# NDLOHGRP/pyReCoDe

Measured on AMD Instinct MI355X. Metric: frames/sec + GB/s in, 4096x4096 uint16 @1% sparsity, 1/2/4/8 GPU, higher is better.
Workload: dtype u16; 1 GPU; 4096x4096 uint16, 1.00% sparsity, L1 + LZ4 frame, source_bit_depth 16, batch 64 frames/GPU/step, 256-frame stack/GPU in HBM; parallelism=dp1 (contiguous frame blocks per rank; single process: no collective), gather_every=0, gathers_issued_in_all=0, launch=single process, collective_ranks=1

## Files before the change

### pyrecode_amd/csrc/rc_api.hip

```cpp
#include "rc_host.h"
#include "rc_deflate_model.h"

thread_local std::string g_last_error;
WorkerPool *g_pool = new WorkerPool;
Util g_utils[RC_MAX_DEV];
thread_local Util *t_util = nullptr;


struct rc_ctx {
    int device = 0;
    hipStream_t own_stream = nullptr, stream = nullptr;
    uint32_t nx = 0, ny = 0, depth = 0, level = 0, op_mode = 0, scheme = 0, clevel = 0, max_batch = 0;
    uint32_t emit = rc::EMIT_RAW;
    rc::Scratch sets[2];
    int cur = 0;
    int last = 0;
    const rc::Scratch &geo() const { return sets[0]; }
    const rc::Scratch &recent() const { return sets[last]; }
    DevMem dmem, model_mem[2];
    PinMem hmem;
    hipStream_t pstream = nullptr;
    hipStream_t pstream_b = nullptr;
    hipStream_t last_ps = nullptr;
    bool two_chains = false;
    hipEvent_t ev_red[2] = {}, ev_post[2] = {}, ev_in[2] = {};
    bool post_pending[2] = {false, false};
    bool pipelined = false;
    bool thr_set = false;
    bool keep_bitmap = true;
    uint32_t src_bytes = 2;
    uint32_t *thr32 = nullptr;
    uint32_t last_n = 0;
    DevBuf d_frames, d_out, d_dark;
    uint64_t *d_rec_off = nullptr;
    uint32_t *d_md = nullptr;
    void *d_ztab = nullptr;
    rc::ValueStage values = rc::VALUES_NONE;
    bool values_on = false;
    bool modelled = false, model_ready = false;
    rc::ZstdModel *d_model = nullptr, *h_model = nullptr;
    rc::ZstdSample *d_sample = nullptr, *h_sample = nullptr;
    rc::DeflateModel *d_dzm = nullptr, *h_dzm = nullptr;
    uint32_t *d_dzhist = nullptr, *h_dzhist = nullptr;
    uint32_t l2_sum = 0;
    rc::u32x2 *d_l2_node[2] = {};
    uint16_t *d_l2_base[2] = {};
    rc::BatchStatus *h_status = nullptr;
    rc::BatchStatus *d_first_err = nullptr;
    uint32_t batch_seq = 0;
    const uint8_t *prev_out = nullptr, *prev_rec = nullptr, *prev_md = nullptr;
    uint64_t prev_out_cap = 0;
    uint32_t prev_n = 0;
    hipEvent_t ev[5] = {};
    float stage_ms[5] = {};
    bool profiling = false;
    uint32_t prof_every = 1, prof_phase = 0;
    bool profile_all = getenv("RC_PROFILE_ALL_STAGES") != nullptr;
    struct PipeSlot {
        uint8_t *d_in = nullptr;
        uint8_t *d_out = nullptr;
        uint64_t *d_rec = nullptr, *h_rec = nullptr;
        uint32_t *d_md = nullptr, *h_md = nullptr;
        rc::BatchStatus *h_stat = nullptr;
        hipEvent_t ev_h2d = nullptr, ev_done = nullptr, ev_fetch = nullptr, ev_val = nullptr;
        uint32_t *d_val = nullptr, *h_val = nullptr;
        bool has_val = false;
        uint32_t n = 0;
        bool zero_copy = false;
        enum State { FREE, SUBMITTED, RESULT_TAKEN, FETCHING } state = FREE;
    } pipe[RC_PIPE_SLOTS];
    hipStream_t copy_stream = nullptr, d2h_stream = nullptr;
    uint32_t val_gap = 0, val_x0 = 0, val_y0 = 0, val_w = 0, val_h = 0;
    std::vector<hipEvent_t> prof_ev;
    size_t prof_used = 0;
    double prof_sum_ms[5] = {};
    uint64_t prof_batches = 0;
};

RC_EXPORT int rc_abi_version(void) { return RC_ABI_VERSION; }

RC_EXPORT const char *rc_strerror(int status)
{
    switch (status) {
    case RC_OK: return "ok";
    case RC_ERR_BAD_ARG: return "bad argument";
    case RC_ERR_OUT_TOO_SMALL: return "output buffer too small";
    case RC_ERR_DEVICE: return "GPU / HIP error";
    case RC_ERR_UNSUPPORTED: return "not implemented on device";
    case RC_ERR_RECORD_TOO_LARGE: return "Buffer size smaller than compressed data size";
    case RC_ERR_CORRUPT: return "corrupt input stream";
    case RC_ERR_WORKSPACE: return "out of device memory for the ctx's workspace";
    default: return "unknown status";
    }
}
RC_EXPORT const char *rc_last_error(void) { return g_last_error.c_str(); }

RC_EXPORT int rc_device_count(int *count)
{
    if (!count) return fail(RC_ERR_BAD_ARG, "count is NULL");
    int n = 0;
    if (hipGetDeviceCount(&n) != hipSuccess) {
        (void)hipGetLastError();
        n = 0;
    }
    *count = n;
    return RC_OK;
}
RC_EXPORT int rc_scheme_on_device(uint32_t scheme)
{
    return (scheme == RC_SCHEME_LZ4 || scheme == RC_SCHEME_ZSTD || scheme == RC_SCHEME_BLOSC_LZ4 || scheme == RC_SCHEME_ZLIB_DEVICE) ? 1 : 0;
}

static int alloc_set(rc_ctx *c, rc::Scratch &sc, DevMem &model_mem)
{
    using namespace rc;
    DevMem &m = c->dmem;
    const uint64_t B = c->max_batch, T = sc.ntiles;
    RC_ALLOC(m, sc.bitmap, B * sc.nb_stride + 64);
    RC_ALLOC(m, sc.tile_cnt, B * T * 4);
    RC_ALLOC(m, sc.tile_off, B * T * 4);
    RC_ALLOC(m, sc.tile_next, B * T * 4);
    RC_ALLOC(m, sc.frame_nnz, B * 4);
    RC_ALLOC(m, sc.frame_cbytes, B * 4);
    RC_ALLOC(m, sc.scan_part, B * ((T + 255) / 256) * 32);
    RC_ALLOC(m, sc.status, sizeof(BatchStatus));
    if (c->level != 3) RC_ALLOC(m, sc.pix_slots, B * T * TILE_PX * 2 + 64);
    if (c->emit != EMIT_RAW) {
        if (c->level == 1) {
            sc.comb = c->emit == EMIT_ZSTD ? COMB_AT_BLK_SLOT : COMB_BEHIND_BLOCK;
            sc.blk_stride = 1536;
        }
        RC_ALLOC(m, sc.blk_slots, B * T * (uint64_t)sc.blk_stride + 256);
        RC_ALLOC(m, sc.blk_size, B * T * 4);
        RC_ALLOC(m, sc.blk_off, B * T * 4);
        if (c->emit == EMIT_DEFLATE) {
            RC_ALLOC(m, sc.blk_aux, B * T * 4);
            RC_ALLOC(m, sc.zl_acc, B * 32);
            HIP_TRY(hipMemset(sc.zl_acc, 0, B * 32));
        }
    }
    if (c->values != VALUES_NONE) {
        const ValueGeom g = value_geom(c->values);
        sc.pixraw_stride = ((sc.N * 2 + 15) & ~15ull) + 32;
        sc.nchunk_max = (uint32_t)((sc.N * 2 + g.chunk - 1) / g.chunk) + 1;
        RC_ALLOC(model_mem, sc.pixraw, B * sc.pixraw_stride + 64);
        RC_ALLOC(model_mem, sc.pix_chunks, B * (uint64_t)sc.nchunk_max * g.slot + 64);
        if (c->values == VALUES_DEFLATE_HUFF) RC_ALLOC(model_mem, sc.chunk_aux, B * (uint64_t)(sc.nchunk_max + 1) * 8);
        RC_ALLOC(model_mem, sc.chunk_size, B * (uint64_t)sc.nchunk_max * 4);
        RC_ALLOC(model_mem, sc.chunk_off, B * (uint64_t)sc.nchunk_max * 4);
        RC_ALLOC(model_mem, sc.frame_pbytes, B * 4);
        HIP_TRY(hipMemset(sc.frame_pbytes, 0, B * 4));
    }
    HIP_TRY(hipMemset(sc.frame_nnz, 0, B * 4));
    HIP_TRY(hipMemset(sc.frame_cbytes, 0, B * 4));
    HIP_TRY(hipMemset(sc.status, 0, sizeof(BatchStatus)));
    return RC_OK;
}

static void free_value_stage(rc_ctx *c)
{
    c->values = rc::VALUES_NONE;
    c->values_on = false;
    for (int k = 0; k < 2; ++k) {
        rc::Scratch &set = c->sets[k];
        c->model_mem[k].release_all();
        set.pixraw = nullptr; set.pix_chunks = nullptr; set.chunk_aux = nullptr; set.chunk_size = nullptr; set.chunk_off = nullptr;
        set.frame_pbytes = nullptr; set.pixraw_stride = 0; set.nchunk_max = 0;
    }
}

static int ctx_alloc(rc_ctx *c)
{
    using namespace rc;
    const uint64_t B = c->max_batch;
    RC_ON_DEVICE(c->device);
    HIP_TRY(hipStreamCreateWithFlags(&c->own_stream, hipStreamNonBlocking));
    HIP_TRY(hipStreamCreateWithFlags(&c->pstream, hipStreamNonBlocking));
    {
        int lo = 0, hi = 0;
        HIP_TRY(hipDeviceGetStreamPriorityRange(&lo, &hi));
        HIP_TRY(hipStreamCreateWithPriority(&c->pstream_b, hipStreamNonBlocking, hi));
    }
    c->last_ps = c->pstream;
    c->stream = c->own_stream;
    DevMem &m = c->dmem;
    int r;
    RC_ALLOC(m, c->sets[0].thr, c->geo().N * 2);
    RC_ALLOC(m, c->d_first_err, sizeof(BatchStatus));
    HIP_TRY(hipMemset(c->d_first_err, 0, sizeof(BatchStatus)));
    c->sets[0].first_err = c->d_first_err;
    c->sets[1] = c->sets[0];
    for (int k = 0; k < 2; ++k)
        if ((r = alloc_set(c, c->sets[k], c->model_mem[k])) != RC_OK) return r;
    c->two_chains = false;
    if (c->level == 2) {
        const uint64_t ids = (uint64_t)c->geo().ntiles * rc::TILE_PX;
        RC_ALLOC(m, c->d_l2_node[0], B * ids * 8);
        HIP_TRY(hipMemset(c->d_l2_node[0], 0, B * ids * 8));
        RC_ALLOC(m, c->d_l2_base[0], B * (uint64_t)c->geo().ntiles * 64 * 2);
        for (int i = 0; i < 2; ++i) {
            Scratch &set = c->sets[i];
            set.l2_node = c->d_l2_node[0]; set.l2_ids_per_frame = ids; set.l2_base = c->d_l2_base[0];
        }
    }
    if (c->emit == EMIT_ZSTD) {
        if ((r = zstd_encoder_tables(m, c->d_ztab)) != RC_OK) return r;
        c->modelled = c->clevel != 0;
        if (c->modelled) {
            RC_ALLOC(m, c->d_model, sizeof(ZstdModel));
            RC_ALLOC(m, c->d_sample, sizeof(ZstdSample));
            RC_ALLOC(c->hmem, c->h_model, sizeof(ZstdModel));
            RC_ALLOC(c->hmem, c->h_sample, sizeof(ZstdSample));
        }
    }
    if (c->values == VALUES_DEFLATE_HUFF) {
        RC_ALLOC(m, c->d_dzm, sizeof(DeflateModel));
        RC_ALLOC(m, c->d_dzhist, 256 * 4);
        RC_ALLOC(c->hmem, c->h_dzm, sizeof(DeflateModel));
        RC_ALLOC(c->hmem, c->h_dzhist, 256 * 4);
    }
    RC_ALLOC(m, c->d_rec_off, (B + 1) * 8);
    RC_ALLOC(m, c->d_md, B * 3 * 4);
    RC_ALLOC(c->hmem, c->h_status, 2 * sizeof(BatchStatus));
    for (auto &e : c->ev) HIP_TRY(hipEventCreate(&e));
    for (auto &e : c->ev_red) HIP_TRY(hipEventCreateWithFlags(&e, hipEventDisableTiming));
    for (auto &e : c->ev_post) HIP_TRY(hipEventCreateWithFlags(&e, hipEventDisableTiming));
    for (auto &e : c->ev_in) HIP_TRY(hipEventCreateWithFlags(&e, hipEventDisableTiming));
    return RC_OK;
}

RC_EXPORT rc_ctx *rc_ctx_create(uint32_t nx, uint32_t ny, uint32_t src_bit_depth, uint32_t reduction_level,
                                uint32_t op_mode, uint32_t scheme, uint32_t clevel, int device_id, uint32_t max_batch,
                                int *status)
{
    int dummy;
    if (!status) status = &dummy;
    *status = RC_OK;
    if (nx == 0 || ny == 0 || max_batch == 0 || max_batch > 65535u || op_mode > 1) {
        *status = fail(RC_ERR_BAD_ARG, "nx, ny, max_batch must be > 0, max_batch <= 65535 and op_mode 0 or 1");
        return nullptr;
    }
    if ((uint64_t)nx * ny >= (1ull << 32)) {
        *status = fail(RC_ERR_BAD_ARG, "nx*ny must be < 2^32");
        return nullptr;
    }
    if ((uint64_t)nx * ny * 2 >= (1ull << 32)) {
        *status = fail(RC_ERR_UNSUPPORTED, "a raw frame of 4 GiB or more (nx*ny*bytes_per_pixel >= 2^32) does not fit the format's u32 size fields");
        return nullptr;
    }
    if (reduction_level < 1 || reduction_level > 3) {
        *status = fail(RC_ERR_UNSUPPORTED, "reduction_level 4 (centroiding) is not implemented on device");
        return nullptr;
    }
    if (reduction_level == 2 && nx > 65535u) {
        *status = fail(RC_ERR_UNSUPPORTED, "reduction_level 2 needs nx <= 65535");
        return nullptr;
    }
    if (src_bit_depth < 1 || src_bit_depth > 32) {
        *status = fail(RC_ERR_UNSUPPORTED, "source_bit_depth must be 1..32 (uint8 / uint16 / uint32 source frames)");
        return nullptr;
    }
    int ndev = 0;
    if (hipGetDeviceCount(&ndev) != hipSuccess || device_id < 0 || device_id >= ndev) {
        (void)hipGetLastError();
        *status = fail(RC_ERR_DEVICE, "no such HIP device (this library has no CPU path)");
        return nullptr;
    }
    rc_ctx *c = new (std::nothrow) rc_ctx();
    if (!c) {
        *status = fail(RC_ERR_DEVICE, "out of host memory");
        return nullptr;
    }
    c->device = device_id;
    c->nx = nx; c->ny = ny; c->depth = src_bit_depth; c->level = reduction_level; c->op_mode = op_mode;
    c->scheme = scheme; c->clevel = clevel; c->max_batch = max_batch;
    c->emit = (op_mode == 1 && rc_scheme_on_device(scheme)) ? scheme : rc::EMIT_RAW;
    c->values = rc::value_stage_of(c->emit, clevel, reduction_level);
    rc::Scratch &sc = c->sets[0];
    sc.N = (uint64_t)nx * ny;
    sc.ntiles = (uint32_t)((sc.N + rc::TILE_PX - 1) / rc::TILE_PX);
    sc.nb = (sc.N + 7) / 8;
    sc.nb_stride = (uint64_t)sc.ntiles * rc::TILE_BM;
    sc.max_batch = max_batch;
    sc.guarded_loads = getenv("RC_REDUCE_GUARDED_LOADS") != nullptr;
    int rcode = ctx_alloc(c);
    if (rcode != RC_OK) {
        *status = rcode;
        std::string keep = g_last_error;
        rc_ctx_destroy(c);
        g_last_error = keep;
        return nullptr;
    }
    return c;
}

RC_EXPORT int rc_ctx_destroy(rc_ctx *c)
{
    if (!c) return RC_OK;
    DeviceGuard dev_guard_;
    (void)dev_guard_.enter(c->device);
    for (hipStream_t st : {c->stream, c->pstream, c->pstream_b, c->own_stream, c->copy_stream, c->d2h_stream})
        if (st) (void)hipStreamSynchronize(st);
    c->dmem.release_all();
    for (DevMem &m : c->model_mem) m.release_all();
    c->hmem.release_all();
    for (auto &p : c->pipe)
        for (hipEvent_t e : {p.ev_h2d, p.ev_done, p.ev_fetch, p.ev_val})
            if (e) (void)hipEventDestroy(e);
    for (hipEvent_t e : {c->ev_red[0], c->ev_red[1], c->ev_post[0], c->ev_post[1], c->ev_in[0], c->ev_in[1]})
        if (e) (void)hipEventDestroy(e);
    for (auto &e : c->ev)
        if (e) (void)hipEventDestroy(e);
    for (auto &e : c->prof_ev) (void)hipEventDestroy(e);
    for (hipStream_t st : {c->copy_stream, c->d2h_stream, c->pstream, c->pstream_b, c->own_stream})
        if (st) (void)hipStreamDestroy(st);
    delete c;
    return RC_OK;
}

RC_EXPORT int rc_ctx_set_stream(rc_ctx *c, void *hip_stream)
{
    if (!c) return fail(RC_ERR_BAD_ARG, "ctx is NULL");
    c->stream = hip_stream ? reinterpret_cast<hipStream_t>(hip_stream) : c->own_stream;
    return RC_OK;
}

RC_EXPORT int rc_set_threshold(rc_ctx *c, const void *thr)
{
    if (!c || !thr) return fail(RC_ERR_BAD_ARG, "ctx / thr is NULL");
    if (c->depth > 16 && c->src_bytes != 4) return fail(RC_ERR_BAD_ARG, "src_bit_depth > 16 means uint32 sources: rc_ctx_set_source_bytes(ctx, 4) first");
    RC_ON_DEVICE(c->device);
    HIP_TRY(hipMemcpyAsync(c->src_bytes == 4 ? (void *)c->thr32 : (void *)c->geo().thr, thr, c->geo().N * (c->src_bytes == 4 ? 4 : 2),
                           is_device_ptr(thr) ? hipMemcpyDeviceToDevice : hipMemcpyHostToDevice,
                           c->stream));
    HIP_TRY(hipStreamSynchronize(c->stream));
    c->thr_set = true;
    return RC_OK;
}

RC_EXPORT int rc_set_dark(rc_ctx *c, const void *dark, int64_t epsilon)
{
    if (!c || !dark) return fail(RC_ERR_BAD_ARG, "ctx / dark is NULL");
    RC_ON_DEVICE(c->device);
    const void *src = dark;
    const uint64_t bytes = c->geo().N * c->src_bytes;
    if (!is_device_ptr(dark)) {
        int r = c->d_dark.ensure(c->dmem, bytes);
        if (r != RC_OK) return r;
        HIP_TRY(hipMemcpyAsync(c->d_dark.p, dark, bytes, hipMemcpyHostToDevice, c->stream));
        src = c->d_dark.p;
    }
    if (c->depth > 16 && c->src_bytes != 4) return fail(RC_ERR_BAD_ARG, "src_bit_depth > 16 means uint32 sources: rc_ctx_set_source_bytes(ctx, 4) first");
    if (c->src_bytes == 4) rc::launch_threshold32(static_cast<const uint32_t *>(src), epsilon, c->geo().N, c->thr32, c->stream);
    else rc::launch_threshold(src, epsilon, c->geo().N, c->geo().thr, c->stream, c->src_bytes);
    HIP_TRY(hipGetLastError());
    HIP_TRY(hipStreamSynchronize(c->stream));
    c->thr_set = true;
    return RC_OK;
}

RC_EXPORT int rc_ctx_set_source_bytes(rc_ctx *c, uint32_t bytes_per_pixel)
{
    if (!c) return fail(RC_ERR_BAD_ARG, "ctx is NULL");
    if (bytes_per_pixel != 1 && bytes_per_pixel != 2 && bytes_per_pixel != 4) return fail(RC_ERR_BAD_ARG, "rc_ctx_set_source_bytes: 1 (uint8), 2 (uint16) or 4 (uint32)");
    if (bytes_per_pixel == 1 && c->depth > 8) return fail(RC_ERR_BAD_ARG, "rc_ctx_set_source_bytes: uint8 sources need src_bit_depth <= 8");
    if (bytes_per_pixel == 2 && c->depth > 16) return fail(RC_ERR_BAD_ARG, "rc_ctx_set_source_bytes: uint16 sources need src_bit_depth <= 16");
    if (c->batch_seq || c->thr_set) return fail(RC_ERR_BAD_ARG, "rc_ctx_set_source_bytes: call before rc_set_dark / rc_set_threshold and the first batch");
    if (c->geo().N * bytes_per_pixel >= (1ull << 32))
        return fail(RC_ERR_UNSUPPORTED, "rc_ctx_set_source_bytes: a raw frame of 4 GiB or more (nx*ny*bytes_per_pixel >= 2^32) does not fit the format's u32 size fields");
    if (bytes_per_pixel == 4) {
        if (c->depth <= 16) return fail(RC_ERR_BAD_ARG, "rc_ctx_set_source_bytes: uint32 sources are what source_bit_depth > 16 means (misc.py:41-49)");
        if (c->level == 2) return fail(RC_ERR_UNSUPPORTED, "rc_ctx_set_source_bytes: reduction level 2 is not implemented for uint32 sources");
        if (c->emit == rc::EMIT_DEFLATE) return fail(RC_ERR_UNSUPPORTED, "rc_ctx_set_source_bytes: the device DEFLATE encoder is not implemented for uint32 sources (use RC_SCHEME_ZLIB: the host's zlib)");
        RC_ON_DEVICE(c->device);
        uint32_t *thr32 = nullptr;
        uint16_t *slots[2] = {nullptr, nullptr};
        bool ok = c->dmem.try_alloc(thr32, c->geo().N * 4) == hipSuccess;
        for (int k = 0; ok && k < 2 && c->level != 3; ++k)
            ok = c->dmem.try_alloc(slots[k], (uint64_t)c->max_batch * c->geo().ntiles * rc::TILE_PX * 4 + 64) == hipSuccess;
        if (!ok) {
            (void)hipGetLastError();
            c->dmem.free_one(thr32);
            for (uint16_t *&p : slots) c->dmem.free_one(p);
            return fail(RC_ERR_DEVICE, "rc_ctx_set_source_bytes: out of device memory for the uint32 threshold / residual slots");
        }
        if (c->depth % 8 == 0) c->depth = 32;
        c->modelled = false;
        free_value_stage(c);
        c->thr32 = thr32;
        for (int k = 0; k < 2; ++k) {
            rc::Scratch *set = &c->sets[k];
            set->pix_slot_bytes = rc::TILE_PX * 4;
            set->comb = rc::COMB_OFF;
            if (c->level != 3) {
                c->dmem.free_one(set->pix_slots);
                set->pix_slots = slots[k];
            }
        }
    }
    c->src_bytes = bytes_per_pixel;
    return RC_OK;
}
RC_EXPORT uint32_t rc_ctx_source_bytes(const rc_ctx *c) { return c ? c->src_bytes : 0; }

RC_EXPORT uint64_t rc_out_capacity(const rc_ctx *c, uint32_t n) { return c ? (uint64_t)n * c->geo().N * c->src_bytes : 0; }

RC_EXPORT uint32_t rc_md_fields(const rc_ctx *c)
{
    if (!c) return 0;
    const bool comp = c->emit != rc::EMIT_RAW;
    if (c->level != 3) return comp ? 3 : 1;
    return comp ? 1 : 0;
}

static int fit_value_model(rc_ctx *c, const void *frames_dev, uint32_t n)
{
    using namespace rc;
    const bool dz = c->values == VALUES_DEFLATE_HUFF;
    hipStream_t s = c->stream;
    const Scratch &sc = c->sets[c->cur];
    const uint32_t ns = n < 2 ? n : 2;
    void *d_sample = dz ? (void *)c->d_dzhist : c->d_sample, *h_sample = dz ? (void *)c->h_dzhist : c->h_sample;
    void *d_model = dz ? (void *)c->d_dzm : c->d_model, *h_model = dz ? (void *)c->h_dzm : c->h_model;
    const size_t sample_bytes = dz ? 256 * 4 : sizeof(ZstdSample), model_bytes = dz ? sizeof(DeflateModel) : sizeof(ZstdModel);
    for (int k = 0; k < 2; ++k)
        if (c->post_pending[k]) HIP_TRY(hipStreamWaitEvent(s, c->ev_post[k], 0));
    HIP_TRY(hipMemsetAsync(d_sample, 0, sample_bytes, s));
    if (dz) {
        launch_reduce(sc, frames_dev, ns, 1u, CODEC_DEFLATE, true, c->depth, s, nullptr, c->src_bytes);
        launch_scans(sc, ns, true, true, s);
        RecordParams rp;
        rp.level = 1u; rp.emit = c->emit; rp.depth = c->depth; rp.first_frame_id = 0; rp.packed_slots = 1u;
        rp.frame_bytes = c->geo().N * c->src_bytes;
        rp.pix_mode = PIX_MODE_FLAT;
        launch_assemble(sc, rp, ns, nullptr, nullptr, c->batch_seq, s);
        launch_pd_hist(sc, ns, c->depth, c->d_dzhist, s);
    } else {
        launch_reduce(sc, frames_dev, ns, c->level == 3 ? 3u : 1u, CODEC_ZSTD_FAST, true, c->depth, s, nullptr, c->src_bytes);
        launch_zstd_sample(sc, ns, c->level == 1, c->depth, c->d_sample, s);
    }
    HIP_TRY(hipGetLastError());
    HIP_TRY(hipMemcpyAsync(h_sample, d_sample, sample_bytes, hipMemcpyDeviceToHost, s));
    HIP_TRY(hipStreamSynchronize(s));
    if (dz) {
        dm_build_model(c->h_dzhist, c->h_dzm);
        c->values_on = c->h_dzm->usable != 0;
    } else {
        zstd_model_from_sample(c->h_sample, c->h_model, c->clevel == 1 ? 50u : (c->clevel == 2 ? 20u : 0u));
        if (c->values == VALUES_NONE || !zm_code_pays(c->h_sample->pix, c->h_model->pix_code)) c->h_model->valid &= ~ZM_PIX_CODE;
        c->values_on = (c->h_model->valid & ZM_PIX_CODE) != 0;
    }
    HIP_TRY(hipMemcpyAsync(d_model, h_model, model_bytes, hipMemcpyHostToDevice, s));
    HIP_TRY(hipStreamSynchronize(s));
    for (Scratch &set : c->sets) {
        if (dz) { set.dz_model = c->d_dzm; continue; }
        const ZstdModel &M = *c->h_model;
        set.zm_model = c->d_model;
        set.zm_lit_code = c->d_model->lit_code;
        set.zm_valid = M.valid;
        set.zm_budget = zm_block_budget(M, BLK_SLOT);
        set.zm_seq_bits = (M.valid & ZM_SEQ_TABLES) ? M.seq.ll_log + M.seq.ml_log : 12u;
    }
    c->model_ready = true;
    return RC_OK;
}

static uint32_t fused_codec(uint32_t emit, uint32_t clevel, bool modelled, uint32_t src_bytes)
{
    using namespace rc;
    switch (emit) {
    case EMIT_ZSTD: return modelled && src_bytes != 4 ? CODEC_ZSTD_MODELLED : CODEC_ZSTD_FAST;
    case EMIT_LZ4: return clevel != 0 ? CODEC_LZ4_EVENTS : CODEC_LZ4_RUNS;
    case EMIT_BLOSC: return CODEC_BLOSC;
    case EMIT_DEFLATE: return CODEC_DEFLATE;
    default: return CODEC_NONE;
    }
}

static int enqueue_batch(rc_ctx *c, const void *frames_dev, uint32_t n, uint32_t first_frame_id, uint8_t *out_dev,
                         uint64_t out_cap, uint64_t *rec_off_dev, uint32_t *md_dev, bool timed)
{
    using namespace rc;
    hipStream_t s = c->stream;
    if ((c->modelled || c->values == VALUES_DEFLATE_HUFF) && !c->model_ready) {
        int r = fit_value_model(c, frames_dev, n);
        if (r != RC_OK) return r;
    }
    RecordParams rp;
    rp.level = c->level == 3 ? 3u : 1u;
    rp.emit = c->emit; rp.depth = c->depth; rp.first_frame_id = first_frame_id;
    rp.packed_slots = 1u;
    rp.frame_bytes = c->geo().N * c->src_bytes;
    hipEvent_t *ev = nullptr;
    if (timed) ev = c->ev;
    else if (c->profiling && (c->prof_phase++ % c->prof_every) == 0) {
        if (c->prof_used + 5 > c->prof_ev.size()) {
            for (int i = 0; i < 5; ++i) {
                hipEvent_t e;
                HIP_TRY(hipEventCreate(&e));
                c->prof_ev.push_back(e);
            }
        }
        ev = c->prof_ev.data() + c->prof_used;
        c->prof_used += 5;
    }
    const int k = c->cur;
    c->cur ^= 1;
    c->last = k;
    const rc::Scratch &sc = c->sets[k];
    const bool two = c->pipelined && c->two_chains;
    hipStream_t ps = two && k == 1 ? c->pstream_b : c->pstream;
    c->last_ps = ps;
    if (c->post_pending[k]) HIP_TRY(hipStreamWaitEvent(s, c->ev_post[k], 0));
    if (ev) HIP_TRY(hipEventRecord(ev[0], s));
    const bool fitted_seq = c->modelled && (c->h_model->valid & ZM_SEQ_TABLES);
    hipStream_t tail = nullptr;
    if (sc.N % TILE_PX) {
        HIP_TRY(hipEventRecord(c->ev_in[k], s));
        HIP_TRY(hipStreamWaitEvent(ps, c->ev_in[k], 0));
        tail = ps;
    }
    const uint32_t codec = fused_codec(c->emit, c->clevel, c->modelled, c->src_bytes);
    const bool keep_maps = c->keep_bitmap || c->emit == EMIT_RAW;
    if (c->src_bytes == 4)
        launch_reduce32(sc, static_cast<const uint32_t *>(frames_dev), c->thr32, n, c->level, c->depth, s, codec, keep_maps);
    else
        launch_reduce(sc, frames_dev, n, c->level, codec, keep_maps, c->depth, s, tail, c->src_bytes);
    const bool all_ev = ev && (timed || c->profile_all);
    hipEvent_t red = ev ? ev[1] : c->ev_red[k];
    HIP_TRY(hipEventRecord(red, s));
    HIP_TRY(hipStreamWaitEvent(ps, red, 0));
    if (c->level == 2) launch_l2(sc, n, c->nx, c->l2_sum, c->depth, ps);
    const bool lits_only = c->modelled && (c->h_model->valid & ZM_LITS_ONLY);
    if (c->emit == EMIT_ZSTD && !lits_only) launch_zstd_fse(sc, n, fitted_seq ? (const void *)&c->d_model->seq : c->d_ztab, fitted_seq, ps);
    if (all_ev) HIP_TRY(hipEventRecord(ev[2], ps));
    launch_scans(sc, n, c->level != 3, c->emit != EMIT_RAW, ps);
    if (all_ev) HIP_TRY(hipEventRecord(ev[3], ps));
    if (c->values_on) {
        rp.pix_mode = PIX_MODE_FLAT;
        launch_assemble(sc, rp, n, out_dev, rec_off_dev, c->batch_seq, ps);
        launch_values_encode(c->values, sc, n, c->depth, ps);
        launch_values_scan(c->values, sc, n, c->depth, ps);
        rp.pix_mode = PIX_MODE_SKIP;
    }
    if (two && c->post_pending[k ^ 1]) {
        auto overlap = [](const uint8_t *a, uint64_t an, const uint8_t *b, uint64_t bn) { return a && b && a < b + bn && b < a + an; };
        const uint8_t *rec8 = reinterpret_cast<const uint8_t *>(rec_off_dev), *md8 = reinterpret_cast<const uint8_t *>(md_dev);
        if (overlap(out_dev, out_cap, c->prev_out, c->prev_out_cap) || overlap(rec8, (uint64_t)(n + 1) * 8, c->prev_rec, (uint64_t)(c->prev_n + 1) * 8) ||
            overlap(md8, (uint64_t)n * 12, c->prev_md, (uint64_t)c->prev_n * 12))
            HIP_TRY(hipStreamWaitEvent(ps, c->ev_post[k ^ 1], 0));
    }
    c->prev_out = out_dev; c->prev_out_cap = out_cap; c->prev_n = n;
    c->prev_rec = reinterpret_cast<const uint8_t *>(rec_off_dev); c->prev_md = reinterpret_cast<const uint8_t *>(md_dev);
    launch_layout(sc, rp, n, out_cap, rec_off_dev, md_dev, ps);
    launch_assemble(sc, rp, n, out_dev, rec_off_dev, c->batch_seq, ps);
    ++c->batch_seq;
    if (c->values_on) launch_values_gather(c->values, sc, n, c->depth, 16, out_dev, rec_off_dev, ps);
    if (ev) HIP_TRY(hipEventRecord(ev[4], ps));
    if (two && c->post_pending[k ^ 1]) HIP_TRY(hipStreamWaitEvent(ps, c->ev_post[k ^ 1], 0));
    HIP_TRY(hipEventRecord(c->ev_post[k], ps));
    c->post_pending[k] = true;
    if (!c->pipelined) HIP_TRY(hipStreamWaitEvent(s, c->ev_post[k], 0));
    HIP_TRY(hipGetLastError());
    c->last_n = n;
    return RC_OK;
}

static int check_batch_args(rc_ctx *c, const void *frames, uint32_t n, const void *out, const void *rec, const void *md)
{
    if (!c || !frames || !out || !rec || !md) return fail(RC_ERR_BAD_ARG, "NULL argument");
    if (n == 0 || n > c->max_batch) return fail(RC_ERR_BAD_ARG, "n must be in 1..max_batch");
    if (!c->thr_set) return fail(RC_ERR_BAD_ARG, "threshold not set (rc_set_threshold / rc_set_dark)");
    return RC_OK;
}

RC_EXPORT int rc_reduce_compress_batch_async(rc_ctx *c, const void *frames_dev, uint32_t n, uint32_t first_frame_id,
                                             uint8_t *out_dev, uint64_t out_cap, uint64_t *rec_offsets_dev, uint32_t *md_dev)
{
    int r = check_batch_args(c, frames_dev, n, out_dev, rec_offsets_dev, md_dev);
    if (r != RC_OK) return r;
    RC_ON_DEVICE(c->device);
    return enqueue_batch(c, frames_dev, n, first_frame_id, out_dev, out_cap, rec_offsets_dev, md_dev, false);
}

static void l2_second_chain(rc_ctx *c)
{
    if (c->level != 2 || c->two_chains) return;
    const uint64_t B = c->max_batch, ids = (uint64_t)c->geo().ntiles * rc::TILE_PX;
    if (!c->d_l2_node[1]) {
        bool ok = c->dmem.try_alloc(c->d_l2_node[1], B * ids * 8) == hipSuccess && hipMemset(c->d_l2_node[1], 0, B * ids * 8) == hipSuccess &&
                  c->dmem.try_alloc(c->d_l2_base[1], B * (uint64_t)c->geo().ntiles * 64 * 2) == hipSuccess && hipDeviceSynchronize() == hipSuccess;
        if (!ok) {
            (void)hipGetLastError();
            c->dmem.free_one(c->d_l2_node[1]);
            c->dmem.free_one(c->d_l2_base[1]);
            return;
        }
    }
    c->sets[1].l2_node = c->d_l2_node[1];
    c->sets[1].l2_base = c->d_l2_base[1];
    c->two_chains = true;
}

RC_EXPORT int rc_ctx_set_pipelined(rc_ctx *c, int on)
{
    if (!c) return fail(RC_ERR_BAD_ARG, "ctx is NULL");
    RC_ON_DEVICE(c->device);
    HIP_TRY(hipStreamSynchronize(c->pstream));
    HIP_TRY(hipStreamSynchronize(c->pstream_b));
    if (on) l2_second_chain(c);
    c->pipelined = on != 0;
    return RC_OK;
}
RC_EXPORT int rc_ctx_wait_results(rc_ctx *c, void *hip_stream)
{
    if (!c) return fail(RC_ERR_BAD_ARG, "ctx is NULL");
    RC_ON_DEVICE(c->device);
    if (c->post_pending[c->last])
        HIP_TRY(hipStreamWaitEvent(hip_stream ? reinterpret_cast<hipStream_t>(hip_stream) : c->stream, c->ev_post[c->last], 0));
    return RC_OK;
}

RC_EXPORT int rc_ctx_sync(rc_ctx *c)
{
    if (!c) return fail(RC_ERR_BAD_ARG, "ctx is NULL");
    RC_ON_DEVICE(c->device);
    HIP_TRY(hipStreamSynchronize(c->pstream_b));
    HIP_TRY(hipMemcpyAsync(&c->h_status[0], c->recent().status, sizeof(rc::BatchStatus), hipMemcpyDeviceToHost, c->pstream));
    HIP_TRY(hipMemcpyAsync(&c->h_status[1], c->d_first_err, sizeof(rc::BatchStatus), hipMemcpyDeviceToHost, c->pstream));
    HIP_TRY(hipMemsetAsync(c->d_first_err, 0, sizeof(rc::BatchStatus), c->pstream));
    HIP_TRY(hipStreamSynchronize(c->pstream));
    HIP_TRY(hipStreamSynchronize(c->stream));
    const uint32_t n_batches = c->batch_seq;
    c->batch_seq = 0;
    for (size_t b = 0; b + 5 <= c->prof_used; b += 5) {
        float ms;
        if (!c->profile_all) {
            if (hipEventElapsedTime(&ms, c->prof_ev[b], c->prof_ev[b + 1]) == hipSuccess) c->prof_sum_ms[0] += ms;
        } else
        for (int i = 0; i < 4; ++i)
            if (hipEventElapsedTime(&ms, c->prof_ev[b + i], c->prof_ev[b + i + 1]) == hipSuccess) c->prof_sum_ms[i] += ms;
        if (hipEventElapsedTime(&ms, c->prof_ev[b], c->prof_ev[b + 4]) == hipSuccess) c->prof_sum_ms[4] += ms;
        ++c->prof_batches;
    }
    c->prof_used = 0;
    if (c->h_status[1].total != 0) c->h_status[1] = rc::first_err_decode(c->h_status[1].total);
    if (c->h_status[1].code != 0) {
        char msg[160];
        if (n_batches > 1)
            snprintf(msg, sizeof msg, "%s (frame %u of batch %llu of the %u enqueued since the last sync)", rc_strerror(c->h_status[1].code),
                     c->h_status[1].frame, (unsigned long long)c->h_status[1].total, n_batches);
        else
            snprintf(msg, sizeof msg, "%s (frame %u of the batch)", rc_strerror(c->h_status[1].code), c->h_status[1].frame);
        return fail(c->h_status[1].code, msg);
    }
    return RC_OK;
}

RC_EXPORT int rc_reduce_compress_batch(rc_ctx *c, const void *frames, uint32_t n, uint32_t first_frame_id, uint8_t *out,
                                       uint64_t out_cap, uint64_t *rec_offsets, uint32_t *md)
{
    int r = check_batch_args(c, frames, n, out, rec_offsets, md);
    if (r != RC_OK) return r;
    RC_ON_DEVICE(c->device);
    const uint64_t frame_bytes = c->geo().N * c->src_bytes;
    const void *fdev = frames;
    if (!is_device_ptr(frames)) {
        r = c->d_frames.ensure(c->dmem, (uint64_t)n * frame_bytes);
        if (r != RC_OK) return r;
        HIP_TRY(hipMemcpyAsync(c->d_frames.p, frames, (uint64_t)n * frame_bytes, hipMemcpyHostToDevice, c->stream));
        fdev = c->d_frames.p;
    }
    uint8_t *odev = out;
    uint64_t cap = out_cap;
    const bool out_host = !is_device_ptr(out);
    if (out_host) {
        const uint64_t worst = (uint64_t)n * frame_bytes;
        cap = out_cap < worst ? out_cap : worst;
        r = c->d_out.ensure(c->dmem, cap);
        if (r != RC_OK) return r;
        odev = c->d_out.p;
    }
    r = enqueue_batch(c, fdev, n, first_frame_id, odev, cap, c->d_rec_off, c->d_md, true);
    if (r != RC_OK) return r;
    r = rc_ctx_sync(c);
    for (int i = 0; i < 4; ++i) (void)hipEventElapsedTime(&c->stage_ms[i], c->ev[i], c->ev[i + 1]);
    (void)hipEventElapsedTime(&c->stage_ms[4], c->ev[0], c->ev[4]);
    if (r != RC_OK) return r;
    int r2 = copy_out(rec_offsets, c->d_rec_off, (uint64_t)(n + 1) * 8, c->stream);
    if (r2 == RC_OK) r2 = copy_out(md, c->d_md, (uint64_t)n * 12, c->stream);
    if (r2 == RC_OK && out_host) r2 = copy_out(out, c->d_out.p, c->h_status->total, c->stream);
    if (r2 != RC_OK) return r2;
    HIP_TRY(hipStreamSynchronize(c->stream));
    return RC_OK;
}

RC_EXPORT void *rc_host_alloc(uint64_t bytes)
{
    void *p = nullptr;
    if (hipHostMalloc(&p, bytes ? bytes : 16, hipHostMallocDefault) != hipSuccess) {
        (void)hipGetLastError();
        fail(RC_ERR_DEVICE, "hipHostMalloc failed");
        return nullptr;
    }
    return p;
}
RC_EXPORT int rc_host_free(void *p)
{
    if (p) HIP_TRY(hipHostFree(p));
    return RC_OK;
}
RC_EXPORT int rc_host_register(void *p, uint64_t bytes)
{
    if (!p || !bytes) return fail(RC_ERR_BAD_ARG, "NULL / zero argument");
    HIP_TRY(hipHostRegister(p, bytes, hipHostRegisterDefault));
    return RC_OK;
}
RC_EXPORT int rc_host_unregister(void *p)
{
    if (p) HIP_TRY(hipHostUnregister(p));
    return RC_OK;
}

static int pipe_slot_init(rc_ctx *c, rc_ctx::PipeSlot &p)
{
    const uint64_t B = c->max_batch;
    if (!c->copy_stream) HIP_TRY(hipStreamCreateWithFlags(&c->copy_stream, hipStreamNonBlocking));
    if (!c->d2h_stream) HIP_TRY(hipStreamCreateWithFlags(&c->d2h_stream, hipStreamNonBlocking));
    RC_ALLOC(c->dmem, p.d_in, B * c->geo().N * c->src_bytes + 64);
    RC_ALLOC(c->dmem, p.d_out, rc_out_capacity(c, (uint32_t)B) + 64);
    RC_ALLOC(c->dmem, p.d_rec, (B + 1) * 8);
    RC_ALLOC(c->dmem, p.d_md, B * 12);
    RC_ALLOC(c->hmem, p.h_rec, (B + 1) * 8);
    RC_ALLOC(c->hmem, p.h_md, B * 12);
    RC_ALLOC(c->hmem, p.h_stat, sizeof(rc::BatchStatus));
    HIP_TRY(hipEventCreateWithFlags(&p.ev_h2d, hipEventDisableTiming));
    HIP_TRY(hipEventCreateWithFlags(&p.ev_done, hipEventDisableTiming));
    HIP_TRY(hipEventCreateWithFlags(&p.ev_fetch, hipEventDisableTiming));
    HIP_TRY(hipEventCreateWithFlags(&p.ev_val, hipEventDisableTiming));
    RC_ALLOC(c->dmem, p.d_val, B * 4 + 64);
    RC_ALLOC(c->hmem, p.h_val, B * 4 + 64);
    return RC_OK;
}

RC_EXPORT int rc_ctx_set_validation(rc_ctx *c, uint32_t gap, uint32_t x0, uint32_t y0, uint32_t w, uint32_t h)
{
    if (!c) return fail(RC_ERR_BAD_ARG, "ctx is NULL");
    if (gap && (w == 0 || h == 0 || w > 128 || h > 128 || (uint64_t)x0 + w > c->nx || (uint64_t)y0 + h > c->ny))
        return fail(RC_ERR_BAD_ARG, "rc_ctx_set_validation: the region must lie inside the frame and hold at most 128 x 128 pixels");
    c->val_gap = gap; c->val_x0 = x0; c->val_y0 = y0; c->val_w = w; c->val_h = h;
    return RC_OK;
}

RC_EXPORT int rc_pipe_validation(rc_ctx *c, uint32_t slot, uint32_t *counts)
{
    if (!c || slot >= RC_PIPE_SLOTS || !counts) return fail(RC_ERR_BAD_ARG, "NULL argument / slot out of range");
    rc_ctx::PipeSlot &p = c->pipe[slot];
    if (p.state != p.SUBMITTED && p.state != p.RESULT_TAKEN) return fail(RC_ERR_BAD_ARG, "nothing submitted on this slot");
    if (!p.has_val) { for (uint32_t i = 0; i < p.n; ++i) counts[i] = 0xFFFFFFFFu; return RC_OK; }
    HIP_TRY(hipEventSynchronize(p.ev_val));
    memcpy(counts, p.h_val, (uint64_t)p.n * 4);
    return RC_OK;
}

RC_EXPORT int rc_pipe_submit(rc_ctx *c, uint32_t slot, const void *frames_host, uint32_t n, uint32_t first_frame_id)
{
    if (!c || !frames_host || slot >= RC_PIPE_SLOTS) return fail(RC_ERR_BAD_ARG, "NULL argument / slot out of range");
    if (n == 0 || n > c->max_batch) return fail(RC_ERR_BAD_ARG, "n must be in 1..max_batch");
    if (!c->thr_set) return fail(RC_ERR_BAD_ARG, "threshold not set (rc_set_threshold / rc_set_dark)");
    RC_ON_DEVICE(c->device);
    rc_ctx::PipeSlot &p = c->pipe[slot];
    if (p.state != p.FREE) return fail(RC_ERR_BAD_ARG, "slot is still in use (result / fetch_wait not called)");
    if (!p.d_in) {
        int r = pipe_slot_init(c, p);
        if (r != RC_OK) return r;
    }
    if (!c->pipelined) {
        HIP_TRY(hipStreamSynchronize(c->pstream));
        HIP_TRY(hipStreamSynchronize(c->pstream_b));
        l2_second_chain(c);
        c->pipelined = true;
    }
    const void *fdev = nullptr;
    hipPointerAttribute_t a;
    if (hipPointerGetAttributes(&a, frames_host) == hipSuccess) {
        if (a.type == hipMemoryTypeHost && a.devicePointer) fdev = a.devicePointer;
    } else (void)hipGetLastError();
    p.zero_copy = fdev != nullptr;
    if (!fdev) {
        HIP_TRY(hipMemcpyAsync(p.d_in, frames_host, (uint64_t)n * c->geo().N * c->src_bytes, hipMemcpyHostToDevice, c->copy_stream));
        HIP_TRY(hipEventRecord(p.ev_h2d, c->copy_stream));
        HIP_TRY(hipStreamWaitEvent(c->stream, p.ev_h2d, 0));
        fdev = p.d_in;
    }
    int r = enqueue_batch(c, fdev, n, first_frame_id, p.d_out, rc_out_capacity(c, c->max_batch), p.d_rec, p.d_md, false);
    if (r != RC_OK) return r;
    p.has_val = c->val_gap != 0;
    if (p.has_val) {
        rc::launch_roi_components(fdev, c->src_bytes == 4 ? (const void *)c->thr32 : (const void *)c->geo().thr, c->geo().N, c->nx, n, first_frame_id, c->val_gap, c->val_x0, c->val_y0, c->val_w, c->val_h, p.d_val, c->stream, c->src_bytes);
        HIP_TRY(hipGetLastError());
        HIP_TRY(hipMemcpyAsync(p.h_val, p.d_val, (uint64_t)n * 4, hipMemcpyDeviceToHost, c->stream));
        HIP_TRY(hipEventRecord(p.ev_val, c->stream));
    }
    if (p.zero_copy) HIP_TRY(hipEventRecord(p.ev_h2d, c->stream));
    hipStream_t ps = c->last_ps;
    HIP_TRY(hipMemcpyAsync(p.h_rec, p.d_rec, (uint64_t)(n + 1) * 8, hipMemcpyDeviceToHost, ps));
    HIP_TRY(hipMemcpyAsync(p.h_md, p.d_md, (uint64_t)n * 12, hipMemcpyDeviceToHost, ps));
    HIP_TRY(hipMemcpyAsync(p.h_stat, c->recent().status, sizeof(rc::BatchStatus), hipMemcpyDeviceToHost, ps));
    HIP_TRY(hipEventRecord(p.ev_done, ps));
    p.n = n;
    p.state = p.SUBMITTED;
    return RC_OK;
}

RC_EXPORT int rc_pipe_input_done(rc_ctx *c, uint32_t slot)
{
    if (!c || slot >= RC_PIPE_SLOTS) return fail(RC_ERR_BAD_ARG, "NULL argument / slot out of range");
    if (c->pipe[slot].state == rc_ctx::PipeSlot::FREE) return RC_OK;
    HIP_TRY(hipEventSynchronize(c->pipe[slot].ev_h2d));
    return RC_OK;
}

RC_EXPORT int rc_pipe_result(rc_ctx *c, uint32_t slot, uint64_t *rec_offsets, uint32_t *md, uint64_t *total)
{
    if (!c || slot >= RC_PIPE_SLOTS || !rec_offsets || !md || !total) return fail(RC_ERR_BAD_ARG, "NULL argument / slot out of range");
    rc_ctx::PipeSlot &p = c->pipe[slot];
    if (p.state != p.SUBMITTED) return fail(RC_ERR_BAD_ARG, "nothing submitted on this slot");
    HIP_TRY(hipEventSynchronize(p.ev_done));
    p.state = p.RESULT_TAKEN;
    if (p.h_stat->code != 0) {
        char msg[128];
        snprintf(msg, sizeof msg, "%s (frame %u of the batch)", rc_strerror(p.h_stat->code), p.h_stat->frame);
        p.state = p.FREE;
        return fail(p.h_stat->code, msg);
    }
    memcpy(rec_offsets, p.h_rec, (uint64_t)(p.n + 1) * 8);
    memcpy(md, p.h_md, (uint64_t)p.n * 12);
    *total = p.h_stat->total;
    return RC_OK;
}

RC_EXPORT int rc_pipe_fetch(rc_ctx *c, uint32_t slot, uint8_t *dst_host, uint64_t bytes)
{
    if (!c || slot >= RC_PIPE_SLOTS || (!dst_host && bytes)) return fail(RC_ERR_BAD_ARG, "NULL argument / slot out of range");
    rc_ctx::PipeSlot &p = c->pipe[slot];
    if (p.state != p.RESULT_TAKEN) return fail(RC_ERR_BAD_ARG, "rc_pipe_result has not been called for this slot");
    if (bytes > p.h_stat->total) return fail(RC_ERR_BAD_ARG, "more bytes than the batch's records hold");
    RC_ON_DEVICE(c->device);
    if (bytes) HIP_TRY(hipMemcpyAsync(dst_host, p.d_out, bytes, hipMemcpyDeviceToHost, c->d2h_stream));
    HIP_TRY(hipEventRecord(p.ev_fetch, c->d2h_stream));
    p.state = p.FETCHING;
    return RC_OK;
}

RC_EXPORT int rc_pipe_fetch_wait(rc_ctx *c, uint32_t slot)
{
    if (!c || slot >= RC_PIPE_SLOTS) return fail(RC_ERR_BAD_ARG, "NULL argument / slot out of range");
    rc_ctx::PipeSlot &p = c->pipe[slot];
    if (p.state == p.RESULT_TAKEN) { p.state = p.FREE; return RC_OK; }
    if (p.state != p.FETCHING) return fail(RC_ERR_BAD_ARG, "rc_pipe_fetch has not been called for this slot");
    HIP_TRY(hipEventSynchronize(p.ev_fetch));
    p.state = p.FREE;
    return RC_OK;
}

RC_EXPORT int rc_ctx_refit_model(rc_ctx *c)
{
    if (!c) return fail(RC_ERR_BAD_ARG, "ctx is NULL");
    c->model_ready = false;
    return RC_OK;
}

RC_EXPORT int rc_get_binary_map(rc_ctx *c, uint32_t i, uint8_t *bitmap_out)
{
    if (!c || !bitmap_out) return fail(RC_ERR_BAD_ARG, "NULL argument");
    if (i >= c->last_n) return fail(RC_ERR_BAD_ARG, "frame index outside the most recent batch");
    if (!c->keep_bitmap && c->emit != rc::EMIT_RAW && c->level != 2) return fail(RC_ERR_BAD_ARG, "binary maps are not kept (rc_ctx_keep_binary_maps(ctx, 0))");
    RC_ON_DEVICE(c->device);
    int r = copy_out(bitmap_out, c->recent().bitmap + (uint64_t)i * c->geo().nb_stride, c->geo().nb, c->stream);
    if (r != RC_OK) return r;
    HIP_TRY(hipStreamSynchronize(c->stream));
    return RC_OK;
}

RC_EXPORT int rc_ctx_set_profiling(rc_ctx *c, int on)
{
    if (!c) return fail(RC_ERR_BAD_ARG, "ctx is NULL");
    c->profiling = on != 0;
    c->prof_every = on > 1 ? (uint32_t)on : 1u;
    c->prof_phase = 0;
    for (double &v : c->prof_sum_ms) v = 0;
    c->prof_batches = 0;
    return RC_OK;
}
RC_EXPORT int rc_ctx_get_profile(rc_ctx *c, double sum_ms[5], uint64_t *batches)
{
    if (!c || !sum_ms || !batches) return fail(RC_ERR_BAD_ARG, "NULL argument");
    memcpy(sum_ms, c->prof_sum_ms, sizeof c->prof_sum_ms);
    *batches = c->prof_batches;
    return RC_OK;
}

RC_EXPORT int rc_ctx_set_l2_statistics(rc_ctx *c, uint32_t l2_statistics)
{
    if (!c || l2_statistics > 2) return fail(RC_ERR_BAD_ARG, "l2_statistics must be 0, 1 (max) or 2 (sum)");
    c->l2_sum = l2_statistics == 2 ? 1u : 0u;
    return RC_OK;
}

RC_EXPORT int rc_ctx_keep_binary_maps(rc_ctx *c, int on)
{
    if (!c) return fail(RC_ERR_BAD_ARG, "ctx is NULL");
    c->keep_bitmap = on != 0;
    return RC_OK;
}

RC_EXPORT int rc_get_stage_ms(rc_ctx *c, float ms[5])
{
    if (!c || !ms) return fail(RC_ERR_BAD_ARG, "NULL argument");
    memcpy(ms, c->stage_ms, sizeof c->stage_ms);
    return RC_OK;
}

RC_EXPORT int64_t rc_unpack_frame_sparse(uint32_t nx, uint32_t ny, uint32_t bit_depth, const uint8_t *bitmap,
                                         const uint8_t *pixvals, uint64_t pixvals_bytes, uint64_t *out,
                                         uint64_t out_cap_triplets, uint32_t reduction_level)
{
    if (!bitmap || nx == 0 || ny == 0 || (!out && out_cap_triplets)) return fail(RC_ERR_BAD_ARG, "NULL / zero argument");
    if (reduction_level == 1 && (bit_depth == 0 || bit_depth > 64)) return fail(RC_ERR_BAD_ARG, "bit_depth must be 1..64");
    if (reduction_level == 1 && !pixvals && pixvals_bytes) return fail(RC_ERR_BAD_ARG, "pixvals is NULL");
    UtilScope util_scope;
    int r = util_scope.enter();
    if (r != RC_OK) return r;
    Util &u = g_util;
    const uint64_t N = (uint64_t)nx * ny, nb = (N + 7) / 8, nb8 = (nb + 7) / 8;
    const uint32_t nblk = (uint32_t)((nb8 + rc::WG - 1) / rc::WG);
    const uint8_t *d_bm = nullptr, *d_px = nullptr;
    r = stage_in(bitmap, nb, u.a, d_bm, nb8 * 8 - nb + 8);
    if (r != RC_OK) return r;
    if (reduction_level == 1 && pixvals_bytes) {
        r = stage_in(pixvals, pixvals_bytes, u.b, d_px);
        if (r != RC_OK) return r;
    }
    r = u.w.ensure(u.dmem, (uint64_t)nblk * 8 + 16);
    if (r != RC_OK) return r;
    uint32_t *blk_cnt = u.w.as<uint32_t>(), *blk_off = blk_cnt + nblk;
    uint64_t *nnz_dev = reinterpret_cast<uint64_t *>(blk_cnt + 2 * (uint64_t)nblk);
    rc::launch_expand_count(d_bm, nb8, N, blk_cnt, blk_off, nnz_dev, u.stream);
    HIP_TRY(hipMemcpyAsync(u.h_scalar, nnz_dev, 8, hipMemcpyDeviceToHost, u.stream));
    HIP_TRY(hipStreamSynchronize(u.stream));
    const uint64_t nnz = *u.h_scalar;
    if (!out) return (int64_t)nnz;
    if (nnz > out_cap_triplets) return fail(RC_ERR_OUT_TOO_SMALL, "out holds fewer triplets than the bitmap has set bits");
    if (reduction_level == 1 && (nnz * bit_depth + 7) / 8 > pixvals_bytes)
        return fail(RC_ERR_CORRUPT, "pixvals shorter than popcount(bitmap) * bit_depth bits");
    if (nnz == 0) return 0;
    StagedOut so;
    if ((r = so.begin(out, nnz * 24)) != RC_OK) return r;
    rc::launch_expand_emit(d_bm, nb8, N, nx, blk_off, d_px, pixvals_bytes, bit_depth, reduction_level, nnz, so.as<uint64_t>(), u.stream);
    HIP_TRY(hipGetLastError());
    if ((r = so.finish(out, nnz * 24)) != RC_OK) return r;
    return (int64_t)nnz;
}

RC_EXPORT int rc_bit_pack(const uint16_t *pixvals, uint64_t n, uint32_t bit_depth, uint8_t *out, uint64_t out_n)
{
    if (!out || (!pixvals && n)) return fail(RC_ERR_BAD_ARG, "NULL argument");
    if (bit_depth == 0 || bit_depth > 32) return fail(RC_ERR_BAD_ARG, "bit_depth must be 1..32");
    if (out_n != (n * bit_depth + 7) / 8) return fail(RC_ERR_BAD_ARG, "out_n must be ceil(n*bit_depth/8)");
    if (out_n == 0) return RC_OK;
    UtilScope util_scope;
    int r = util_scope.enter();
    if (r != RC_OK) return r;
    Util &u = g_util;
    const uint16_t *d_in = nullptr;
    r = stage_in(pixvals, n * 2, u.a, d_in);
    if (r != RC_OK) return r;
    StagedOut so;
    if ((r = so.begin(out, out_n)) != RC_OK) return r;
    rc::launch_bit_pack(d_in, n, bit_depth, so.as<uint8_t>(), out_n, u.stream);
    HIP_TRY(hipGetLastError());
    return so.finish(out, out_n);
}

RC_EXPORT int rc_bit_unpack(const uint8_t *packed, uint64_t packed_bytes, uint64_t n, uint32_t bit_depth, uint64_t *out)
{
    if (!out || (!packed && packed_bytes)) return fail(RC_ERR_BAD_ARG, "NULL argument");
    if (bit_depth == 0 || bit_depth > 64) return fail(RC_ERR_BAD_ARG, "bit_depth must be 1..64");
    if ((n * bit_depth + 7) / 8 > packed_bytes) return fail(RC_ERR_CORRUPT, "packed shorter than n * bit_depth bits");
    if (n == 0) return RC_OK;
    UtilScope util_scope;
    int r = util_scope.enter();
    if (r != RC_OK) return r;
    Util &u = g_util;
    const uint8_t *d_in = nullptr;
    r = stage_in(packed, packed_bytes, u.a, d_in);
    if (r != RC_OK) return r;
    StagedOut so;
    if ((r = so.begin(out, n * 8)) != RC_OK) return r;
    rc::launch_bit_unpack(d_in, packed_bytes, n, bit_depth, so.as<uint64_t>(), u.stream);
    HIP_TRY(hipGetLastError());
    return so.finish(out, n * 8);
}

RC_EXPORT int rc_synth_dark(int device_id, uint32_t seed, uint64_t n_pixels, uint16_t *dark_dev)
{
    if (!dark_dev) return fail(RC_ERR_BAD_ARG, "NULL argument");
    RC_ON_DEVICE(device_id);
    rc::launch_synth_dark(seed, n_pixels, dark_dev, nullptr);
    HIP_TRY(hipGetLastError());
    HIP_TRY(hipDeviceSynchronize());
    return RC_OK;
}
RC_EXPORT int rc_synth_frames_clustered(int device_id, uint32_t seed, uint32_t first_frame, uint32_t n_frames, uint32_t nx, uint32_t ny,
                                        uint32_t seed_ppm, const uint16_t *dark_dev, uint16_t *frames_dev)
{
    if (!dark_dev || !frames_dev || n_frames == 0 || nx == 0 || ny == 0) return fail(RC_ERR_BAD_ARG, "NULL / zero argument");
    if ((uint64_t)nx * ny > 0xFFFFFFFFull) return fail(RC_ERR_BAD_ARG, "rc_synth_frames_clustered: nx * ny must fit 32 bits");
    RC_ON_DEVICE(device_id);
    rc::launch_synth_frames_clustered(seed, first_frame, n_frames, nx, ny, seed_ppm, dark_dev, frames_dev, nullptr);
    HIP_TRY(hipGetLastError());
    HIP_TRY(hipDeviceSynchronize());
    return RC_OK;
}
RC_EXPORT int rc_synth_frames(int device_id, uint32_t seed, uint32_t first_frame, uint32_t n_frames, uint64_t n_pixels,
                              uint32_t sparsity_ppm, const uint16_t *dark_dev, uint16_t *frames_dev)
{
    if (!dark_dev || !frames_dev || n_frames == 0) return fail(RC_ERR_BAD_ARG, "NULL / zero argument");
    RC_ON_DEVICE(device_id);
    rc::launch_synth_frames(seed, first_frame, n_frames, n_pixels, sparsity_ppm, dark_dev, frames_dev, nullptr);
    HIP_TRY(hipGetLastError());
    HIP_TRY(hipDeviceSynchronize());
    return RC_OK;
}
```

### pyrecode_amd/csrc/rc_device.h

```cpp
#pragma once
#include <hip/hip_runtime.h>
#include <stdint.h>
#include <type_traits>

namespace rc {

template <int V> using int_c = std::integral_constant<int, V>;

constexpr int WG = 256;
constexpr int WAVES = WG / 64;
constexpr int R = 8;
constexpr int GROUP_PX = 64 * 8;
constexpr int TILE_PX = R * GROUP_PX;
constexpr int TILE_BM = TILE_PX / 8;
constexpr int SLOT_PX = TILE_PX;
constexpr int BLK_SLOT = TILE_BM + 128;

typedef uint32_t u32x4 __attribute__((ext_vector_type(4)));
typedef uint32_t u32x2 __attribute__((ext_vector_type(2)));
typedef uint16_t u16x2 __attribute__((ext_vector_type(2)));

__device__ __forceinline__ int lane_id() { return threadIdx.x & 63; }

template <int CTRL, int ROW_MASK = 0xF>
__device__ __forceinline__ uint32_t dpp_zero(uint32_t x)
{
    return (uint32_t)__builtin_amdgcn_update_dpp(0, (int)x, CTRL, ROW_MASK, 0xF, true);
}

__device__ __forceinline__ uint32_t wave_incl_scan(uint32_t x)
{
    x += dpp_zero<0x111>(x);
    x += dpp_zero<0x112>(x);
    x += dpp_zero<0x114>(x);
    x += dpp_zero<0x118>(x);
    x += dpp_zero<0x142, 0xA>(x);
    x += dpp_zero<0x143, 0xC>(x);
    return x;
}

__device__ __forceinline__ uint32_t wave_prev(uint32_t x) { return dpp_zero<0x138>(x); }
__device__ __forceinline__ uint32_t wave_next(uint32_t x) { return dpp_zero<0x130>(x); }

__device__ __forceinline__ uint32_t wave_last(uint32_t x) { return (uint32_t)__builtin_amdgcn_readlane((int)x, 63); }

__device__ __forceinline__ uint64_t wave_incl_scan64(uint64_t x)
{
#pragma unroll
    for (int d = 1; d < 64; d <<= 1) {
        uint64_t y = __shfl_up(x, d);
        if (lane_id() >= d) x += y;
    }
    return x;
}

__device__ __forceinline__ uint32_t block_excl_scan(uint32_t v, uint32_t *sm, uint32_t *total)
{
    const int w = threadIdx.x >> 6;
    uint32_t inc = wave_incl_scan(v);
    if (lane_id() == 63) sm[w] = inc;
    __syncthreads();
    uint32_t base = 0, tot = 0;
#pragma unroll
    for (int i = 0; i < WAVES; ++i) {
        uint32_t t = sm[i];
        if (i < w) base += t;
        tot += t;
    }
    __syncthreads();
    *total = tot;
    return base + inc - v;
}

struct BatchStatus {
    int32_t code;
    uint32_t frame;
    uint64_t total;
};
__host__ __device__ inline unsigned long long first_err_key(uint32_t batch_seq, int32_t code, uint32_t frame)
{
    return ~(((unsigned long long)(batch_seq & 0xFFFFFFu) << 40) | ((unsigned long long)((uint32_t)(-code) & 0xFFu) << 32) | frame);
}
inline BatchStatus first_err_decode(unsigned long long key)
{
    const unsigned long long k = ~key;
    return BatchStatus{-(int32_t)((k >> 32) & 0xFFu), (uint32_t)k, k >> 40};
}

}
```

### pyrecode_amd/csrc/rc_gather.hip

```cpp
#include <cstdlib>

#include "rc_launch.h"
#include "rc_record.h"
#include "rc_deflate_block.h"

namespace rc {

struct GatherArgs {
    const uint8_t *blk_slots, *bitmap;
    const uint16_t *pix_slots;
    const uint32_t *blk_size, *blk_off, *tile_cnt, *tile_off, *tile_next, *frame_nnz, *frame_cbytes, *frame_pbytes;
    const uint32_t *blk_aux;
    uint32_t *zl_acc;
    uint8_t *pixraw;
    BatchStatus *status, *first_err;
    uint64_t nb, nb_stride, pixraw_stride;
    uint32_t ntiles, blk_stride, pix_slot_bytes, comb;
};

typedef u32x4 u32x4_u __attribute__((aligned(1)));
typedef u32x2 u32x2_u __attribute__((aligned(1)));
typedef uint32_t u32_u __attribute__((aligned(1)));
typedef uint16_t u16_u __attribute__((aligned(1)));

__device__ __forceinline__ uint32_t lane_get(uint32_t v, uint32_t src_lane)
{
    return (uint32_t)__builtin_amdgcn_ds_bpermute((int)(4u * src_lane), (int)v);
}

template <bool BITS>
__device__ __forceinline__ u32x4 shift_piece(const u32x4 &x, uint32_t e, uint32_t sh)
{
    u32x4 y = x;
    if (BITS) {
        y[0] = __builtin_amdgcn_alignbit(x[1], x[0], sh); y[1] = __builtin_amdgcn_alignbit(x[2], x[1], sh);
        y[2] = __builtin_amdgcn_alignbit(x[3], x[2], sh); y[3] = __builtin_amdgcn_alignbit(e, x[3], sh);
    }
    return y;
}
__device__ __forceinline__ void put_piece(uint8_t *p, const u32x4 &y, uint32_t valid)
{
    if (valid >= 16) { *reinterpret_cast<u32x4_u *>(p) = y; return; }
    uint32_t a0 = y[0], a1 = y[1];
    if (valid & 8u) { *reinterpret_cast<u32x2_u *>(p) = u32x2{a0, a1}; p += 8; a0 = y[2]; a1 = y[3]; }
    if (valid & 4u) { *reinterpret_cast<u32_u *>(p) = a0; p += 4; a0 = a1; }
    if (valid & 2u) { *reinterpret_cast<u16_u *>(p) = (uint16_t)a0; p += 2; a0 >>= 16; }
    if (valid & 1u) *p = (uint8_t)a0;
}

struct AdlerAcc { uint32_t A, W; };
__device__ __forceinline__ void adler_piece(AdlerAcc &acc, const u32x4 &y, uint32_t valid, uint32_t sp)
{
    uint32_t a = 0, q = 0;
#pragma unroll
    for (int k = 0; k < 4; ++k) {
        const uint32_t nb = valid > 4u * k ? min(valid - 4u * k, 4u) : 0u;
        const uint32_t v = y[k] & (nb >= 4u ? 0xFFFFFFFFu : ((1u << (8u * nb)) - 1u));
        a = __builtin_amdgcn_sad_u8(v, 0u, a);
        q = __builtin_amdgcn_udot4(v, 0x03020100u + 0x04040404u * (uint32_t)k, q, false);
    }
    acc.A += a;
    acc.W = (acc.W + (sp % ADLER_P) * a + q) % ADLER_P;
}
__device__ __forceinline__ void adler_byte(AdlerAcc &acc, uint32_t byte, uint32_t sp)
{
    acc.A += byte;
    acc.W = (acc.W + (sp % ADLER_P) * byte) % ADLER_P;
}

struct ResidGeom { uint32_t b_lo, n, ps0, avail; };
__device__ __forceinline__ ResidGeom resid_geom(uint32_t coff, uint32_t cnt, uint32_t d)
{
    const uint64_t dbit = (uint64_t)coff * d;
    const uint32_t nbits = cnt * d;
    const uint64_t b_lo = (dbit + 7) >> 3, b_hi = (dbit + nbits + 7) >> 3;
    ResidGeom g{(uint32_t)b_lo, (uint32_t)(b_hi - b_lo), (uint32_t)(8 * b_lo - dbit), (uint32_t)((dbit + nbits) & 7u)};
    if (g.avail && g.n) --g.n;
    else g.avail = 0;
    return g;
}

constexpr int GATHER_U = 4, GATHER_UB = 3;
constexpr int GATHER_WPE = 8;
template <bool BITS, int U, bool ADLER>
__global__ __launch_bounds__(64) __attribute__((amdgpu_waves_per_eu(GATHER_WPE))) void k_gather(GatherArgs sc, RecordParams rp, uint8_t *__restrict__ out, const uint64_t *__restrict__ rec_off,
                                               uint32_t lz4f_hdr_bitmap, uint32_t lz4f_hdr_pix, uint32_t batch_seq, uint32_t gpf, uint32_t nitems, uint32_t tpi)
{
    if (sc.status->code != 0) {
        if (blockIdx.x == 0 && threadIdx.x == 0 && sc.first_err)
            atomicMax(reinterpret_cast<unsigned long long *>(&sc.first_err->total), first_err_key(batch_seq, sc.status->code, sc.status->frame));
        return;
    }
    const uint32_t lane = (uint32_t)lane_id();
    const bool flat = rp.pix_mode == PIX_MODE_FLAT, skip_pix = rp.pix_mode == PIX_MODE_SKIP;
    const bool pixp = rp.level == 1 && rp.packed_slots && !skip_pix;
    const bool plain_pos = rp.emit == EMIT_RAW || flat;
    const uint32_t d = rp.depth;
    const FrameFmt ff = frame_fmt(rp.emit);
    const uint32_t bhdr = bitmap_hdr(ff, rp.emit, sc.ntiles);
    const uint8_t *pix_base = reinterpret_cast<const uint8_t *>(sc.pix_slots);
    for (uint32_t item = blockIdx.x; item < nitems; item += gridDim.x) {
        const uint32_t f = item / gpf, g = item - f * gpf, t0 = tpi * g, t = t0 + lane;
        const bool have = lane < tpi && t < sc.ntiles;
        const uint64_t frow = (uint64_t)f * sc.ntiles;
        uint8_t *rec = flat ? sc.pixraw + (uint64_t)f * sc.pixraw_stride : out + rec_off[f];
        const uint32_t nnz = rp.level == 1 ? sc.frame_nnz[f] : 0;
        const uint32_t npk = rp.level == 1 ? packed_bytes(nnz, d) : 0;
        uint64_t bitmap_pos = 0, pix_pos = 0;
        uint32_t cb = 0;
        if (!flat) {
            if (rp.emit == EMIT_RAW) { bitmap_pos = rp.level == 1 ? 8 : 4; pix_pos = bitmap_pos + sc.nb; }
            else { cb = bhdr + sc.frame_cbytes[f] + ff.end; bitmap_pos = rp.level == 1 ? 16 : 8; pix_pos = bitmap_pos + cb; }
        }
        if (g == 0 && lane == 0 && !flat) record_fixed_fields(sc, rp, f, rec, bitmap_pos, pix_pos, cb, npk, ff, skip_pix, lz4f_hdr_bitmap, lz4f_hdr_pix);
        uint8_t *pdst = rec + pix_pos;

        uint32_t word = 0, bsz = 0, bdst = 0, cnt = 0, rn = 0, rdst = 0, rs = 0xFFFFFFFFu, ps0 = 0, flags = 0, blo = 0;
        AdlerAcc ad{0u, 0u};
        if (have && rp.emit != EMIT_RAW && (!flat || (sc.comb == COMB_BEHIND_BLOCK && pixp))) word = sc.blk_size[frow + t];
        if (have && !flat) {
            if (rp.emit == EMIT_RAW) {
                const uint64_t b0 = (uint64_t)t * TILE_BM;
                bsz = (uint32_t)min((uint64_t)TILE_BM, sc.nb - b0);
                bdst = (uint32_t)(bitmap_pos + b0);
            } else {
                bsz = word;
                const uint32_t boff = bhdr + sc.blk_off[frow + t];
                bdst = (uint32_t)bitmap_pos + boff;
                if (rp.emit == EMIT_BLOSC) store_u32_le(rec + bitmap_pos + 16 + 4 * (uint64_t)t, boff);
            }
        }
        if (have && pixp) {
            cnt = sc.tile_cnt[frow + t];
            if (cnt) {
                const ResidGeom q = resid_geom(sc.tile_off[frow + t], cnt, d);
                ps0 = q.ps0;
                if (ADLER) blo = q.b_lo;
                if (sc.comb) {
                    const uint32_t ro16 = sc.comb == COMB_AT_BLK_SLOT ? (uint32_t)BLK_SLOT / 16 : (word + 15) >> 4, r16 = (cnt * d + 127) >> 7;
                    if (16 * (ro16 + r16) <= sc.blk_stride) rs = 16 * ro16;
                }
                if (q.n && !plain_pos && ((uint64_t)q.b_lo >> ff.chunk_shift) != (((uint64_t)q.b_lo + q.n - 1) >> ff.chunk_shift)) flags = 1u << 31;
                else rn = q.n;
                rdst = (uint32_t)(pix_pos + (plain_pos ? (uint64_t)q.b_lo : stored_pos(ff, q.b_lo)));
            }
        }
        uint32_t ext_cnt = 0, ext_first = 0;
        if (BITS && pixp && t0 + tpi < sc.ntiles) {
            ext_cnt = sc.tile_cnt[frow + t0 + tpi];
            if (ext_cnt)
                ext_first = *reinterpret_cast<const uint32_t *>(residual_src(sc, frow + t0 + tpi, sc.comb == COMB_BEHIND_BLOCK ? sc.blk_size[frow + t0 + tpi] : 0u, ext_cnt, d));
        }
        const uint8_t *slot = rp.emit == EMIT_RAW ? sc.bitmap + (uint64_t)f * sc.nb_stride + (uint64_t)t0 * TILE_BM : sc.blk_slots + (frow + t0) * sc.blk_stride;
        const uint32_t slot_stride = rp.emit == EMIT_RAW ? (uint32_t)TILE_BM : sc.blk_stride;
        const uint8_t *rslot = pix_base + (frow + t0) * sc.pix_slot_bytes;

        const uint32_t nb16 = (bsz + 15) >> 4, tot = nb16 + ((rn + 15) >> 4);
        const uint32_t incl = wave_incl_scan(tot), cum = incl - tot, T = wave_last(incl);
        const uint32_t packed = bsz | (ps0 << 10) | (rn << 13) | flags;
        for (uint32_t i0 = 0; 64u * i0 < T; i0 += U) {
            u32x4 x[U];
            uint32_t e[U], dsto[U], meta[U];
            uint32_t spos[ADLER ? U : 1];
#pragma unroll
            for (int u = 0; u < U; ++u) {
                const uint32_t P = 64u * (i0 + u) + lane;
                uint32_t k = 0;
#pragma unroll
                for (uint32_t step = 32; step; step >>= 1) {
                    const uint32_t c = lane_get(cum, k + step);
                    if (c <= P) k += step;
                }
                const uint32_t ck = lane_get(cum, k), pk = lane_get(packed, k), bd = lane_get(bdst, k), rd = lane_get(rdst, k), rsk = lane_get(rs, k);
                const uint32_t blk = ADLER ? lane_get(blo, k) : 0u;
                const uint32_t bsz_k = pk & 1023u, ps0_k = (pk >> 10) & 7u, rn_k = (pk >> 13) & 0x7FFFu;
                const uint32_t idx = P - ck, nbk = (bsz_k + 15) >> 4;
                const bool isb = idx < nbk;
                const uint32_t j = isb ? idx : idx - nbk;
                const uint32_t left = (isb ? bsz_k : rn_k) - 16u * j;
                const bool act = P < T;
                const uint8_t *src = isb ? slot + (uint64_t)k * slot_stride + 16u * j
                                         : (rsk == 0xFFFFFFFFu ? rslot + (uint64_t)k * sc.pix_slot_bytes : slot + (uint64_t)k * slot_stride + rsk) + 16u * j;
                dsto[u] = (isb ? bd : rd) + 16u * j;
                meta[u] = act ? (min(left, 16u) | ((isb ? 0u : ps0_k) << 8)) : 0u;
                if (ADLER) spos[u] = isb ? 0xFFFFFFFFu : blk + 16u * j;
                x[u] = u32x4{0u, 0u, 0u, 0u};
                e[u] = 0;
                if (act) {
                    x[u] = *reinterpret_cast<const u32x4 *>(src);
                    if (BITS && !isb && ps0_k) e[u] = *reinterpret_cast<const uint32_t *>(src + 16);
                }
            }
#pragma unroll
            for (int u = 0; u < U; ++u)
                if (meta[u] & 0xFFu) {
                    const u32x4 y = shift_piece<BITS>(x[u], e[u], meta[u] >> 8);
                    put_piece(rec + dsto[u], y, meta[u] & 0xFFu);
                    if (ADLER && spos[u] != 0xFFFFFFFFu) adler_piece(ad, y, meta[u] & 0xFFu, spos[u]);
                }
        }
        if (pixp) {
        ResidGeom q{0u, 0u, 0u, 0u};
        if (cnt) q = resid_geom(sc.tile_off[frow + t], cnt, d);
        for (uint64_t m = __builtin_amdgcn_ballot_w64((packed >> 31) != 0); m; m &= m - 1) {
            const uint32_t k = (uint32_t)__builtin_ctzll(m);
            const uint32_t n = lane_get(q.n, k), p0 = lane_get(q.ps0, k), b0 = lane_get(q.b_lo, k), rsk = lane_get(rs, k);
            const uint32_t *s32 = reinterpret_cast<const uint32_t *>(rsk == 0xFFFFFFFFu ? rslot + (uint64_t)k * sc.pix_slot_bytes : slot + (uint64_t)k * slot_stride + rsk);
            for (uint32_t i = lane; i < n; i += 64) {
                const uint32_t qb = 8 * i + p0;
                const uint32_t v = __builtin_amdgcn_alignbit(s32[(qb >> 5) + 1], s32[qb >> 5], qb & 31u) & 0xFFu;
                pdst[stored_pos(ff, (uint64_t)b0 + i)] = (uint8_t)v;
                if (ADLER) adler_byte(ad, v, b0 + i);
            }
        }
        if (BITS) {

        const uint32_t fin_avail = q.avail, fin_q = 8 * q.n + q.ps0, fin_b = q.b_lo + q.n;
        const uint8_t *psrc = rs == 0xFFFFFFFFu ? rslot + (uint64_t)lane * sc.pix_slot_bytes : slot + (uint64_t)lane * slot_stride + rs;
        const uint32_t first = cnt ? *reinterpret_cast<const uint32_t *>(psrc) : 0u;
        uint32_t byte = 0, got = 8;
        if (fin_avail) {
            byte = (*reinterpret_cast<const u32_u *>(psrc + (fin_q >> 3)) >> (fin_q & 7u)) & ((1u << fin_avail) - 1u);
            got = fin_avail;
        }
        const uint64_t nonempty = __builtin_amdgcn_ballot_w64(cnt != 0);
        uint32_t cur = lane;
        while (__builtin_amdgcn_ballot_w64(got < 8 && cur < 64) != 0) {
            const uint64_t higher = cur >= 63 ? 0ull : nonempty & (~0ull << (cur + 1));
            const uint32_t nxt = higher ? (uint32_t)__builtin_ctzll(higher) : 64u;
            const uint32_t cc = lane_get(cnt, nxt & 63u), fd = lane_get(first, nxt & 63u);
            if (got < 8 && cur < 64) {
                const bool in = nxt < 64;
                const uint32_t c2 = in ? cc : ext_cnt, f2 = in ? fd : ext_first;
                if (in || c2) {
                    const uint32_t take = min(8u - got, c2 * d);
                    byte |= (f2 & ((1u << take) - 1u)) << got;
                    got += take;
                    cur = nxt;
                } else cur = 65;
            }
        }
        if (got < 8) {
            uint32_t tt = cur == 65 ? (t0 + tpi - 1 < sc.ntiles ? sc.tile_next[frow + t0 + tpi - 1] : sc.ntiles) : (t0 + tpi < sc.ntiles ? sc.tile_next[frow + t0 + tpi] : sc.ntiles);
            while (tt < sc.ntiles) {
                const uint32_t cc = sc.tile_cnt[frow + tt];
                const uint32_t fd = *reinterpret_cast<const uint32_t *>(residual_src(sc, frow + tt, sc.comb == COMB_BEHIND_BLOCK ? sc.blk_size[frow + tt] : 0u, cc, d));
                const uint32_t take = min(8u - got, cc * d);
                byte |= (fd & ((1u << take) - 1u)) << got;
                got += take;
                if (got >= 8) break;
                tt = sc.tile_next[frow + tt];
            }
        }
        if (fin_avail) {
            pdst[plain_pos ? (uint64_t)fin_b : stored_pos(ff, fin_b)] = (uint8_t)byte;
            if (ADLER) adler_byte(ad, byte & 0xFFu, fin_b);
        }
        }
        }
        if (ADLER && !flat) {
            const uint32_t aux = have ? sc.blk_aux[frow + t] : 0u;
            const uint32_t tA0 = wave_last(wave_incl_scan(aux & 0xFFFFu)), tW0 = wave_last(wave_incl_scan(aux >> 16));
            const uint32_t tA1 = wave_last(wave_incl_scan(ad.A % ADLER_P)), tW1 = wave_last(wave_incl_scan(ad.W));
            if (lane == 0) {
                uint32_t *acc = sc.zl_acc + 8 * (uint64_t)f;
                if (tA0 | tW0) {
                    __hip_atomic_fetch_add(&acc[0], tA0 % ADLER_P, __ATOMIC_RELAXED, __HIP_MEMORY_SCOPE_AGENT);
                    __hip_atomic_fetch_add(&acc[1], tW0 % ADLER_P, __ATOMIC_RELAXED, __HIP_MEMORY_SCOPE_AGENT);
                }
                if (tA1 | tW1) {
                    __hip_atomic_fetch_add(&acc[2], tA1 % ADLER_P, __ATOMIC_RELAXED, __HIP_MEMORY_SCOPE_AGENT);
                    __hip_atomic_fetch_add(&acc[3], tW1 % ADLER_P, __ATOMIC_RELAXED, __HIP_MEMORY_SCOPE_AGENT);
                }
            }
        }
    }
}

__global__ __launch_bounds__(64) void k_zlib_finish(GatherArgs sc, RecordParams rp, uint8_t *__restrict__ out, const uint64_t *__restrict__ rec_off, uint32_t B)
{
    const uint32_t f = blockIdx.x * 64 + threadIdx.x;
    if (f >= B || sc.status->code != 0) return;
    const FrameFmt ff = frame_fmt(rp.emit);
    const uint32_t *acc = sc.zl_acc + 8 * (uint64_t)f;
    uint8_t *rec = out + rec_off[f];
    const uint32_t cb = bitmap_hdr(ff, rp.emit, sc.ntiles) + sc.frame_cbytes[f] + ff.end, bitmap_pos = rp.level == 1 ? 16u : 8u;
    store_u32_be(rec + bitmap_pos + cb - 4, adler_from_sums(sc.nb, acc[0], acc[1]));
    if (rp.level == 1 && rp.pix_mode != PIX_MODE_SKIP) {
        const uint32_t npk = packed_bytes(sc.frame_nnz[f], rp.depth);
        store_u32_be(rec + bitmap_pos + cb + stored_size(ff, npk) - 4, adler_from_sums(npk, acc[2], acc[3]));
    }
}


void launch_gather(const Scratch &sc, const RecordParams &rp, uint32_t B, uint8_t *out, const uint64_t *rec_off, uint32_t hdr_bitmap, uint32_t hdr_pix,
                   uint32_t batch_seq, hipStream_t s)
{
    uint32_t tpi = 64;
    while (tpi > 8 && (uint64_t)B * ((sc.ntiles + tpi - 1) / tpi) < 1024) tpi >>= 1;
    const uint32_t gpf = (sc.ntiles + tpi - 1) / tpi, nitems = gpf * B, wgs = nitems;
    const GatherArgs ga{sc.blk_slots, sc.bitmap, sc.pix_slots, sc.blk_size, sc.blk_off, sc.tile_cnt, sc.tile_off, sc.tile_next, sc.frame_nnz, sc.frame_cbytes,
                        sc.frame_pbytes, sc.blk_aux, sc.zl_acc, sc.pixraw, sc.status, sc.first_err, sc.nb, sc.nb_stride, sc.pixraw_stride, sc.ntiles, sc.blk_stride, sc.pix_slot_bytes, sc.comb};
    const bool bits = rp.level == 1 && rp.depth % 8 != 0;
    if (rp.emit == EMIT_DEFLATE) {
        if (bits) hipLaunchKernelGGL((k_gather<true, GATHER_UB - 1, true>), dim3(wgs), dim3(64), 0, s, ga, rp, out, rec_off, hdr_bitmap, hdr_pix, batch_seq, gpf, nitems, tpi);
        else hipLaunchKernelGGL((k_gather<false, GATHER_U, true>), dim3(wgs), dim3(64), 0, s, ga, rp, out, rec_off, hdr_bitmap, hdr_pix, batch_seq, gpf, nitems, tpi);
        if (rp.pix_mode != PIX_MODE_FLAT) hipLaunchKernelGGL(k_zlib_finish, dim3((B + 63) / 64), dim3(64), 0, s, ga, rp, out, rec_off, B);
    } else if (bits)
        hipLaunchKernelGGL((k_gather<true, GATHER_UB, false>), dim3(wgs), dim3(64), 0, s, ga, rp, out, rec_off, hdr_bitmap, hdr_pix, batch_seq, gpf, nitems, tpi);
    else
        hipLaunchKernelGGL((k_gather<false, GATHER_U, false>), dim3(wgs), dim3(64), 0, s, ga, rp, out, rec_off, hdr_bitmap, hdr_pix, batch_seq, gpf, nitems, tpi);
}

}
```

### pyrecode_amd/csrc/rc_launch.h

```cpp
#pragma once
#include <hip/hip_runtime.h>
#include <stdint.h>

#include "../../include/recode_hip.h"
#include "rc_device.h"

namespace rc {

struct ZstdModel;
struct DeflateModel;
struct InfStream;

constexpr uint32_t COMB_OFF = 0u;
constexpr uint32_t COMB_BEHIND_BLOCK = 1u;
constexpr uint32_t COMB_AT_BLK_SLOT = 2u;

struct Scratch {
    uint64_t N = 0;
    uint32_t ntiles = 0;
    uint64_t nb = 0;
    uint64_t nb_stride = 0;
    uint32_t max_batch = 0;
    bool guarded_loads = false;
    uint16_t *thr = nullptr;
    uint8_t *bitmap = nullptr;
    uint16_t *pix_slots = nullptr;
    uint32_t pix_slot_bytes = SLOT_PX * 2;
    uint32_t *tile_cnt = nullptr;
    uint32_t *tile_off = nullptr;
    uint32_t *tile_next = nullptr;
    uint8_t *blk_slots = nullptr;
    uint32_t blk_stride = BLK_SLOT;
    uint32_t comb = COMB_OFF;
    uint32_t *blk_size = nullptr;
    uint32_t *blk_aux = nullptr;
    uint32_t *zl_acc = nullptr;
    uint32_t *blk_off = nullptr;
    uint32_t *frame_nnz = nullptr;
    uint32_t *frame_cbytes = nullptr;
    uint32_t *scan_part = nullptr;
    BatchStatus *status = nullptr;
    BatchStatus *first_err = nullptr;
    uint8_t *pixraw = nullptr;
    uint64_t pixraw_stride = 0;
    uint8_t *pix_chunks = nullptr;
    uint32_t *chunk_size = nullptr;
    uint32_t *chunk_off = nullptr;
    uint32_t *frame_pbytes = nullptr;
    uint32_t nchunk_max = 0;
    const ZstdModel *zm_model = nullptr;
    const void *zm_lit_code = nullptr;
    uint32_t zm_valid = 0, zm_budget = 0, zm_seq_bits = 12;
    u32x2 *l2_node = nullptr;
    uint64_t l2_ids_per_frame = 0;
    uint16_t *l2_base = nullptr;
    uint32_t *chunk_aux = nullptr;
    const DeflateModel *dz_model = nullptr;
};

constexpr uint32_t EMIT_RAW = 0u;
constexpr uint32_t EMIT_ZSTD = 1u;
constexpr uint32_t EMIT_LZ4 = 2u;
constexpr uint32_t EMIT_BLOSC = 8u;
constexpr uint32_t EMIT_DEFLATE = 0x100u;
static_assert(EMIT_ZSTD == RC_SCHEME_ZSTD && EMIT_LZ4 == RC_SCHEME_LZ4 && EMIT_BLOSC == RC_SCHEME_BLOSC_LZ4 && EMIT_DEFLATE == RC_SCHEME_ZLIB_DEVICE,
              "rc_ctx_create assigns emit = compression_scheme");

constexpr int CODEC_NONE = 0;
constexpr int CODEC_ZSTD_FAST = 1;
constexpr int CODEC_LZ4_RUNS = 2;
constexpr int CODEC_ZSTD_MODELLED = 3;
constexpr int CODEC_LZ4_EVENTS = 4;
constexpr int CODEC_DEFLATE = 5;
constexpr int CODEC_BLOSC = 8;

constexpr uint32_t PIX_MODE_STORED = 0u;
constexpr uint32_t PIX_MODE_FLAT = 1u;
constexpr uint32_t PIX_MODE_SKIP = 2u;

struct RecordParams {
    uint32_t level;
    uint32_t emit;
    uint32_t depth;
    uint32_t packed_slots;
    uint32_t first_frame_id;
    uint64_t frame_bytes;
    uint32_t pix_mode = PIX_MODE_STORED;
};

void launch_threshold(const void *dark, int64_t eps, uint64_t N, uint16_t *thr, hipStream_t s, uint32_t src_bytes = 2);
void launch_reduce(const Scratch &sc, const void *frames, uint32_t B, uint32_t level, uint32_t codec, bool keep_bitmap,
                   uint32_t depth, hipStream_t s, hipStream_t s_tail = nullptr, uint32_t src_bytes = 2);
void launch_threshold32(const uint32_t *dark, int64_t eps, uint64_t N, uint32_t *thr, hipStream_t s);
void launch_reduce32(const Scratch &sc, const uint32_t *frames, const uint32_t *thr32, uint32_t B, uint32_t level, uint32_t depth, hipStream_t s,
                     uint32_t codec = CODEC_NONE, bool keep_bitmap = true);
void launch_l2(const Scratch &sc, uint32_t B, uint32_t nx, uint32_t use_sum, uint32_t depth, hipStream_t s);
void launch_scans(const Scratch &sc, uint32_t B, bool with_counts, bool with_blocks, hipStream_t s);
void launch_layout(const Scratch &sc, const RecordParams &rp, uint32_t B, uint64_t out_cap, uint64_t *rec_off,
                   uint32_t *md, hipStream_t s);
void launch_assemble(const Scratch &sc, const RecordParams &rp, uint32_t B, uint8_t *out, const uint64_t *rec_off,
                     uint32_t batch_seq, hipStream_t s);
void launch_gather(const Scratch &sc, const RecordParams &rp, uint32_t B, uint8_t *out, const uint64_t *rec_off, uint32_t hdr_bitmap, uint32_t hdr_pix,
                   uint32_t batch_seq, hipStream_t s);
enum ValueStage : uint32_t {
    VALUES_NONE = 0,
    VALUES_ZSTD_HUFF,
    VALUES_DEFLATE_HUFF,
};
inline ValueStage value_stage_of(uint32_t emit, uint32_t clevel, uint32_t level)
{
    if (level == 1 && emit == EMIT_ZSTD && clevel != 0) return VALUES_ZSTD_HUFF;
    return level == 1 && emit == EMIT_DEFLATE && clevel >= 2 ? VALUES_DEFLATE_HUFF : VALUES_NONE;
}
constexpr uint32_t PIX_CHUNK = 1008, PIX_SLOT = 1024, PD_CHUNK = 1u << 15, PD_SLOT = PD_CHUNK + 32;
struct ValueGeom { uint32_t chunk, slot; };
inline ValueGeom value_geom(ValueStage kind) { return kind == VALUES_DEFLATE_HUFF ? ValueGeom{PD_CHUNK, PD_SLOT} : ValueGeom{PIX_CHUNK, PIX_SLOT}; }
void launch_values_encode(ValueStage kind, const Scratch &sc, uint32_t B, uint32_t depth, hipStream_t s);
void launch_values_scan(ValueStage kind, const Scratch &sc, uint32_t B, uint32_t depth, hipStream_t s);
void launch_values_gather(ValueStage kind, const Scratch &sc, uint32_t B, uint32_t depth, uint32_t level1_hdr, uint8_t *out, const uint64_t *rec_off,
                          hipStream_t s);
void launch_pd_hist(const Scratch &sc, uint32_t B, uint32_t depth, uint32_t *hist_dev, hipStream_t s);
struct Lz4Block { uint64_t src_off; uint32_t size; uint32_t raw; };
void launch_lz4_encode_buffer(const Scratch &sc, hipStream_t s, bool events = false);
void launch_lz4_encode_rows(const Scratch &sc, uint32_t B, hipStream_t s, bool events);
void launch_lz4f_gather(const Scratch &sc, uint32_t hdr3, uint8_t *out, hipStream_t s);
void launch_lz4_decode(const uint8_t *src, const Lz4Block *blks, uint32_t nblk, uint32_t *sizes, const uint64_t *dst_off,
                       uint8_t *dst, uint64_t cap, int linked, int *err, hipStream_t s, uint32_t max_stored = 0);
uint32_t lz4f_descriptor(uint8_t bd);
void launch_blosc_encode_blocks(const Scratch &sc, uint32_t B, hipStream_t s);
void launch_blosc_gather(const Scratch &sc, uint8_t *out, hipStream_t s);
void launch_blosc_unshuffle(const uint8_t *in, uint8_t *out, uint64_t nbytes, uint32_t blocksize, uint32_t typesize,
                            uint32_t shuffle, hipStream_t s);
void launch_zstd_encode_blocks(const Scratch &sc, uint32_t B, const void *tables_dev, hipStream_t s);
void launch_zstd_tokenize_rows(const Scratch &sc, uint32_t B, hipStream_t s);
void launch_zstd_fse(const Scratch &sc, uint32_t B, const void *tables_dev, bool fitted, hipStream_t s);
void launch_zstd_sample(const Scratch &sc, uint32_t B, bool with_pix, uint32_t depth, void *sample_dev, hipStream_t s);
size_t zstd_model_bytes();
size_t zstd_sample_bytes();
void zstd_model_from_sample(const void *sample_host, void *model_host, uint32_t speed_permille = 0);
void launch_zstd_gather(const Scratch &sc, uint8_t *out, hipStream_t s);
size_t zstd_tables_bytes();
void zstd_tables_host(void *dst);

template <class S>
__host__ __device__ inline const uint8_t *residual_src(const S &sc, uint64_t ft, uint32_t bn, uint32_t cnt, uint32_t d)
{
    if (sc.comb) {
        const uint32_t ro16 = sc.comb == COMB_AT_BLK_SLOT ? (uint32_t)BLK_SLOT / 16 : (bn + 15) >> 4, r16 = (cnt * d + 127) >> 7;
        if (16 * (ro16 + r16) <= sc.blk_stride) return sc.blk_slots + ft * sc.blk_stride + 16 * ro16;
    }
    return reinterpret_cast<const uint8_t *>(sc.pix_slots) + ft * sc.pix_slot_bytes;
}

void launch_inflate(const uint8_t *data, const InfStream *streams, uint32_t n_map, uint32_t n_val, uint32_t map_cap_max, uint32_t map_units_max,
                    uint32_t val_cap_max, uint32_t val_units_max, uint32_t *cand_pos, uint32_t *ncand, uint32_t *link, uint32_t *unit_cand,
                    uint8_t *out, int *err, hipStream_t s);

void launch_roi_components(const void *frames, const void *thr, uint64_t N, uint32_t nx, uint32_t n, uint32_t first_frame_id, uint32_t gap,
                           uint32_t x0, uint32_t y0, uint32_t w, uint32_t h, uint32_t *counts, hipStream_t s, uint32_t src_bytes = 2);

constexpr uint32_t CALIB_LDS_MAX_FRAMES = 512;
void launch_calib_stats(const uint16_t *stack, uint32_t n, uint64_t N, uint32_t n_stats, float *median, float *sdev, int32_t *range2, hipStream_t s);
void launch_calib_hist(const uint16_t *frames, uint32_t n_stats, uint64_t N, const float *median, const double *edges, uint32_t n_bins,
                       uint64_t *counts, hipStream_t s);
void launch_calib_top(const uint16_t *stack, uint32_t n, uint64_t N, const float *median, uint32_t k, float *acc, uint64_t *n_undefined, hipStream_t s);
}
```

### pyrecode_amd/csrc/rc_reduce.hip

```cpp
#include <cstddef>
#include <cstdlib>
#include <type_traits>

#include "rc_launch.h"
#include "rc_values.h"
#include "rc_pack.h"
#ifdef RC_PHASE_TIMING
__device__ unsigned long long g_phase[16];
#define RC_LZ4_PHASE 1
#endif
#include "rc_lz4_block.h"
#include "rc_zstd_wave.h"
#include "rc_deflate_block.h"

namespace rc {

#ifdef RC_PHASE_TIMING
#define RC_PHASE_BEGIN unsigned long long ph_t_ = __builtin_amdgcn_s_memtime(); unsigned long long ph_a_[8] = {};
#define RC_PHASE(i) do { const unsigned long long ph_n_ = __builtin_amdgcn_s_memtime(); ph_a_[i] = ph_n_ - ph_t_; ph_t_ = ph_n_; \
        if ((i) == 6 && lane_id() == 0 && (blockIdx.x & 63u) == 0) { for (int q_ = 0; q_ < 7; ++q_) atomicAdd(&g_phase[q_], ph_a_[q_]); atomicAdd(&g_phase[7], 1ull); } } while (0)
#else
#define RC_PHASE_BEGIN
#define RC_PHASE(i) do { } while (0)
#endif
constexpr int REDUCE_BZ = 4;

__device__ __forceinline__ uint32_t pk_sub_sat_u16(uint32_t a, uint32_t b)
{
    uint32_t r;
    asm("v_pk_sub_u16 %0, %1, %2 clamp" : "=v"(r) : "v"(a), "v"(b));
    return r;
}
__device__ __forceinline__ uint32_t pk_add_u16(uint32_t a, uint32_t b)
{
    uint32_t r;
    asm("v_pk_add_u16 %0, %1, %2" : "=v"(r) : "v"(a), "v"(b));
    return r;
}
__device__ __forceinline__ uint32_t pk_min_u16(uint32_t a, uint32_t b)
{
    uint32_t r;
    asm("v_pk_min_u16 %0, %1, %2" : "=v"(r) : "v"(a), "v"(b));
    return r;
}

__global__ void k_threshold(const uint16_t *__restrict__ dark, uint32_t eps16, uint64_t N, uint16_t *__restrict__ thr)
{
    uint64_t i = (uint64_t)blockIdx.x * blockDim.x + threadIdx.x;
    const uint64_t stride = (uint64_t)gridDim.x * blockDim.x;
    for (; i < N; i += stride) thr[i] = (uint16_t)(dark[i] + eps16);
}

__global__ void k_threshold8(const uint8_t *__restrict__ dark, uint32_t eps8, uint64_t N, uint16_t *__restrict__ thr)
{
    uint64_t i = (uint64_t)blockIdx.x * blockDim.x + threadIdx.x;
    const uint64_t stride = (uint64_t)gridDim.x * blockDim.x;
    for (; i < N; i += stride) thr[i] = (uint16_t)(uint8_t)(dark[i] + eps8);
}

void launch_threshold(const void *dark, int64_t eps, uint64_t N, uint16_t *thr, hipStream_t s, uint32_t src_bytes)
{
    uint32_t blocks = (uint32_t)((N + 255) / 256);
    if (blocks > 4096) blocks = 4096;
    if (src_bytes == 1)
        hipLaunchKernelGGL(k_threshold8, dim3(blocks), dim3(256), 0, s, static_cast<const uint8_t *>(dark), (uint32_t)((uint64_t)eps & 0xFF), N, thr);
    else
        hipLaunchKernelGGL(k_threshold, dim3(blocks), dim3(256), 0, s, static_cast<const uint16_t *>(dark), (uint32_t)((uint64_t)eps & 0xFFFF), N, thr);
}

template <int SB> struct Src;
template <> struct Src<2> { typedef uint16_t T; typedef u32x4 X; };
template <> struct Src<1> { typedef uint8_t T; typedef u32x2 X; };
__device__ __forceinline__ u32x4 widen8(const u32x2 &v)
{
    return u32x4{__builtin_amdgcn_perm(0u, v[0], 0x0C010C00u), __builtin_amdgcn_perm(0u, v[0], 0x0C030C02u),
                 __builtin_amdgcn_perm(0u, v[1], 0x0C010C00u), __builtin_amdgcn_perm(0u, v[1], 0x0C030C02u)};
}
__device__ __forceinline__ u32x4 widen8(const u32x4 &v) { return v; }

template <bool ALIGNED, bool STREAM, int SB = 2>
__device__ __forceinline__ typename Src<SB>::X load8(const typename Src<SB>::T *__restrict__ base, uint64_t px0, uint64_t N, uint32_t fill)
{
    typedef typename Src<SB>::X X;
    constexpr int PER = 4 / SB;
    if (ALIGNED || px0 + 8 <= N) {
        if (px0 < N) {
            typedef X XU __attribute__((aligned(SB)));
            const XU *p = reinterpret_cast<const XU *>(base + px0);
            return STREAM ? __builtin_nontemporal_load(p) : *p;
        }
    }
    X v;
#pragma unroll
    for (int j = 0; j < 8 / PER; ++j) {
        uint32_t w = 0;
#pragma unroll
        for (int e = 0; e < PER; ++e) {
            const uint64_t k = px0 + (uint64_t)(PER * j + e);
            const uint32_t val = (!ALIGNED && k < N) ? (uint32_t)base[k] : fill;
            w |= val << (8 * SB * e);
        }
        v[j] = w;
    }
    return v;
}

struct Pending {
    bool valid;
    uint64_t ft;
    uint32_t f;
    uint32_t cnt;
    uint32_t csize;
    uint32_t staged;
    u32x2 own;
    uint64_t cown;
    uint32_t aux;
    bool last;
    uint32_t depth;
    uint16_t *buf;
};

__device__ __forceinline__ void vm_issue_loads(u32x4 (&x)[R], const uint16_t *lane_ptr)
{
    const uint8_t *p0 = reinterpret_cast<const uint8_t *>(lane_ptr), *p1 = p0 + 4096;
    asm volatile("global_load_dwordx4 %0, %4, off nt\n\t"
                 "global_load_dwordx4 %1, %4, off offset:1024 nt\n\t"
                 "global_load_dwordx4 %2, %4, off offset:2048 nt\n\t"
                 "global_load_dwordx4 %3, %4, off offset:3072 nt"
                 : "=&v"(x[0]), "=&v"(x[1]), "=&v"(x[2]), "=&v"(x[3]) : "v"(p0) : "memory");
    asm volatile("global_load_dwordx4 %0, %4, off nt\n\t"
                 "global_load_dwordx4 %1, %4, off offset:1024 nt\n\t"
                 "global_load_dwordx4 %2, %4, off offset:2048 nt\n\t"
                 "global_load_dwordx4 %3, %4, off offset:3072 nt"
                 : "=&v"(x[4]), "=&v"(x[5]), "=&v"(x[6]), "=&v"(x[7]) : "v"(p1) : "memory");
}
__device__ __forceinline__ void vm_issue_loads(u32x2 (&x)[R], const uint8_t *lane_ptr)
{
    asm volatile("global_load_dwordx2 %0, %8, off nt\n\t"
                 "global_load_dwordx2 %1, %8, off offset:512 nt\n\t"
                 "global_load_dwordx2 %2, %8, off offset:1024 nt\n\t"
                 "global_load_dwordx2 %3, %8, off offset:1536 nt\n\t"
                 "global_load_dwordx2 %4, %8, off offset:2048 nt\n\t"
                 "global_load_dwordx2 %5, %8, off offset:2560 nt\n\t"
                 "global_load_dwordx2 %6, %8, off offset:3072 nt\n\t"
                 "global_load_dwordx2 %7, %8, off offset:3584 nt"
                 : "=&v"(x[0]), "=&v"(x[1]), "=&v"(x[2]), "=&v"(x[3]), "=&v"(x[4]), "=&v"(x[5]), "=&v"(x[6]), "=&v"(x[7]) : "v"(lane_ptr) : "memory");
}
__device__ __forceinline__ void vm_issue_load1(u32x4 &xr, const uint16_t *lane_ptr, int r)
{
    const uint8_t *p = reinterpret_cast<const uint8_t *>(lane_ptr) + (r >= 4 ? 4096 : 0);
    switch (r & 3) {
    case 0: asm volatile("global_load_dwordx4 %0, %1, off nt" : "=&v"(xr) : "v"(p) : "memory"); break;
    case 1: asm volatile("global_load_dwordx4 %0, %1, off offset:1024 nt" : "=&v"(xr) : "v"(p) : "memory"); break;
    case 2: asm volatile("global_load_dwordx4 %0, %1, off offset:2048 nt" : "=&v"(xr) : "v"(p) : "memory"); break;
    default: asm volatile("global_load_dwordx4 %0, %1, off offset:3072 nt" : "=&v"(xr) : "v"(p) : "memory"); break;
    }
}
__device__ __forceinline__ void vm_issue_load1(u32x2 &xr, const uint8_t *p, int r)
{
    switch (r) {
    case 0: asm volatile("global_load_dwordx2 %0, %1, off nt" : "=&v"(xr) : "v"(p) : "memory"); break;
    case 1: asm volatile("global_load_dwordx2 %0, %1, off offset:512 nt" : "=&v"(xr) : "v"(p) : "memory"); break;
    case 2: asm volatile("global_load_dwordx2 %0, %1, off offset:1024 nt" : "=&v"(xr) : "v"(p) : "memory"); break;
    case 3: asm volatile("global_load_dwordx2 %0, %1, off offset:1536 nt" : "=&v"(xr) : "v"(p) : "memory"); break;
    case 4: asm volatile("global_load_dwordx2 %0, %1, off offset:2048 nt" : "=&v"(xr) : "v"(p) : "memory"); break;
    case 5: asm volatile("global_load_dwordx2 %0, %1, off offset:2560 nt" : "=&v"(xr) : "v"(p) : "memory"); break;
    case 6: asm volatile("global_load_dwordx2 %0, %1, off offset:3072 nt" : "=&v"(xr) : "v"(p) : "memory"); break;
    default: asm volatile("global_load_dwordx2 %0, %1, off offset:3584 nt" : "=&v"(xr) : "v"(p) : "memory"); break;
    }
}
template <class X>
__device__ __forceinline__ void vm_wait_loads(uint32_t later, X (&x)[R])
{
    switch (later) {
    case 1: asm volatile("s_waitcnt vmcnt(1)" ::: "memory"); break;
    case 2: asm volatile("s_waitcnt vmcnt(2)" ::: "memory"); break;
    case 3: asm volatile("s_waitcnt vmcnt(3)" ::: "memory"); break;
    case 4: asm volatile("s_waitcnt vmcnt(4)" ::: "memory"); break;
    case 5: asm volatile("s_waitcnt vmcnt(5)" ::: "memory"); break;
    case 6: asm volatile("s_waitcnt vmcnt(6)" ::: "memory"); break;
    case 7: asm volatile("s_waitcnt vmcnt(7)" ::: "memory"); break;
    case 8: asm volatile("s_waitcnt vmcnt(8)" ::: "memory"); break;
    default: asm volatile("s_waitcnt vmcnt(0)" ::: "memory"); break;
    }
    asm volatile("" : "+v"(x[0]), "+v"(x[1]), "+v"(x[2]), "+v"(x[3]), "+v"(x[4]), "+v"(x[5]), "+v"(x[6]), "+v"(x[7]) :: "memory");
}

constexpr int STAGE_CAP = 256;
struct __attribute__((aligned(16))) WaveStage {
    uint16_t val[TILE_PX];
    uint16_t out[STAGE_CAP];
};
static_assert(offsetof(WaveStage, out) == sizeof(uint16_t) * TILE_PX && STAGE_CAP >= 64, "compact_dense_in_place: `out` lies right behind `val`, an entry per lane");

__device__ __forceinline__ uint32_t store_lines2(const uint8_t *s0, uint8_t *d0, uint32_t q0, const uint8_t *s1, uint8_t *d1, uint32_t q1)
{
    const uint32_t total = q0 + q1, lane = (uint32_t)lane_id();
    for (uint32_t base = 0; base < total; base += 64) {
        const uint32_t i = base + lane;
        if (i < total) {
            const bool second = i >= q0;
            const uint32_t j = second ? i - q0 : i;
            const u32x4 v = *reinterpret_cast<const u32x4 *>((second ? s1 : s0) + 16 * j);
            *reinterpret_cast<u32x4 *>((second ? d1 : d0) + 16 * j) = v;
        }
    }
    return (total + 63u) >> 6;
}

template <bool LEVEL1, int CODEC, bool KEEP_BITMAP>
__device__ __forceinline__ uint32_t flush_pending(const Pending &p, uint32_t tile, uint32_t n_blk, uint8_t *__restrict__ bitmap,
                                                  uint64_t nb_stride, uint16_t *__restrict__ pix_slots, uint32_t *__restrict__ tile_cnt,
                                                  uint8_t *__restrict__ blk_slots, uint32_t *__restrict__ blk_size, Lz4Lds *lz,
                                                  const WaveStage *st, uint32_t blk_stride, uint32_t comb, uint32_t *__restrict__ blk_aux)
{
    if (!p.valid) return 0;
    const int lane = lane_id();
    uint32_t nst = 0;
    const uint8_t *s0 = nullptr, *s1 = nullptr;
    uint8_t *d0 = nullptr, *d1 = nullptr;
    uint32_t q0 = 0, q1 = 0, bsz = 0;
    if (LEVEL1) {
        s0 = reinterpret_cast<const uint8_t *>(p.buf);
        d0 = reinterpret_cast<uint8_t *>(pix_slots + p.ft * SLOT_PX);
        q0 = ((((p.cnt * p.depth + 31) >> 5) + 31u) & ~31u) >> 2;
    }
    if (CODEC == CODEC_LZ4_RUNS || CODEC == CODEC_LZ4_EVENTS || CODEC == CODEC_BLOSC) {
        const uint64_t bytes = CODEC != CODEC_BLOSC ? ((uint64_t)p.own[0] | ((uint64_t)p.own[1] << 32)) : p.cown;
        bsz = lz4_stage_slot(bytes, n_blk, p.csize, *lz, CODEC == CODEC_BLOSC);
    }
    if (CODEC == CODEC_ZSTD_FAST || CODEC == CODEC_ZSTD_MODELLED) {
        (void)zstd_stage_slot(n_blk, p.last, p.staged, *lz);
        bsz = p.staged ? p.staged : 4u;
    }
    if (CODEC == CODEC_DEFLATE) bsz = p.csize;
    if (CODEC) {
        s1 = lz->out;
        d1 = blk_slots + p.ft * blk_stride;
        q1 = min((((bsz + 3) >> 2) + 31u) & ~31u, (uint32_t)BLK_SLOT / 4) >> 2;
    }
    if (LEVEL1 && CODEC && comb) {
        const uint32_t ro16 = comb == COMB_AT_BLK_SLOT ? (uint32_t)BLK_SLOT / 16 : (bsz + 15) >> 4, r16 = (p.cnt * p.depth + 127) >> 7;
        if (16 * (ro16 + r16) <= blk_stride) {
            d0 = d1 + 16 * ro16;
            if (comb == COMB_AT_BLK_SLOT) q0 = (r16 + 7u) & ~7u;
            else { q1 = ro16; q0 = ((ro16 + r16 + 7u) & ~7u) - ro16; }
        }
    }
    if (q0 + q1) nst += store_lines2(s0, d0, q0, s1, d1, q1);
    if (KEEP_BITMAP) {
        *reinterpret_cast<u32x2 *>(bitmap + (uint64_t)p.f * nb_stride + (uint64_t)tile * TILE_BM + lane * 8) = p.own;
        nst += 1;
    }
    if (LEVEL1 || CODEC) {
        const uint32_t word = CODEC == CODEC_ZSTD_FAST || CODEC == CODEC_ZSTD_MODELLED ? p.csize : bsz;
        if (LEVEL1 && CODEC == CODEC_DEFLATE) {
            if (lane < 3) *(lane == 0 ? &tile_cnt[p.ft] : (lane == 1 ? &blk_size[p.ft] : &blk_aux[p.ft])) = lane == 0 ? p.cnt : (lane == 1 ? word : p.aux);
        } else if (LEVEL1 && CODEC) {
            if (lane < 2) *(lane == 0 ? &tile_cnt[p.ft] : &blk_size[p.ft]) = lane == 0 ? p.cnt : word;
        } else if (LEVEL1) {
            if (lane == 0) tile_cnt[p.ft] = p.cnt;
        } else if (CODEC == CODEC_DEFLATE) {
            if (lane < 2) *(lane == 0 ? &blk_size[p.ft] : &blk_aux[p.ft]) = lane == 0 ? word : p.aux;
        } else {
            if (lane == 0) blk_size[p.ft] = word;
        }
        nst += 1;
    }
    return (uint32_t)__builtin_amdgcn_readfirstlane((int)nst);
}

__device__ __forceinline__ void compact_dense_in_place(WaveStage *st, const uint8_t *bm)
{
    const int lane = lane_id();
    uint32_t inc[3], tot[3];
#pragma unroll
    for (int g = 0; g < 3; ++g) {
        uint32_t pk = 0;
#pragma unroll
        for (int k = 0; k < 3; ++k)
            if (3 * g + k < R) pk |= (uint32_t)__builtin_popcount((uint32_t)bm[(3 * g + k) * 64 + lane]) << (10 * k);
        inc[g] = wave_incl_scan(pk);
        tot[g] = wave_last(inc[g]);
    }
    uint32_t base = 0;
#pragma unroll
    for (int r = 0; r < R; ++r) {
        const uint32_t m = bm[r * 64 + lane];
        const uint32_t dst = base + ((inc[r / 3] >> (10 * (r % 3))) & 0x3FFu) - (uint32_t)__builtin_popcount(m);
        const u32x4 v = (reinterpret_cast<const u32x4 *>(st->val) + lane)[r * 64];
        __builtin_amdgcn_wave_barrier();
        uint16_t *const vo = st->val;
#pragma unroll
        for (int j = 0; j < 8; ++j) {
            const uint32_t a = (m >> j) & 1u ? dst + (uint32_t)__builtin_popcount(m & ((1u << j) - 1u)) : (uint32_t)TILE_PX + (uint32_t)lane;
            vo[a] = (uint16_t)(v[j >> 1] >> (16 * (j & 1)));
        }
        __builtin_amdgcn_wave_barrier();
        base += (tot[r / 3] >> (10 * (r % 3))) & 0x3FFu;
    }
}

constexpr uint32_t FUSED12_CAP = (uint32_t)(STAGE_CAP * 16 / 12);
__device__ __forceinline__ void compact_pack12(WaveStage *st, const u32x2 &own, uint32_t exc, uint32_t cnt)
{
    const int lane = lane_id();
    uint32_t *out32 = reinterpret_cast<uint32_t *>(st->out);
    *reinterpret_cast<u32x2 *>(out32 + 2 * lane) = u32x2{0u, 0u};
    __builtin_amdgcn_wave_barrier();
    const uint16_t *mine = st->val + 64 * lane;
    uint64_t q = (uint64_t)own[0] | ((uint64_t)own[1] << 32);
    uint32_t left = cnt, P = 12u * exc;
    do {
        uint32_t x[4];
#pragma unroll
        for (int k = 0; k < 4; ++k) {
            const uint32_t i = q ? (uint32_t)__builtin_ctzll(q) : 0u;
            q &= q - 1;
            x[k] = mine[i];
        }
#pragma unroll
        for (int k = 0; k < 4; ++k) x[k] = (uint32_t)k < left ? (x[k] & 0xFFFu) : 0u;
        const uint32_t lo = x[0] | (x[1] << 12) | (x[2] << 24), hi = (x[2] >> 8) | (x[3] << 4);
        const uint32_t w = P >> 5, sh = P & 31u;
        const uint64_t a = (uint64_t)lo << sh, b = (uint64_t)hi << sh;
        const uint32_t d0 = (uint32_t)a, d1 = (uint32_t)(a >> 32) | (uint32_t)b, d2 = (uint32_t)(b >> 32);
        if (left) {
            __hip_atomic_fetch_or(&out32[w], d0, __ATOMIC_RELAXED, __HIP_MEMORY_SCOPE_WAVEFRONT);
            if (d1) __hip_atomic_fetch_or(&out32[w + 1], d1, __ATOMIC_RELAXED, __HIP_MEMORY_SCOPE_WAVEFRONT);
            if (d2) __hip_atomic_fetch_or(&out32[w + 2], d2, __ATOMIC_RELAXED, __HIP_MEMORY_SCOPE_WAVEFRONT);
        }
        left = left > 4u ? left - 4u : 0u;
        P += 48u;
    } while (__builtin_amdgcn_ballot_w64(left != 0) != 0);
    __builtin_amdgcn_wave_barrier();
}

template <bool ALIGNED, bool ASMLOAD, bool LEVEL1, int CODEC, bool KEEP_BITMAP, bool RAWVAL, int SB>
__device__ __forceinline__ void reduce_one_frame(typename Src<SB>::X (&x)[R], const typename Src<SB>::T *__restrict__ cur, const typename Src<SB>::T *__restrict__ next, bool have_next,
                                                 const u32x4 (&t)[R], uint64_t lane_px0, uint64_t N, bool full,
                                                 uint32_t f, uint32_t tile, uint64_t ft, uint32_t n_blk, uint8_t *__restrict__ bitmap,
                                                 uint64_t nb_stride, uint16_t *__restrict__ pix_slots,
                                                 uint32_t *__restrict__ tile_cnt, uint8_t *__restrict__ blk_slots,
                                                 uint32_t *__restrict__ blk_size, Lz4Lds *s_lz, uint8_t *s_bm, WaveStage *st,
                                                 Pending &pend, uint32_t &stores_behind, const ZmParams &zp, uint32_t blk_stride, uint32_t comb,
                                                 uint32_t *__restrict__ blk_aux)
{
    const int lane = lane_id();
    RC_PHASE_BEGIN
    if (ASMLOAD) vm_wait_loads(stores_behind, x);
    else if (ALIGNED && full) {
        typedef typename Src<SB>::X XU __attribute__((aligned(SB)));
        const XU *p = reinterpret_cast<const XU *>(cur + lane_px0);
#pragma unroll
        for (int r = 0; r < R; ++r) x[r] = __builtin_nontemporal_load(p + r * (GROUP_PX / 8));
    } else {
#pragma unroll
        for (int r = 0; r < R; ++r) x[r] = load8<ALIGNED, true, SB>(cur, lane_px0 + (uint64_t)r * GROUP_PX, N, 0);
    }
    RC_PHASE(0);
    uint32_t m8[R];
#pragma unroll
    for (int r = 0; r < R; ++r) {
        const u32x4 tt = t[r];
        u32x4 xv = widen8(x[r]);
#pragma unroll
        for (int k = 0; k < 4; ++k) xv[k] = pk_sub_sat_u16(xv[k], tt[k]);
        const uint32_t one = 0x00010001u;
        uint32_t M = 0;
#pragma unroll
        for (int k = 3; k >= 0; --k)
            M = __builtin_amdgcn_udot2(__builtin_bit_cast(u16x2, pk_min_u16(xv[k], one)),
                                       __builtin_bit_cast(u16x2, (uint32_t)((1u << (2 * k)) | (2u << (2 * k + 16)))), M, false);
        m8[r] = M;
        if (LEVEL1) {
            u32x4 v = xv;
            if (RAWVAL) {
#pragma unroll
                for (int k = 0; k < 4; ++k) v[k] = pk_add_u16(v[k], tt[k]);
            }
            (reinterpret_cast<u32x4 *>(st->val) + lane)[r * 64] = v;
        }
        if (ASMLOAD && have_next) vm_issue_load1(x[r], next + lane_px0, r);
    }
    RC_PHASE(1);
    RC_PHASE(2);
    pend.valid = true;
    pend.ft = ft;
    pend.f = f;
    pend.cnt = 0;
    pend.csize = 0;
    pend.buf = st->out;
    if (LEVEL1 || KEEP_BITMAP || CODEC) {
        uint8_t *bm = CODEC ? s_lz->raw : s_bm;
#pragma unroll
        for (int r = 0; r < R; ++r) bm[r * 64 + lane] = (uint8_t)m8[r];
        __builtin_amdgcn_wave_barrier();
        pend.own = *reinterpret_cast<const u32x2 *>(&bm[lane * 8]);
    }
    RC_PHASE(3);
    if (LEVEL1) {
        const uint32_t cnt = (uint32_t)__builtin_popcount(pend.own[0]) + (uint32_t)__builtin_popcount(pend.own[1]);
        const uint32_t inc = wave_incl_scan(cnt);
        const uint32_t wave_total = wave_last(inc);
        bool packed = false;
        if (pend.depth == 12 && wave_total <= FUSED12_CAP) {
            if (wave_total) compact_pack12(st, pend.own, inc - cnt, cnt);
            packed = true;
        } else if (wave_total <= (uint32_t)STAGE_CAP) {
#pragma unroll
            for (int h = 0; h < 2; ++h) {
                const uint16_t *mine = st->val + 64 * lane + 32 * h;
                uint32_t qh = pend.own[h];
                uint32_t o = inc - cnt + (h ? (uint32_t)__builtin_popcount(pend.own[0]) : 0u);
                while (qh) {
                    const uint32_t i0 = (uint32_t)__builtin_ctz(qh);
                    qh &= qh - 1;
                    const bool two = qh != 0;
                    const uint32_t i1 = two ? (uint32_t)__builtin_ctz(qh) : i0;
                    qh &= qh - 1;
                    const uint16_t v0 = mine[i0], v1 = mine[i1];
                    st->out[o] = v0;
                    if (two) st->out[o + 1] = v1;
                    o += 2;
                }
            }
        } else {
            pend.buf = st->val;
            __builtin_amdgcn_wave_barrier();
            compact_dense_in_place(st, CODEC ? s_lz->raw : s_bm);
        }
        __builtin_amdgcn_wave_barrier();
        pend.cnt = wave_total;
        if (!packed && pend.depth < 16 && wave_total) pack_stage(pend.buf, wave_total, pend.depth);
    }
    RC_PHASE(4);
    if (CODEC == CODEC_LZ4_RUNS) {
        const uint64_t bytes = (uint64_t)pend.own[0] | ((uint64_t)pend.own[1] << 32);
        pend.csize = lz4_encode_block<false>(bytes, n_blk, *s_lz);
    }
    if (CODEC == CODEC_LZ4_EVENTS) {
        const uint64_t bytes = (uint64_t)pend.own[0] | ((uint64_t)pend.own[1] << 32);
        pend.csize = lz4_encode_block<true>(bytes, n_blk, *s_lz);
    }
    if (CODEC == CODEC_ZSTD_FAST) {
        const uint64_t bytes = (uint64_t)pend.own[0] | ((uint64_t)pend.own[1] << 32);
        pend.csize = zstd_tokenize_block(bytes, n_blk, pend.last, *s_lz, pend.staged);
    }
    if (CODEC == CODEC_ZSTD_MODELLED) {
        const uint64_t bytes = (uint64_t)pend.own[0] | ((uint64_t)pend.own[1] << 32);
        pend.csize = zstd_tokenize_block_m(bytes, n_blk, pend.last, *s_lz, pend.staged, zp);
    }
    if (CODEC == CODEC_DEFLATE) {
        const uint64_t bytes = (uint64_t)pend.own[0] | ((uint64_t)pend.own[1] << 32);
        pend.aux = deflate_adler_word(bytes, tile);
        pend.csize = deflate_encode_block<true>(bytes, n_blk, pend.last, *s_lz);
    }
    if (CODEC == CODEC_BLOSC) {
        const uint64_t bytes = (uint64_t)pend.own[0] | ((uint64_t)pend.own[1] << 32);
        pend.cown = bitshuffle_block(bytes, n_blk, *s_lz);
        pend.csize = lz4_encode_block(pend.cown, n_blk, *s_lz);
    }
    RC_PHASE(5);
    stores_behind = flush_pending<LEVEL1, CODEC, KEEP_BITMAP>(pend, tile, n_blk, bitmap, nb_stride, pix_slots, tile_cnt, blk_slots, blk_size, s_lz, st, blk_stride, comb, blk_aux);
    pend.valid = false;
    RC_PHASE(6);
}

template <int RWAVES, int BZ, bool ALIGNED, bool ASMLOAD, bool LEVEL1, int CODEC, bool KEEP_BITMAP, bool RAWVAL, int SB>
__global__ __launch_bounds__(64 * RWAVES) __attribute__((amdgpu_waves_per_eu((ALIGNED && ASMLOAD) ? ((RWAVES == 4 && LEVEL1) ? 3 : 4) : 1))) void k_reduce_tiles(const typename Src<SB>::T *__restrict__ frames,
                                                       const uint16_t *__restrict__ thr, uint64_t N, uint32_t ntiles,
                                                       uint32_t tile0, uint32_t tile_end,
                                                       uint32_t B, uint32_t ngroups, uint64_t nb,
                                                       uint8_t *__restrict__ bitmap, uint64_t nb_stride,
                                                       uint16_t *__restrict__ pix_slots, uint32_t *__restrict__ tile_cnt,
                                                       uint8_t *__restrict__ blk_slots, uint32_t *__restrict__ blk_size, uint32_t depth,
                                                       BatchStatus *__restrict__ status, ZmParams zm, uint32_t blk_stride, uint32_t comb,
                                                       uint32_t *__restrict__ blk_aux)
{
    if (blockIdx.x == 0 && threadIdx.x == 0) { status->code = 0; status->frame = 0; status->total = 0; }
    __shared__ uint16_t s_code[CODEC == CODEC_ZSTD_MODELLED ? 256 : 2];
    if (CODEC == CODEC_ZSTD_MODELLED) {
        for (uint32_t i = threadIdx.x; i < 128; i += 64 * RWAVES) reinterpret_cast<uint32_t *>(s_code)[i] = reinterpret_cast<const uint32_t *>(zm.lit_code)[i];
        __syncthreads();
        zm.lit_code = s_code;
    }
    __shared__ Lz4Lds s_lz[CODEC ? RWAVES : 1];
    __shared__ __attribute__((aligned(16))) uint8_t s_bm[CODEC ? 1 : RWAVES][CODEC ? 16 : TILE_BM];
    __shared__ WaveStage s_stage[LEVEL1 ? RWAVES : 1];

    const uint32_t xcd = blockIdx.x & 7u, j = blockIdx.x >> 3;
    const uint32_t grp = j % ngroups;
    const uint32_t tblock = (j / ngroups) * 8u + xcd;
    const int lane = lane_id();
    const int w = __builtin_amdgcn_readfirstlane((int)(threadIdx.x >> 6));
    const uint32_t tile = tile0 + tblock * RWAVES + w;
    if (tile >= tile_end) return;
    const uint64_t lane_px0 = (uint64_t)tile * TILE_PX + (uint64_t)lane * 8;
    const uint32_t f0 = grp * BZ;
    if (f0 >= B) return;
    const bool full = (uint64_t)(tile + 1) * TILE_PX <= N;

    typename Src<SB>::X xa[R];
    if (ASMLOAD) vm_issue_loads(xa, frames + (uint64_t)f0 * N + lane_px0);
    u32x4 t[R];
#pragma unroll
    for (int r = 0; r < R; ++r) t[r] = load8<ALIGNED, false, 2>(thr, lane_px0 + (uint64_t)r * GROUP_PX, N, 0xFFFF);
    const uint32_t n_blk = (uint32_t)min((uint64_t)TILE_BM, nb - (uint64_t)tile * TILE_BM);
    Lz4Lds *lz = &s_lz[CODEC ? w : 0];
    uint8_t *bm = s_bm[CODEC ? 0 : w];
    WaveStage *st = &s_stage[LEVEL1 ? w : 0];
    Pending pend;
    pend.valid = false;
    pend.ft = 0; pend.f = 0; pend.cnt = 0; pend.csize = 0; pend.own = u32x2{0u, 0u};
    pend.staged = 0; pend.last = tile + 1 == ntiles; pend.cown = 0; pend.aux = 0;
    pend.depth = (LEVEL1 && !RAWVAL) ? depth : 16u;
    pend.buf = nullptr;

    uint32_t stores_behind = 0;
#pragma unroll 1
    for (int z = 0; z < BZ; ++z) {
        const uint32_t f = f0 + z;
        if (f >= B) break;
        const bool nxt = z + 1 < BZ && f + 1 < B;
        reduce_one_frame<ALIGNED, ASMLOAD, LEVEL1, CODEC, KEEP_BITMAP, RAWVAL, SB>(xa, frames + (uint64_t)f * N, frames + (uint64_t)(f + 1) * N, nxt, t,
                                                                             lane_px0, N, full, f, tile, (uint64_t)f * ntiles + tile, n_blk,
                                                                             bitmap, nb_stride, pix_slots, tile_cnt, blk_slots,
                                                                             blk_size, lz, bm, st, pend, stores_behind, zm, blk_stride, comb, blk_aux);
        if (!nxt) break;
    }
    flush_pending<LEVEL1, CODEC, KEEP_BITMAP>(pend, tile, n_blk, bitmap, nb_stride, pix_slots, tile_cnt, blk_slots, blk_size, lz, st, blk_stride, comb, blk_aux);
}

template <int BZ, bool AL, bool L1, int CODEC, bool KEEP, bool RAW, int SB>
static void launch_reduce_t(const Scratch &sc, const typename Src<SB>::T *frames, uint32_t B, uint32_t depth, hipStream_t s, hipStream_t s_tail)
{
    const uint32_t ngroups = (B + BZ - 1) / BZ;
    const uint32_t nfull = AL ? (uint32_t)(sc.N / TILE_PX) : 0u;
    const ZmParams zm{reinterpret_cast<const uint16_t *>(sc.zm_lit_code), sc.zm_valid, sc.zm_budget, sc.zm_seq_bits};
    const uint32_t comb = (L1 && !RAW && CODEC) ? sc.comb : COMB_OFF;
    const bool three = L1 && !RAW && CODEC != CODEC_DEFLATE &&
                       (CODEC == CODEC_LZ4_RUNS || CODEC == CODEC_LZ4_EVENTS || sc.ntiles > 8192 || (CODEC == CODEC_ZSTD_MODELLED && (sc.zm_valid & ZM_LITS_ONLY)));
    auto go = [&](auto rw) {
        constexpr int RW = decltype(rw)::value;
        auto grid_for = [&](uint32_t nt) { return (((nt + RW - 1) / RW + 7) / 8) * 8 * ngroups; };
        if (nfull)
            hipLaunchKernelGGL((k_reduce_tiles<RW, BZ, AL, AL, L1, CODEC, KEEP, RAW, SB>), dim3(grid_for(nfull)), dim3(64 * RW), 0, s, frames, sc.thr, sc.N,
                               sc.ntiles, 0u, nfull, B, ngroups, sc.nb, sc.bitmap, sc.nb_stride, sc.pix_slots, sc.tile_cnt, sc.blk_slots,
                               sc.blk_size, depth, sc.status, zm, sc.blk_stride, comb, sc.blk_aux);
        if (nfull < sc.ntiles) {
            if (AL && sc.N % 8 != 0)
                hipLaunchKernelGGL((k_reduce_tiles<RW, BZ, false, false, L1, CODEC, KEEP, RAW, SB>), dim3(grid_for(sc.ntiles - nfull)), dim3(64 * RW), 0, nfull ? s_tail : s, frames,
                                   sc.thr, sc.N, sc.ntiles, nfull, sc.ntiles, B, ngroups, sc.nb, sc.bitmap, sc.nb_stride, sc.pix_slots, sc.tile_cnt,
                                   sc.blk_slots, sc.blk_size, depth, sc.status, zm, sc.blk_stride, comb, sc.blk_aux);
            else
                hipLaunchKernelGGL((k_reduce_tiles<RW, BZ, AL, false, L1, CODEC, KEEP, RAW, SB>), dim3(grid_for(sc.ntiles - nfull)), dim3(64 * RW), 0, nfull ? s_tail : s, frames,
                                   sc.thr, sc.N, sc.ntiles, nfull, sc.ntiles, B, ngroups, sc.nb, sc.bitmap, sc.nb_stride, sc.pix_slots, sc.tile_cnt,
                                   sc.blk_slots, sc.blk_size, depth, sc.status, zm, sc.blk_stride, comb, sc.blk_aux);
        }
    };
    if constexpr (SB == 2) {
        if (three) { go(int_c<3>{}); return; }
    }
    go(int_c<4>{});
}
template <int BZ, bool AL, bool L1, bool RAW, int SB>
static void launch_reduce_c(const Scratch &sc, const typename Src<SB>::T *frames, uint32_t B, uint32_t codec, bool keep, uint32_t depth, hipStream_t s, hipStream_t s_tail)
{
    if (RAW) keep = true;
#define RC_CODEC(C)                                                                                      \
    if (codec == C) {                                                                                    \
        if (keep) launch_reduce_t<BZ, AL, L1, C, true, RAW, SB>(sc, frames, B, depth, s, s_tail);        \
        else if (!RAW) launch_reduce_t<BZ, AL, L1, C, false, false, SB>(sc, frames, B, depth, s, s_tail); \
        return;                                                                                          \
    }
    RC_CODEC(CODEC_LZ4_RUNS) RC_CODEC(CODEC_LZ4_EVENTS) RC_CODEC(CODEC_ZSTD_FAST) RC_CODEC(CODEC_ZSTD_MODELLED) RC_CODEC(CODEC_BLOSC) RC_CODEC(CODEC_DEFLATE)
#undef RC_CODEC
    launch_reduce_t<BZ, AL, L1, CODEC_NONE, true, RAW, SB>(sc, frames, B, depth, s, s_tail);
}
template <int BZ, bool AL, int SB>
static void launch_reduce_a(const Scratch &sc, const typename Src<SB>::T *frames, uint32_t B, uint32_t level, uint32_t codec, bool keep,
                            uint32_t depth, hipStream_t s, hipStream_t s_tail)
{
    if (level == 2) launch_reduce_c<BZ, AL, true, true, SB>(sc, frames, B, codec, keep, depth, s, s_tail);
    else if (level == 1) launch_reduce_c<BZ, AL, true, false, SB>(sc, frames, B, codec, keep, depth, s, s_tail);
    else launch_reduce_c<BZ, AL, false, false, SB>(sc, frames, B, codec, keep, depth, s, s_tail);
}
#ifdef RC_PHASE_TIMING
extern "C" __attribute__((visibility("default"))) int rc_debug_phases(unsigned long long *out16)
{
    unsigned long long z[16] = {};
    if (hipDeviceSynchronize() != hipSuccess) return -1;
    if (hipMemcpyFromSymbol(out16, HIP_SYMBOL(g_phase), sizeof z) != hipSuccess) return -1;
    if (hipMemcpyToSymbol(HIP_SYMBOL(g_phase), z, sizeof z) != hipSuccess) return -1;
    return 0;
}
#endif
void launch_reduce(const Scratch &sc, const void *frames, uint32_t B, uint32_t level, uint32_t codec, bool keep_bitmap,
                   uint32_t depth, hipStream_t s, hipStream_t s_tail, uint32_t src_bytes)
{
    if (depth == 0 || depth > 16) depth = 16;
    if (!s_tail) s_tail = s;
    const bool aligned = !sc.guarded_loads;
    if (src_bytes == 1) {
        const uint8_t *f8 = static_cast<const uint8_t *>(frames);
        if (aligned) launch_reduce_a<REDUCE_BZ, true, 1>(sc, f8, B, level, codec, keep_bitmap, depth, s, s_tail);
        else launch_reduce_a<REDUCE_BZ, false, 1>(sc, f8, B, level, codec, keep_bitmap, depth, s, s_tail);
        return;
    }
    const uint16_t *f16 = static_cast<const uint16_t *>(frames);
    if (aligned) launch_reduce_a<REDUCE_BZ, true, 2>(sc, f16, B, level, codec, keep_bitmap, depth, s, s_tail);
    else launch_reduce_a<REDUCE_BZ, false, 2>(sc, f16, B, level, codec, keep_bitmap, depth, s, s_tail);
}

constexpr int SCAN_T = 256, SCAN_W = SCAN_T / 64;

__device__ __forceinline__ uint32_t scan_block_excl(uint32_t v, uint32_t *sm, uint32_t *total)
{
    const int w = threadIdx.x >> 6;
    const uint32_t inc = wave_incl_scan(v);
    if (lane_id() == 63) sm[w] = inc;
    __syncthreads();
    uint32_t base = 0, tot = 0;
#pragma unroll
    for (int i = 0; i < SCAN_W; ++i) {
        const uint32_t x = sm[i];
        if (i < w) base += x;
        tot += x;
    }
    __syncthreads();
    *total = tot;
    return base + inc - v;
}

template <int SCAN_I>
__device__ __forceinline__ void scan_row(uint32_t *__restrict__ row, uint32_t *__restrict__ orow, uint32_t n,
                                         uint32_t *__restrict__ total, uint32_t *sm, const uint32_t *adj = nullptr)
{
    uint32_t carry = 0;
    for (uint32_t t0 = 0; t0 < n; t0 += SCAN_T * SCAN_I) {
        const uint32_t t = t0 + threadIdx.x * SCAN_I;
        uint32_t v[SCAN_I], s = 0;
#pragma unroll
        for (int k = 0; k < SCAN_I; ++k) {
            v[k] = t + k < n ? row[t + k] : 0;
            if (adj) {
                v[k] &= 0xFFFFu;
                if (t + k == adj[0]) v[k] += adj[1];
                if (t + k == adj[2]) v[k] += adj[3];
                if (t + k < n) row[t + k] = v[k];
            }
            s += v[k];
        }
        uint32_t tot;
        uint32_t ex = carry + scan_block_excl(s, sm, &tot);
#pragma unroll
        for (int k = 0; k < SCAN_I; ++k) {
            if (t + k < n) orow[t + k] = ex;
            ex += v[k];
        }
        carry += tot;
    }
    if (threadIdx.x == 0) *total = carry;
}

__device__ __forceinline__ void zstd_rewrite_defs(const uint32_t *__restrict__ row, uint8_t *__restrict__ slots, uint32_t stride,
                                                  const uint8_t *__restrict__ tree, uint32_t tl, const uint8_t *__restrict__ sdesc, uint32_t sl,
                                                  uint32_t t_tree, uint32_t t_seq, uint32_t which, uint8_t *s_img, uint32_t *s_pos)
{
    for (int pass = 0; pass < 2; ++pass) {
        const uint32_t t = pass == 0 ? t_tree : t_seq;
        if (t == 0xFFFFFFFFu || (pass == 1 && t == t_tree) || !((which >> pass) & 1u)) continue;
        const uint32_t a_tl = pass == 0 ? tl : 0u, a_sl = (pass == 1 || t_seq == t_tree) ? sl : 0u;
        uint8_t *slot = slots + (uint64_t)t * stride;
        const uint32_t size = row[t] & 0xFFFFu;
        __syncthreads();
        for (uint32_t i = threadIdx.x; i < (size + 3) / 4; i += blockDim.x)
            reinterpret_cast<uint32_t *>(s_img)[i] = reinterpret_cast<const uint32_t *>(slot)[i];
        __syncthreads();
        if (threadIdx.x == 0) { uint32_t q; (void)zm_block_needs(s_img, &q); *s_pos = q; }
        __syncthreads();
        const uint32_t pos = *s_pos;
        for (uint32_t i = threadIdx.x; i < size + a_tl + a_sl; i += blockDim.x)
            slot[i] = zm_defs_byte(s_img, pos, tree, a_tl, sdesc, a_sl, i);
    }
    __syncthreads();
}

__device__ __forceinline__ void zstd_place_defs(const uint32_t *__restrict__ row, uint32_t n, uint8_t *__restrict__ slots, uint32_t stride,
                                                const uint8_t *__restrict__ tree, uint32_t tree_len, const uint8_t *__restrict__ sdesc,
                                                uint32_t sdesc_len, uint32_t *adj)
{
    __shared__ uint32_t s_first[2];
    __shared__ uint32_t s_pos;
    __shared__ __attribute__((aligned(16))) uint8_t s_img[PIX_SLOT + 16];
    if (threadIdx.x < 2) s_first[threadIdx.x] = 0xFFFFFFFFu;
    __syncthreads();
    const uint32_t w0 = row[0];
    const bool both0 = (w0 & ZW_TREE) && ((w0 & ZW_SEQ) || !sdesc_len);
    if (both0) {
        if (threadIdx.x == 0) { s_first[0] = 0; if (sdesc_len) s_first[1] = 0; }
    } else {
        uint32_t mt = 0xFFFFFFFFu, mq = 0xFFFFFFFFu;
        for (uint32_t t = threadIdx.x; t < n; t += SCAN_T) {
            const uint32_t w = row[t];
            if ((w & ZW_TREE) && t < mt) mt = t;
            if ((w & ZW_SEQ) && t < mq) mq = t;
        }
        if (mt != 0xFFFFFFFFu) atomicMin(&s_first[0], mt);
        if (mq != 0xFFFFFFFFu) atomicMin(&s_first[1], mq);
    }
    __syncthreads();
    const uint32_t t_tree = s_first[0], t_seq = s_first[1];
    const uint32_t tl = t_tree != 0xFFFFFFFFu ? tree_len : 0u, sl = t_seq != 0xFFFFFFFFu ? sdesc_len : 0u;
    if (threadIdx.x == 0) { adj[0] = t_tree; adj[1] = tl; adj[2] = t_seq; adj[3] = sl; }
    zstd_rewrite_defs(row, slots, stride, tree, tl, sdesc, sl, t_tree, t_seq, 3u, s_img, &s_pos);
}

__global__ __launch_bounds__(SCAN_T) void k_pix_scan(Scratch sc, uint32_t depth)
{
    __shared__ uint32_t sm[SCAN_W];
    __shared__ uint32_t s_adj[4];
    const uint32_t f = blockIdx.x;
    const ZstdModel *M = sc.zm_model;
    const uint32_t npk = packed_bytes(sc.frame_nnz[f], depth);
    const uint32_t nch = value_chunks(npk, PIX_CHUNK);
    uint32_t *row = sc.chunk_size + (uint64_t)f * sc.nchunk_max;
    zstd_place_defs(row, nch, sc.pix_chunks + (uint64_t)f * sc.nchunk_max * PIX_SLOT, PIX_SLOT, M->pix_desc, M->pix_desc_len, nullptr, 0, s_adj);
    scan_row<16>(row, sc.chunk_off + (uint64_t)f * sc.nchunk_max, nch, sc.frame_pbytes + f, sm, s_adj);
}
void launch_pix_scan(const Scratch &sc, uint32_t B, uint32_t depth, hipStream_t s)
{
    hipLaunchKernelGGL(k_pix_scan, dim3(B), dim3(SCAN_T), 0, s, sc, depth);
}

template <int SCAN_I>
__global__ __launch_bounds__(SCAN_T) void k_scan_frames(Scratch sc, int with_counts, int with_blocks)
{
    __shared__ uint32_t sm[SCAN_W];
    __shared__ uint32_t s_carry;
    __shared__ uint32_t s_adj[4];
    const uint32_t f = blockIdx.x, n = sc.ntiles;
    const uint64_t fr = (uint64_t)f * n;
    if (with_blocks) {
        if (sc.zm_model) {
            const ZstdModel *M = sc.zm_model;
            zstd_place_defs(sc.blk_size + fr, n, sc.blk_slots + fr * sc.blk_stride, sc.blk_stride, M->lit_desc, M->lit_desc_len, M->seq_desc,
                            M->seq_desc_len, s_adj);
        }
        scan_row<SCAN_I>(sc.blk_size + fr, sc.blk_off + fr, n, sc.frame_cbytes + f, sm, sc.zm_model ? s_adj : nullptr);
    }
    if (!with_counts) return;
    uint32_t *row = sc.tile_cnt + fr;
    scan_row<SCAN_I>(row, sc.tile_off + fr, n, sc.frame_nnz + f, sm);
    uint32_t *nrow = sc.tile_next + fr;
    if (threadIdx.x == 0) s_carry = n;
    __syncthreads();
    const uint32_t per_round = SCAN_T * SCAN_I;
    const uint32_t nrounds = (n + per_round - 1) / per_round;
    for (uint32_t c = nrounds; c-- > 0;) {
        const uint32_t t = c * per_round + threadIdx.x * SCAN_I;
        uint32_t v[SCAN_I];
        uint32_t first = 0xFFFFFFFFu;
#pragma unroll
        for (int k = SCAN_I - 1; k >= 0; --k) {
            v[k] = t + k < n ? row[t + k] : 0;
            if (v[k]) first = t + k;
        }
        uint32_t m = first;
#pragma unroll
        for (int d = 1; d < 64; d <<= 1) {
            const uint32_t y = __shfl_down(m, d);
            if (lane_id() + d < 64) m = min(m, y);
        }
        const int w = threadIdx.x >> 6;
        if (lane_id() == 0) sm[w] = m;
        __syncthreads();
        uint32_t right = s_carry;
#pragma unroll
        for (int i = SCAN_W - 1; i >= 0; --i)
            if (i > w) right = min(right, sm[i]);
        uint32_t excl = __shfl_down(m, 1);
        if (lane_id() == 63) excl = 0xFFFFFFFFu;
        uint32_t nxt = min(excl, right);
#pragma unroll
        for (int k = SCAN_I - 1; k >= 0; --k) {
            if (t + k < n) nrow[t + k] = nxt;
            if (v[k]) nxt = t + k;
        }
        __syncthreads();
        if (threadIdx.x == 0) {
            uint32_t all = s_carry;
#pragma unroll
            for (int i = 0; i < SCAN_W; ++i) all = min(all, sm[i]);
            s_carry = all;
        }
        __syncthreads();
    }
}

constexpr int SEG_I = 16, SEG = SCAN_T * SEG_I;
struct ScanPart { uint32_t blk_sum, cnt_sum, first_nonempty, first_tree, first_seq, pad[3]; };

__global__ __launch_bounds__(SCAN_T) void k_scan_seg(Scratch sc, int with_counts, int with_blocks)
{
    __shared__ uint32_t sm[SCAN_W];
    __shared__ uint32_t s_min[3];
    const uint32_t seg = blockIdx.x, f = blockIdx.y, n = sc.ntiles, nseg = gridDim.x;
    const uint64_t fr = (uint64_t)f * n;
    const uint32_t t = seg * SEG + threadIdx.x * SEG_I;
    ScanPart *part = reinterpret_cast<ScanPart *>(sc.scan_part) + (uint64_t)f * nseg + seg;
    if (threadIdx.x < 3) s_min[threadIdx.x] = 0xFFFFFFFFu;
    __syncthreads();
    uint32_t blk_sum = 0, cnt_sum = 0;
    if (with_blocks) {
        uint32_t *row = sc.blk_size + fr, *orow = sc.blk_off + fr;
        const bool zm = sc.zm_model != nullptr;
        uint32_t v[SEG_I], sum = 0, mt = 0xFFFFFFFFu, mq = 0xFFFFFFFFu;
#pragma unroll
        for (int k = 0; k < SEG_I; ++k) {
            const uint32_t w = t + k < n ? row[t + k] : 0;
            if (zm) {
                if ((w & ZW_TREE) && mt == 0xFFFFFFFFu) mt = t + k;
                if ((w & ZW_SEQ) && mq == 0xFFFFFFFFu) mq = t + k;
                v[k] = w & 0xFFFFu;
                if (t + k < n) row[t + k] = v[k];
            } else v[k] = w;
            sum += v[k];
        }
        if (mt != 0xFFFFFFFFu) atomicMin(&s_min[1], mt);
        if (mq != 0xFFFFFFFFu) atomicMin(&s_min[2], mq);
        uint32_t ex = scan_block_excl(sum, sm, &blk_sum);
#pragma unroll
        for (int k = 0; k < SEG_I; ++k) {
            if (t + k < n) orow[t + k] = ex;
            ex += v[k];
        }
    }
    if (with_counts) {
        const uint32_t *row = sc.tile_cnt + fr;
        uint32_t *orow = sc.tile_off + fr, *nrow = sc.tile_next + fr;
        uint32_t v[SEG_I], sum = 0, first = 0xFFFFFFFFu;
#pragma unroll
        for (int k = SEG_I - 1; k >= 0; --k) {
            v[k] = t + k < n ? row[t + k] : 0;
            if (v[k]) first = t + k;
            sum += v[k];
        }
        uint32_t ex = scan_block_excl(sum, sm, &cnt_sum);
#pragma unroll
        for (int k = 0; k < SEG_I; ++k) {
            if (t + k < n) orow[t + k] = ex;
            ex += v[k];
        }
        uint32_t m = first;
#pragma unroll
        for (int d = 1; d < 64; d <<= 1) {
            const uint32_t y = __shfl_down(m, d);
            if (lane_id() + d < 64) m = min(m, y);
        }
        const int w = threadIdx.x >> 6;
        __syncthreads();
        if (lane_id() == 0) sm[w] = m;
        __syncthreads();
        uint32_t right = 0xFFFFFFFFu;
#pragma unroll
        for (int i = SCAN_W - 1; i >= 0; --i)
            if (i > w) right = min(right, sm[i]);
        uint32_t excl = __shfl_down(m, 1);
        if (lane_id() == 63) excl = 0xFFFFFFFFu;
        uint32_t nxt = min(excl, right);
#pragma unroll
        for (int k = SEG_I - 1; k >= 0; --k) {
            if (t + k < n) nrow[t + k] = nxt;
            if (v[k]) nxt = t + k;
        }
        if (first != 0xFFFFFFFFu) atomicMin(&s_min[0], first);
    }
    __syncthreads();
    if (threadIdx.x == 0) {
        if (with_blocks) { part->blk_sum = blk_sum; part->first_tree = s_min[1]; part->first_seq = s_min[2]; }
        if (with_counts) { part->cnt_sum = cnt_sum; part->first_nonempty = s_min[0]; }
    }
}

__global__ __launch_bounds__(SCAN_T) void k_scan_fix(Scratch sc, int with_counts, int with_blocks)
{
    __shared__ uint32_t s_v[8];
    __shared__ uint32_t s_pos;
    __shared__ __attribute__((aligned(16))) uint8_t s_img[PIX_SLOT + 16];
    const uint32_t seg = blockIdx.x, f = blockIdx.y, n = sc.ntiles, nseg = gridDim.x;
    const uint64_t fr = (uint64_t)f * n;
    const ScanPart *parts = reinterpret_cast<const ScanPart *>(sc.scan_part) + (uint64_t)f * nseg;
    if (threadIdx.x == 0) {
        uint32_t bb = 0, cb = 0, bt = 0, ct = 0, nx = n, tt = 0xFFFFFFFFu, tq = 0xFFFFFFFFu;
        for (uint32_t i = 0; i < nseg; ++i) {
            const ScanPart p = parts[i];
            if (i < seg) { bb += p.blk_sum; cb += p.cnt_sum; }
            bt += p.blk_sum; ct += p.cnt_sum;
            if (i > seg && p.first_nonempty < nx) nx = p.first_nonempty;
            tt = min(tt, p.first_tree); tq = min(tq, p.first_seq);
        }
        s_v[0] = bb; s_v[1] = cb; s_v[2] = nx; s_v[3] = tt; s_v[4] = tq; s_v[5] = bt; s_v[6] = ct;
    }
    __syncthreads();
    const uint32_t lo = seg * SEG, hi = min(lo + (uint32_t)SEG, n);
    if (with_blocks) {
        uint32_t tl = 0, sl = 0;
        const uint32_t t_tree = s_v[3], t_seq = s_v[4];
        if (sc.zm_model) {
            const ZstdModel *M = sc.zm_model;
            tl = t_tree != 0xFFFFFFFFu ? M->lit_desc_len : 0u;
            sl = t_seq != 0xFFFFFFFFu ? M->seq_desc_len : 0u;
            const uint32_t mine = (t_tree >= lo && t_tree < hi ? 1u : 0u) | (t_seq >= lo && t_seq < hi ? 2u : 0u);
            if (mine) {
                zstd_rewrite_defs(sc.blk_size + fr, sc.blk_slots + fr * sc.blk_stride, sc.blk_stride, M->lit_desc, tl, M->seq_desc, sl, t_tree, t_seq, mine, s_img, &s_pos);
                if (threadIdx.x == 0) {
                    if (mine & 1u) sc.blk_size[fr + t_tree] += tl;
                    if (mine & 2u) sc.blk_size[fr + t_seq] += sl;
                }
            }
        }
        uint32_t *orow = sc.blk_off + fr;
        const uint32_t base = s_v[0];
        for (uint32_t t = lo + threadIdx.x; t < hi; t += SCAN_T)
            orow[t] += base + (t > t_tree ? tl : 0u) + (t > t_seq ? sl : 0u);
        if (seg == 0 && threadIdx.x == 0) sc.frame_cbytes[f] = s_v[5] + tl + sl;
    }
    if (with_counts) {
        uint32_t *orow = sc.tile_off + fr, *nrow = sc.tile_next + fr;
        const uint32_t base = s_v[1], nx = s_v[2];
        for (uint32_t t = lo + threadIdx.x; t < hi; t += SCAN_T) {
            orow[t] += base;
            if (nrow[t] == 0xFFFFFFFFu) nrow[t] = nx;
        }
        if (seg == 0 && threadIdx.x == 0) sc.frame_nnz[f] = s_v[6];
    }
}

void launch_scans(const Scratch &sc, uint32_t B, bool with_counts, bool with_blocks, hipStream_t s)
{
    if (!with_counts && !with_blocks) return;
    if (sc.ntiles > (uint32_t)SEG && sc.scan_part) {
        const dim3 grid((sc.ntiles + SEG - 1) / SEG, B);
        hipLaunchKernelGGL(k_scan_seg, grid, dim3(SCAN_T), 0, s, sc, with_counts ? 1 : 0, with_blocks ? 1 : 0);
        hipLaunchKernelGGL(k_scan_fix, grid, dim3(SCAN_T), 0, s, sc, with_counts ? 1 : 0, with_blocks ? 1 : 0);
        return;
    }
    if (sc.ntiles > 8192) hipLaunchKernelGGL(k_scan_frames<32>, dim3(B), dim3(SCAN_T), 0, s, sc, with_counts ? 1 : 0, with_blocks ? 1 : 0);
    else hipLaunchKernelGGL(k_scan_frames<16>, dim3(B), dim3(SCAN_T), 0, s, sc, with_counts ? 1 : 0, with_blocks ? 1 : 0);
}

constexpr int LWG = WG;
__global__ __launch_bounds__(LWG) void k_layout(const uint32_t *__restrict__ frame_nnz,
                                                 const uint32_t *__restrict__ frame_cbytes, const uint32_t *__restrict__ frame_pbytes,
                                                 RecordParams rp, uint64_t nb,
                                                 uint32_t ntiles, uint32_t B, uint64_t out_cap, uint64_t *__restrict__ rec_off,
                                                 uint32_t *__restrict__ md, BatchStatus *__restrict__ st, u32x4 *__restrict__ zl_acc)
{
    __shared__ uint64_t s_part[LWG];
    __shared__ uint32_t s_bad;
    if (threadIdx.x == 0) s_bad = 0xFFFFFFFFu;
    __syncthreads();
    const uint32_t per = (B + LWG - 1) / LWG;
    const uint32_t lo = threadIdx.x * per;
    const uint32_t hi = min(lo + per, B);
    uint64_t sum = 0;
    for (uint32_t f = lo; f < hi; ++f) {
        const uint32_t nnz = rp.level == 1 ? frame_nnz[f] : 0;
        const uint32_t npk = rp.level == 1 ? packed_bytes(nnz, rp.depth) : 0;
        uint64_t sz;
        uint32_t m0 = 0, m1 = 0, m2 = 0;
        if (rp.emit == EMIT_RAW) {
            if (rp.level == 1) { sz = 8 + nb + npk; m0 = npk; }
            else sz = 4 + nb;
        } else {
            const FrameFmt ff = frame_fmt(rp.emit);
            const uint32_t cb = bitmap_hdr(ff, rp.emit, ntiles) + frame_cbytes[f] + ff.end;
            if (rp.level == 1) {
                const uint32_t cp = rp.pix_mode == PIX_MODE_SKIP ? ff.hdr + frame_pbytes[f] : stored_size(ff, npk);
                sz = 16 + (uint64_t)cb + cp; m0 = cb; m1 = cp; m2 = npk;
            } else { sz = 8 + (uint64_t)cb; m0 = cb; }
        }
        md[3 * f] = m0; md[3 * f + 1] = m1; md[3 * f + 2] = m2;
        if (zl_acc) { zl_acc[2 * f] = u32x4{0u, 0u, 0u, 0u}; zl_acc[2 * f + 1] = u32x4{0u, 0u, 0u, 0u}; }
        if (sz > rp.frame_bytes) atomicMin(&s_bad, f);
        rec_off[f + 1] = sz;
        sum += sz;
    }
    s_part[threadIdx.x] = sum;
    __syncthreads();
    uint64_t base = 0;
    for (uint32_t i = 0; i < threadIdx.x; ++i) base += s_part[i];
    for (uint32_t f = lo; f < hi; ++f) {
        const uint64_t sz = rec_off[f + 1];
        base += sz;
        rec_off[f + 1] = base;
    }
    if (threadIdx.x == 0) rec_off[0] = 0;
    __syncthreads();
    if (threadIdx.x == LWG - 1) {
        uint64_t total = 0;
        for (uint32_t i = 0; i < LWG; ++i) total += s_part[i];
        st->total = total;
        if (s_bad != 0xFFFFFFFFu) { st->code = -5; st->frame = s_bad; }
        else if (total > out_cap) { st->code = -2; st->frame = 0; }
    }
}

void launch_layout(const Scratch &sc, const RecordParams &rp, uint32_t B, uint64_t out_cap, uint64_t *rec_off,
                   uint32_t *md, hipStream_t s)
{
    hipLaunchKernelGGL(k_layout, dim3(1), dim3(LWG), 0, s, sc.frame_nnz, sc.frame_cbytes, sc.frame_pbytes, rp, sc.nb, sc.ntiles, B, out_cap,
                       rec_off, md, sc.status, reinterpret_cast<u32x4 *>(sc.zl_acc));
}

static uint32_t xxh32_small(const uint8_t *p, size_t n)
{
    const uint32_t P1 = 2654435761u, P2 = 2246822519u, P3 = 3266489917u, P4 = 668265263u, P5 = 374761393u;
    (void)P1; (void)P4;
    uint32_t h = 0  + P5 + (uint32_t)n;
    for (size_t i = 0; i < n; ++i) {
        h += p[i] * P5;
        h = ((h << 11) | (h >> 21)) * P1;
    }
    h ^= h >> 15; h *= P2; h ^= h >> 13; h *= P3; h ^= h >> 16;
    return h;
}
uint32_t lz4f_descriptor(uint8_t bd)
{
    const uint8_t desc[2] = {0x60 , bd};
    const uint8_t hc = (uint8_t)((xxh32_small(desc, 2) >> 8) & 0xFF);
    return desc[0] | ((uint32_t)desc[1] << 8) | ((uint32_t)hc << 16);
}

void launch_assemble(const Scratch &sc, const RecordParams &rp, uint32_t B, uint8_t *out, const uint64_t *rec_off,
                     uint32_t batch_seq, hipStream_t s)
{
    static const uint32_t hdr_bitmap = lz4f_descriptor(0x40);
    static const uint32_t hdr_pix = lz4f_descriptor(0x70);
    launch_gather(sc, rp, B, out, rec_off, hdr_bitmap, hdr_pix, batch_seq, s);
}

}
```

### pyrecode_amd/csrc/rc_reduce32.hip

```cpp
#include <type_traits>

#include "rc_launch.h"
#include "rc_lz4_block.h"
#include "rc_zstd_wave.h"

namespace rc {

constexpr int R32_WAVES = 1;
constexpr int R32_FPW = 16;
struct __attribute__((aligned(16))) Stage32 {
    uint32_t out[TILE_PX];
    Lz4Lds lz;
};

__global__ void k_threshold32(const uint32_t *__restrict__ dark, uint32_t eps, uint64_t N, uint32_t *__restrict__ thr)
{
    uint64_t i = (uint64_t)blockIdx.x * blockDim.x + threadIdx.x;
    const uint64_t stride = (uint64_t)gridDim.x * blockDim.x;
    for (; i < N; i += stride) thr[i] = dark[i] + eps;
}
void launch_threshold32(const uint32_t *dark, int64_t eps, uint64_t N, uint32_t *thr, hipStream_t s)
{
    uint32_t blocks = (uint32_t)((N + 255) / 256);
    if (blocks > 4096) blocks = 4096;
    hipLaunchKernelGGL(k_threshold32, dim3(blocks), dim3(256), 0, s, dark, (uint32_t)(uint64_t)eps, N, thr);
}

template <bool FULL, bool NT>
__device__ __forceinline__ void load_tile32(const uint32_t *__restrict__ base, uint64_t px0, uint64_t N, uint32_t fill, u32x4 (&v)[2 * R])
{
    const int lane = lane_id();
#pragma unroll
    for (int i = 0; i < 2 * R; ++i) {
        if (FULL) {
            typedef u32x4 u32x4_dw __attribute__((aligned(4)));
            const u32x4_dw *p = reinterpret_cast<const u32x4_dw *>(base + px0 + (uint64_t)i * 256 + (uint64_t)lane * 4);
            v[i] = NT ? __builtin_nontemporal_load(p) : *p;
        } else {
            const uint64_t px = px0 + (uint64_t)i * 256 + (uint64_t)lane * 4;
            if (px + 4 <= N) {
                typedef u32x4 u32x4_dw __attribute__((aligned(4)));
                v[i] = *reinterpret_cast<const u32x4_dw *>(base + px);
            } else {
#pragma unroll
                for (int k = 0; k < 4; ++k) v[i][k] = px + k < N ? base[px + k] : fill;
            }
        }
    }
}

template <int CODEC>
__device__ __forceinline__ void reduce_tile32(Stage32 &S, const u32x4 (&x)[2 * R], const u32x4 (&t)[2 * R], uint8_t *__restrict__ bm_dst,
                                              uint8_t *__restrict__ slot, uint32_t *__restrict__ cnt_dst, uint32_t depth, bool level1,
                                              uint8_t *__restrict__ blk_slot, uint32_t *__restrict__ blk_size_dst, uint32_t n_blk, bool last_blk)
{
    const int lane = lane_id();
    uint32_t base = 0;
#pragma unroll
    for (int g = 0; g < R; ++g) {
        uint32_t m = 0;
        u32x4 ra, rb;
#pragma unroll
        for (int k = 0; k < 4; ++k) {
            const uint32_t a = x[2 * g][k], ta = t[2 * g][k], b = x[2 * g + 1][k], tb = t[2 * g + 1][k];
            m |= (a > ta ? 1u : 0u) << k | (b > tb ? 1u : 0u) << (4 + k);
            ra[k] = a - ta;
            rb[k] = b - tb;
        }
        const uint32_t other = (uint32_t)__builtin_amdgcn_mov_dpp((int)m, 0xB1, 0xF, 0xF, true);
        const uint32_t byte = (lane & 1) ? ((other >> 4) | (m & 0xF0u)) : ((m & 0xFu) | ((other & 0xFu) << 4));
        S.lz.raw[g * 64 + (lane & 1) * 32 + (lane >> 1)] = (uint8_t)byte;
        if (level1) {
            const uint32_t ca = (uint32_t)__builtin_popcount(m & 0xFu), cb = (uint32_t)__builtin_popcount(m >> 4);
            const uint32_t inc = wave_incl_scan(ca | cb << 16);
            const uint32_t tot = wave_last(inc);
            if (tot) {
                uint32_t pa = base + (inc & 0xFFFFu) - ca, pb = base + (tot & 0xFFFFu) + (inc >> 16) - cb;
#pragma unroll
                for (int k = 0; k < 4; ++k) {
                    if (m >> k & 1u) S.out[pa++] = ra[k];
                    if (m >> (4 + k) & 1u) S.out[pb++] = rb[k];
                }
            }
            base += (tot & 0xFFFFu) + (tot >> 16);
        }
    }
    __builtin_amdgcn_wave_barrier();
    const u32x2 ownv = *reinterpret_cast<const u32x2 *>(&S.lz.raw[lane * 8]);
    if (bm_dst) *reinterpret_cast<u32x2 *>(bm_dst + lane * 8) = ownv;
    if (CODEC == CODEC_ZSTD_FAST) {
        uint32_t staged;
        const uint32_t word = zstd_tokenize_block((uint64_t)ownv[0] | ((uint64_t)ownv[1] << 32), n_blk, last_blk, S.lz, staged);
        zstd_store_block(blk_slot, n_blk, last_blk, word, staged, S.lz);
        if (lane == 0) *blk_size_dst = word;
        __builtin_amdgcn_wave_barrier();
    } else if (CODEC) {
        uint64_t own = (uint64_t)ownv[0] | ((uint64_t)ownv[1] << 32);
        if (CODEC == CODEC_BLOSC) own = bitshuffle_block(own, n_blk, S.lz);
        const uint32_t csize = lz4_encode_block<CODEC == CODEC_LZ4_EVENTS>(own, n_blk, S.lz);
        const uint32_t used = lz4_store_block(blk_slot, own, n_blk, csize, S.lz, CODEC == CODEC_BLOSC);
        if (lane == 0) *blk_size_dst = used;
        __builtin_amdgcn_wave_barrier();
    }
    if (!level1) return;
    const uint32_t total = base;
    const uint32_t nbits = total * depth;
    const uint32_t ndw = (((nbits + 31) >> 5) + 31u) & ~31u;
    if (depth < 32) {
        const uint32_t dmask = (1u << depth) - 1u;
        for (uint32_t j0 = 0; j0 < ndw; j0 += 64) {
            const uint32_t j = j0 + lane;
            uint32_t v = (32u * j) / depth;
            const uint32_t o = 32u * j - v * depth;
            uint64_t acc = 0;
            uint32_t filled = 0;
            if (v < total) { acc = (uint64_t)(S.out[v] & dmask) >> o; filled = depth - o; ++v; }
            while (filled < 32 && v < total) {
                acc |= (uint64_t)(S.out[v] & dmask) << filled;
                filled += depth;
                ++v;
            }
            __builtin_amdgcn_wave_barrier();
            if (j < ndw) S.out[j] = (uint32_t)acc;
            __builtin_amdgcn_wave_barrier();
        }
    } else {
        for (uint32_t j = total + lane; j < ndw; j += 64) S.out[j] = 0;
        __builtin_amdgcn_wave_barrier();
    }
    uint32_t *dst = reinterpret_cast<uint32_t *>(slot);
    for (uint32_t j = lane; j < ndw; j += 64) dst[j] = S.out[j];
    if (lane == 0) *cnt_dst = total;
    __builtin_amdgcn_wave_barrier();
}

template <bool FULL, int CODEC>
__global__ __launch_bounds__(64 * R32_WAVES) __attribute__((amdgpu_waves_per_eu(2, 2))) void k_reduce_tiles32(const uint32_t *__restrict__ frames, const uint32_t *__restrict__ thr, uint64_t N,
                                                       uint32_t ntiles, uint32_t tile0, uint32_t tile_n, uint32_t B, uint8_t *__restrict__ bitmap, uint64_t nb_stride,
                                                       uint8_t *__restrict__ pix_slots, uint32_t pix_slot_bytes,
                                                       uint32_t *__restrict__ tile_cnt, uint32_t depth, uint32_t level1,
                                                       BatchStatus *__restrict__ status, uint8_t *__restrict__ blk_slots, uint32_t blk_stride,
                                                       uint32_t *__restrict__ blk_size, uint64_t nb)
{
    if (blockIdx.x == 0 && blockIdx.y == 0 && threadIdx.x == 0) { status->code = 0; status->frame = 0; status->total = 0; }
    __shared__ Stage32 s_st[R32_WAVES];
    const int wv = __builtin_amdgcn_readfirstlane((int)(threadIdx.x >> 6));
    Stage32 &S = s_st[wv];
    const uint32_t tile = tile0 + blockIdx.x * R32_WAVES + wv;
    if (tile >= (FULL ? tile0 + tile_n : ntiles)) return;
    const uint32_t f0 = blockIdx.y * R32_FPW, f1 = f0 + R32_FPW < B ? f0 + R32_FPW : B;
    const uint64_t px0 = (uint64_t)tile * TILE_PX;
    const uint32_t n_blk = (uint32_t)min((uint64_t)TILE_BM, nb - (uint64_t)tile * TILE_BM);
    u32x4 t[2 * R], xa[2 * R];
    load_tile32<FULL, false>(thr, px0, N, 0xFFFFFFFFu, t);
    auto one = [&](const u32x4 (&x)[2 * R], uint32_t f) {
        const uint64_t ft = (uint64_t)f * ntiles + tile;
        reduce_tile32<CODEC>(S, x, t, bitmap ? bitmap + (uint64_t)f * nb_stride + (uint64_t)tile * TILE_BM : nullptr, pix_slots + ft * pix_slot_bytes,
                             tile_cnt + ft, depth, level1 != 0, blk_slots + ft * blk_stride, blk_size + ft, n_blk, tile + 1 == ntiles);
    };
    if (FULL) {
        u32x4 xb[2 * R];
        load_tile32<true, true>(frames + (uint64_t)f0 * N, px0, N, 0, xa);
        for (uint32_t f = f0; f < f1; f += 2) {
            if (f + 1 < f1) load_tile32<true, true>(frames + (uint64_t)(f + 1) * N, px0, N, 0, xb);
            one(xa, f);
            if (f + 1 < f1) {
                if (f + 2 < f1) load_tile32<true, true>(frames + (uint64_t)(f + 2) * N, px0, N, 0, xa);
                one(xb, f + 1);
            }
        }
    } else {
        for (uint32_t f = f0; f < f1; ++f) {
            load_tile32<false, true>(frames + (uint64_t)f * N, px0, N, 0, xa);
            one(xa, f);
        }
    }
}

void launch_reduce32(const Scratch &sc, const uint32_t *frames, const uint32_t *thr32, uint32_t B, uint32_t level, uint32_t depth, hipStream_t s,
                     uint32_t codec, bool keep_bitmap)
{
    const uint32_t nfull = (uint32_t)(sc.N / TILE_PX), fy = (B + R32_FPW - 1) / R32_FPW;
    uint8_t *slots = reinterpret_cast<uint8_t *>(sc.pix_slots);
    uint8_t *bitmap = (codec == CODEC_NONE || keep_bitmap) ? sc.bitmap : nullptr;
    auto go = [&](auto full, auto cd) {
        constexpr bool FULL = decltype(full)::value;
        constexpr int CODEC = decltype(cd)::value;
        hipLaunchKernelGGL((k_reduce_tiles32<FULL, CODEC>), FULL ? dim3((nfull + R32_WAVES - 1) / R32_WAVES, fy) : dim3(1, fy), dim3(64 * R32_WAVES), 0, s, frames, thr32, sc.N, sc.ntiles,
                           FULL ? 0u : nfull, FULL ? nfull : 1u, B,
                           bitmap, sc.nb_stride, slots, sc.pix_slot_bytes, sc.tile_cnt, depth, level == 1 ? 1u : 0u, sc.status, sc.blk_slots, sc.blk_stride,
                           sc.blk_size, sc.nb);
    };
    auto both = [&](auto cd) {
        if (nfull) go(std::true_type{}, cd);
        if (nfull < sc.ntiles) go(std::false_type{}, cd);
    };
    if (codec == CODEC_LZ4_RUNS) both(int_c<CODEC_LZ4_RUNS>{});
    else if (codec == CODEC_LZ4_EVENTS) both(int_c<CODEC_LZ4_EVENTS>{});
    else if (codec == CODEC_BLOSC) both(int_c<CODEC_BLOSC>{});
    else if (codec == CODEC_ZSTD_FAST) both(int_c<CODEC_ZSTD_FAST>{});
    else both(int_c<CODEC_NONE>{});
}

}
```

Measured before the change: 167,400 frames/s.

## Replace per-tile scans and layout with fused per-item plan kernel for L1/L3 LZ4 chains

For level 1/3 with raw, LZ4 or blosc emission, the separate multi-pass scan kernels and the layout kernel are replaced by one plan kernel. It computes per-frame totals and per-gather-item offsets, and its last workgroup, picked by an atomic ticket, runs the layout. The gather kernel rebuilds per-tile offsets with an in-wave inclusive scan over the item base, and finds the next nonzero tile by ballot scanning instead of the tile_next array. The reduce launch can also signal its completion event directly, which cuts launches and scratch traffic but adds ticket-based cross-workgroup synchronisation and extra wave scans inside gather.

```diff
diff --git a/pyrecode_amd/csrc/rc_api.hip b/pyrecode_amd/csrc/rc_api.hip
--- a/pyrecode_amd/csrc/rc_api.hip
+++ b/pyrecode_amd/csrc/rc_api.hip
@@ -111,19 +111,31 @@
     return (scheme == RC_SCHEME_LZ4 || scheme == RC_SCHEME_ZSTD || scheme == RC_SCHEME_BLOSC_LZ4 || scheme == RC_SCHEME_ZLIB_DEVICE) ? 1 : 0;
 }
 
+static bool plain_chain(const rc_ctx *c)
+{
+    using namespace rc;
+    return (c->level == 1 || c->level == 3) && (c->emit == EMIT_RAW || c->emit == EMIT_LZ4 || c->emit == EMIT_BLOSC);
+}
+
 static int alloc_set(rc_ctx *c, rc::Scratch &sc, DevMem &model_mem)
 {
     using namespace rc;
     DevMem &m = c->dmem;
     const uint64_t B = c->max_batch, T = sc.ntiles;
+    const bool plan = plain_chain(c);
     RC_ALLOC(m, sc.bitmap, B * sc.nb_stride + 64);
     RC_ALLOC(m, sc.tile_cnt, B * T * 4);
-    RC_ALLOC(m, sc.tile_off, B * T * 4);
-    RC_ALLOC(m, sc.tile_next, B * T * 4);
+    if (plan) {
+        RC_ALLOC(m, sc.item_coff, B * ((T + 7) / 8) * 4);
+        RC_ALLOC(m, sc.item_boff, B * ((T + 7) / 8) * 4);
+    } else {
+        RC_ALLOC(m, sc.tile_off, B * T * 4);
+        RC_ALLOC(m, sc.tile_next, B * T * 4);
+    }
     RC_ALLOC(m, sc.frame_nnz, B * 4);
     RC_ALLOC(m, sc.frame_cbytes, B * 4);
-    RC_ALLOC(m, sc.scan_part, B * ((T + 255) / 256) * 32);
-    RC_ALLOC(m, sc.status, sizeof(BatchStatus));
+    if (!plan) RC_ALLOC(m, sc.scan_part, B * ((T + 255) / 256) * 32);
+    RC_ALLOC(m, sc.status, STATUS_BYTES);
     if (c->level != 3) RC_ALLOC(m, sc.pix_slots, B * T * TILE_PX * 2 + 64);
     if (c->emit != EMIT_RAW) {
         if (c->level == 1) {
@@ -132,7 +144,7 @@
         }
         RC_ALLOC(m, sc.blk_slots, B * T * (uint64_t)sc.blk_stride + 256);
         RC_ALLOC(m, sc.blk_size, B * T * 4);
-        RC_ALLOC(m, sc.blk_off, B * T * 4);
+        if (!plan) RC_ALLOC(m, sc.blk_off, B * T * 4);
         if (c->emit == EMIT_DEFLATE) {
             RC_ALLOC(m, sc.blk_aux, B * T * 4);
             RC_ALLOC(m, sc.zl_acc, B * 32);
@@ -153,7 +165,7 @@
     }
     HIP_TRY(hipMemset(sc.frame_nnz, 0, B * 4));
     HIP_TRY(hipMemset(sc.frame_cbytes, 0, B * 4));
-    HIP_TRY(hipMemset(sc.status, 0, sizeof(BatchStatus)));
+    HIP_TRY(hipMemset(sc.status, 0, STATUS_BYTES));
     return RC_OK;
 }
 
@@ -522,19 +534,21 @@
     }
     const uint32_t codec = fused_codec(c->emit, c->clevel, c->modelled, c->src_bytes);
     const bool keep_maps = c->keep_bitmap || c->emit == EMIT_RAW;
+    const bool plan = plain_chain(c);
+    hipEvent_t red = ev ? ev[1] : c->ev_red[k];
+    bool red_signalled = false;
     if (c->src_bytes == 4)
         launch_reduce32(sc, static_cast<const uint32_t *>(frames_dev), c->thr32, n, c->level, c->depth, s, codec, keep_maps);
     else
-        launch_reduce(sc, frames_dev, n, c->level, codec, keep_maps, c->depth, s, tail, c->src_bytes);
+        red_signalled = launch_reduce(sc, frames_dev, n, c->level, codec, keep_maps, c->depth, s, tail, c->src_bytes, plan && !ev ? red : nullptr);
     const bool all_ev = ev && (timed || c->profile_all);
-    hipEvent_t red = ev ? ev[1] : c->ev_red[k];
-    HIP_TRY(hipEventRecord(red, s));
+    if (!red_signalled) HIP_TRY(hipEventRecord(red, s));
     HIP_TRY(hipStreamWaitEvent(ps, red, 0));
     if (c->level == 2) launch_l2(sc, n, c->nx, c->l2_sum, c->depth, ps);
     const bool lits_only = c->modelled && (c->h_model->valid & ZM_LITS_ONLY);
     if (c->emit == EMIT_ZSTD && !lits_only) launch_zstd_fse(sc, n, fitted_seq ? (const void *)&c->d_model->seq : c->d_ztab, fitted_seq, ps);
     if (all_ev) HIP_TRY(hipEventRecord(ev[2], ps));
-    launch_scans(sc, n, c->level != 3, c->emit != EMIT_RAW, ps);
+    if (!plan) launch_scans(sc, n, c->level != 3, c->emit != EMIT_RAW, ps);
     if (all_ev) HIP_TRY(hipEventRecord(ev[3], ps));
     if (c->values_on) {
         rp.pix_mode = PIX_MODE_FLAT;
@@ -552,8 +566,9 @@
     }
     c->prev_out = out_dev; c->prev_out_cap = out_cap; c->prev_n = n;
     c->prev_rec = reinterpret_cast<const uint8_t *>(rec_off_dev); c->prev_md = reinterpret_cast<const uint8_t *>(md_dev);
-    launch_layout(sc, rp, n, out_cap, rec_off_dev, md_dev, ps);
-    launch_assemble(sc, rp, n, out_dev, rec_off_dev, c->batch_seq, ps);
+    if (plan) launch_plan(sc, rp, n, c->level != 3, c->emit != EMIT_RAW, out_cap, rec_off_dev, md_dev, ps);
+    else launch_layout(sc, rp, n, out_cap, rec_off_dev, md_dev, ps);
+    launch_assemble(sc, rp, n, out_dev, rec_off_dev, c->batch_seq, ps, plan);
     ++c->batch_seq;
     if (c->values_on) launch_values_gather(c->values, sc, n, c->depth, 16, out_dev, rec_off_dev, ps);
     if (ev) HIP_TRY(hipEventRecord(ev[4], ps));
diff --git a/pyrecode_amd/csrc/rc_device.h b/pyrecode_amd/csrc/rc_device.h
--- a/pyrecode_amd/csrc/rc_device.h
+++ b/pyrecode_amd/csrc/rc_device.h
@@ -77,6 +77,9 @@
     uint32_t frame;
     uint64_t total;
 };
+__host__ __device__ inline uint32_t *plan_ticket(BatchStatus *st) { return reinterpret_cast<uint32_t *>(st + 1); }
+constexpr size_t STATUS_BYTES = 2 * sizeof(BatchStatus);
+
 __host__ __device__ inline unsigned long long first_err_key(uint32_t batch_seq, int32_t code, uint32_t frame)
 {
     return ~(((unsigned long long)(batch_seq & 0xFFFFFFu) << 40) | ((unsigned long long)((uint32_t)(-code) & 0xFFu) << 32) | frame);
diff --git a/pyrecode_amd/csrc/rc_gather.hip b/pyrecode_amd/csrc/rc_gather.hip
--- a/pyrecode_amd/csrc/rc_gather.hip
+++ b/pyrecode_amd/csrc/rc_gather.hip
@@ -16,6 +16,7 @@
     BatchStatus *status, *first_err;
     uint64_t nb, nb_stride, pixraw_stride;
     uint32_t ntiles, blk_stride, pix_slot_bytes, comb;
+    const uint32_t *item_coff, *item_boff;
 };
 
 typedef u32x4 u32x4_u __attribute__((aligned(1)));
@@ -82,7 +83,7 @@
 
 constexpr int GATHER_U = 4, GATHER_UB = 3;
 constexpr int GATHER_WPE = 8;
-template <bool BITS, int U, bool ADLER>
+template <bool BITS, int U, bool ADLER, bool PLAN>
 __global__ __launch_bounds__(64) __attribute__((amdgpu_waves_per_eu(GATHER_WPE))) void k_gather(GatherArgs sc, RecordParams rp, uint8_t *__restrict__ out, const uint64_t *__restrict__ rec_off,
                                                uint32_t lz4f_hdr_bitmap, uint32_t lz4f_hdr_pix, uint32_t batch_seq, uint32_t gpf, uint32_t nitems, uint32_t tpi)
 {
@@ -118,6 +119,8 @@
         uint32_t word = 0, bsz = 0, bdst = 0, cnt = 0, rn = 0, rdst = 0, rs = 0xFFFFFFFFu, ps0 = 0, flags = 0, blo = 0;
         AdlerAcc ad{0u, 0u};
         if (have && rp.emit != EMIT_RAW && (!flat || (sc.comb == COMB_BEHIND_BLOCK && pixp))) word = sc.blk_size[frow + t];
+        uint32_t plan_boff = 0, plan_coff = 0;
+        if (PLAN && rp.emit != EMIT_RAW && !flat) plan_boff = sc.item_boff[item] + wave_incl_scan(word) - word;
         if (have && !flat) {
             if (rp.emit == EMIT_RAW) {
                 const uint64_t b0 = (uint64_t)t * TILE_BM;
@@ -125,15 +128,16 @@
                 bdst = (uint32_t)(bitmap_pos + b0);
             } else {
                 bsz = word;
-                const uint32_t boff = bhdr + sc.blk_off[frow + t];
+                const uint32_t boff = bhdr + (PLAN ? plan_boff : sc.blk_off[frow + t]);
                 bdst = (uint32_t)bitmap_pos + boff;
                 if (rp.emit == EMIT_BLOSC) store_u32_le(rec + bitmap_pos + 16 + 4 * (uint64_t)t, boff);
             }
         }
+        if (have && pixp) cnt = sc.tile_cnt[frow + t];
+        if (PLAN && pixp) plan_coff = sc.item_coff[item] + wave_incl_scan(cnt) - cnt;
         if (have && pixp) {
-            cnt = sc.tile_cnt[frow + t];
             if (cnt) {
-                const ResidGeom q = resid_geom(sc.tile_off[frow + t], cnt, d);
+                const ResidGeom q = resid_geom(PLAN ? plan_coff : sc.tile_off[frow + t], cnt, d);
                 ps0 = q.ps0;
                 if (ADLER) blo = q.b_lo;
                 if (sc.comb) {
@@ -201,7 +205,8 @@
         }
         if (pixp) {
         ResidGeom q{0u, 0u, 0u, 0u};
-        if (cnt) q = resid_geom(sc.tile_off[frow + t], cnt, d);
+        if (PLAN) plan_coff = sc.item_coff[item] + wave_incl_scan(cnt) - cnt;
+        if (cnt) q = resid_geom(PLAN ? plan_coff : sc.tile_off[frow + t], cnt, d);
         for (uint64_t m = __builtin_amdgcn_ballot_w64((packed >> 31) != 0); m; m &= m - 1) {
             const uint32_t k = (uint32_t)__builtin_ctzll(m);
             const uint32_t n = lane_get(q.n, k), p0 = lane_get(q.ps0, k), b0 = lane_get(q.b_lo, k), rsk = lane_get(rs, k);
@@ -240,7 +245,21 @@
                 } else cur = 65;
             }
         }
-        if (got < 8) {
+        if (PLAN) {
+            for (uint32_t w0 = t0 + tpi + 1; w0 < sc.ntiles && __builtin_amdgcn_ballot_w64(got < 8) != 0; w0 += 64) {
+                const uint32_t wc = w0 + lane < sc.ntiles ? sc.tile_cnt[frow + w0 + lane] : 0u;
+                for (uint64_t m = __builtin_amdgcn_ballot_w64(wc != 0); m && __builtin_amdgcn_ballot_w64(got < 8) != 0; m &= m - 1) {
+                    const uint32_t k = (uint32_t)__builtin_ctzll(m), tt = w0 + k;
+                    const uint32_t cc = lane_get(wc, k);
+                    const uint32_t fd = *reinterpret_cast<const uint32_t *>(residual_src(sc, frow + tt, sc.comb == COMB_BEHIND_BLOCK ? sc.blk_size[frow + tt] : 0u, cc, d));
+                    if (got < 8) {
+                        const uint32_t take = min(8u - got, cc * d);
+                        byte |= (fd & ((1u << take) - 1u)) << got;
+                        got += take;
+                    }
+                }
+            }
+        } else if (got < 8) {
             uint32_t tt = cur == 65 ? (t0 + tpi - 1 < sc.ntiles ? sc.tile_next[frow + t0 + tpi - 1] : sc.ntiles) : (t0 + tpi < sc.ntiles ? sc.tile_next[frow + t0 + tpi] : sc.ntiles);
             while (tt < sc.ntiles) {
                 const uint32_t cc = sc.tile_cnt[frow + tt];
@@ -294,22 +313,24 @@
 
 
 void launch_gather(const Scratch &sc, const RecordParams &rp, uint32_t B, uint8_t *out, const uint64_t *rec_off, uint32_t hdr_bitmap, uint32_t hdr_pix,
-                   uint32_t batch_seq, hipStream_t s)
-{
-    uint32_t tpi = 64;
-    while (tpi > 8 && (uint64_t)B * ((sc.ntiles + tpi - 1) / tpi) < 1024) tpi >>= 1;
+                   uint32_t batch_seq, hipStream_t s, bool plan)
+{
+    const uint32_t tpi = gather_tpi(B, sc.ntiles);
     const uint32_t gpf = (sc.ntiles + tpi - 1) / tpi, nitems = gpf * B, wgs = nitems;
     const GatherArgs ga{sc.blk_slots, sc.bitmap, sc.pix_slots, sc.blk_size, sc.blk_off, sc.tile_cnt, sc.tile_off, sc.tile_next, sc.frame_nnz, sc.frame_cbytes,
-                        sc.frame_pbytes, sc.blk_aux, sc.zl_acc, sc.pixraw, sc.status, sc.first_err, sc.nb, sc.nb_stride, sc.pixraw_stride, sc.ntiles, sc.blk_stride, sc.pix_slot_bytes, sc.comb};
+                        sc.frame_pbytes, sc.blk_aux, sc.zl_acc, sc.pixraw, sc.status, sc.first_err, sc.nb, sc.nb_stride, sc.pixraw_stride, sc.ntiles, sc.blk_stride, sc.pix_slot_bytes, sc.comb, sc.item_coff, sc.item_boff};
     const bool bits = rp.level == 1 && rp.depth % 8 != 0;
-    if (rp.emit == EMIT_DEFLATE) {
-        if (bits) hipLaunchKernelGGL((k_gather<true, GATHER_UB - 1, true>), dim3(wgs), dim3(64), 0, s, ga, rp, out, rec_off, hdr_bitmap, hdr_pix, batch_seq, gpf, nitems, tpi);
-        else hipLaunchKernelGGL((k_gather<false, GATHER_U, true>), dim3(wgs), dim3(64), 0, s, ga, rp, out, rec_off, hdr_bitmap, hdr_pix, batch_seq, gpf, nitems, tpi);
+    if (plan) {
+        if (bits) hipLaunchKernelGGL((k_gather<true, GATHER_UB, false, true>), dim3(wgs), dim3(64), 0, s, ga, rp, out, rec_off, hdr_bitmap, hdr_pix, batch_seq, gpf, nitems, tpi);
+        else hipLaunchKernelGGL((k_gather<false, GATHER_U, false, true>), dim3(wgs), dim3(64), 0, s, ga, rp, out, rec_off, hdr_bitmap, hdr_pix, batch_seq, gpf, nitems, tpi);
+    } else if (rp.emit == EMIT_DEFLATE) {
+        if (bits) hipLaunchKernelGGL((k_gather<true, GATHER_UB - 1, true, false>), dim3(wgs), dim3(64), 0, s, ga, rp, out, rec_off, hdr_bitmap, hdr_pix, batch_seq, gpf, nitems, tpi);
+        else hipLaunchKernelGGL((k_gather<false, GATHER_U, true, false>), dim3(wgs), dim3(64), 0, s, ga, rp, out, rec_off, hdr_bitmap, hdr_pix, batch_seq, gpf, nitems, tpi);
         if (rp.pix_mode != PIX_MODE_FLAT) hipLaunchKernelGGL(k_zlib_finish, dim3((B + 63) / 64), dim3(64), 0, s, ga, rp, out, rec_off, B);
     } else if (bits)
-        hipLaunchKernelGGL((k_gather<true, GATHER_UB, false>), dim3(wgs), dim3(64), 0, s, ga, rp, out, rec_off, hdr_bitmap, hdr_pix, batch_seq, gpf, nitems, tpi);
+        hipLaunchKernelGGL((k_gather<true, GATHER_UB, false, false>), dim3(wgs), dim3(64), 0, s, ga, rp, out, rec_off, hdr_bitmap, hdr_pix, batch_seq, gpf, nitems, tpi);
     else
-        hipLaunchKernelGGL((k_gather<false, GATHER_U, false>), dim3(wgs), dim3(64), 0, s, ga, rp, out, rec_off, hdr_bitmap, hdr_pix, batch_seq, gpf, nitems, tpi);
-}
-
-}
+        hipLaunchKernelGGL((k_gather<false, GATHER_U, false, false>), dim3(wgs), dim3(64), 0, s, ga, rp, out, rec_off, hdr_bitmap, hdr_pix, batch_seq, gpf, nitems, tpi);
+}
+
+}
diff --git a/pyrecode_amd/csrc/rc_launch.h b/pyrecode_amd/csrc/rc_launch.h
--- a/pyrecode_amd/csrc/rc_launch.h
+++ b/pyrecode_amd/csrc/rc_launch.h
@@ -56,7 +56,16 @@
     uint16_t *l2_base = nullptr;
     uint32_t *chunk_aux = nullptr;
     const DeflateModel *dz_model = nullptr;
+    uint32_t *item_coff = nullptr;
+    uint32_t *item_boff = nullptr;
 };
+
+inline uint32_t gather_tpi(uint32_t B, uint32_t ntiles)
+{
+    uint32_t tpi = 64;
+    while (tpi > 8 && (uint64_t)B * ((ntiles + tpi - 1) / tpi) < 1024) tpi >>= 1;
+    return tpi;
+}
 
 constexpr uint32_t EMIT_RAW = 0u;
 constexpr uint32_t EMIT_ZSTD = 1u;
@@ -89,8 +98,8 @@
 };
 
 void launch_threshold(const void *dark, int64_t eps, uint64_t N, uint16_t *thr, hipStream_t s, uint32_t src_bytes = 2);
-void launch_reduce(const Scratch &sc, const void *frames, uint32_t B, uint32_t level, uint32_t codec, bool keep_bitmap,
-                   uint32_t depth, hipStream_t s, hipStream_t s_tail = nullptr, uint32_t src_bytes = 2);
+bool launch_reduce(const Scratch &sc, const void *frames, uint32_t B, uint32_t level, uint32_t codec, bool keep_bitmap,
+                   uint32_t depth, hipStream_t s, hipStream_t s_tail = nullptr, uint32_t src_bytes = 2, hipEvent_t done = nullptr);
 void launch_threshold32(const uint32_t *dark, int64_t eps, uint64_t N, uint32_t *thr, hipStream_t s);
 void launch_reduce32(const Scratch &sc, const uint32_t *frames, const uint32_t *thr32, uint32_t B, uint32_t level, uint32_t depth, hipStream_t s,
                      uint32_t codec = CODEC_NONE, bool keep_bitmap = true);
@@ -98,10 +107,12 @@
 void launch_scans(const Scratch &sc, uint32_t B, bool with_counts, bool with_blocks, hipStream_t s);
 void launch_layout(const Scratch &sc, const RecordParams &rp, uint32_t B, uint64_t out_cap, uint64_t *rec_off,
                    uint32_t *md, hipStream_t s);
+void launch_plan(const Scratch &sc, const RecordParams &rp, uint32_t B, bool with_counts, bool with_blocks, uint64_t out_cap, uint64_t *rec_off,
+                 uint32_t *md, hipStream_t s);
 void launch_assemble(const Scratch &sc, const RecordParams &rp, uint32_t B, uint8_t *out, const uint64_t *rec_off,
-                     uint32_t batch_seq, hipStream_t s);
+                     uint32_t batch_seq, hipStream_t s, bool plan = false);
 void launch_gather(const Scratch &sc, const RecordParams &rp, uint32_t B, uint8_t *out, const uint64_t *rec_off, uint32_t hdr_bitmap, uint32_t hdr_pix,
-                   uint32_t batch_seq, hipStream_t s);
+                   uint32_t batch_seq, hipStream_t s, bool plan);
 enum ValueStage : uint32_t {
     VALUES_NONE = 0,
     VALUES_ZSTD_HUFF,
diff --git a/pyrecode_amd/csrc/rc_reduce.hip b/pyrecode_amd/csrc/rc_reduce.hip
--- a/pyrecode_amd/csrc/rc_reduce.hip
+++ b/pyrecode_amd/csrc/rc_reduce.hip
@@ -1,6 +1,7 @@
 #include <cstddef>
 #include <cstdlib>
 #include <type_traits>
+#include <hip/hip_ext.h>
 
 #include "rc_launch.h"
 #include "rc_values.h"
@@ -478,7 +479,7 @@
                                                        BatchStatus *__restrict__ status, ZmParams zm, uint32_t blk_stride, uint32_t comb,
                                                        uint32_t *__restrict__ blk_aux)
 {
-    if (blockIdx.x == 0 && threadIdx.x == 0) { status->code = 0; status->frame = 0; status->total = 0; }
+    if (blockIdx.x == 0 && threadIdx.x == 0) { status->code = 0; status->frame = 0; status->total = 0; *plan_ticket(status) = 0; }
     __shared__ uint16_t s_code[CODEC == CODEC_ZSTD_MODELLED ? 256 : 2];
     if (CODEC == CODEC_ZSTD_MODELLED) {
         for (uint32_t i = threadIdx.x; i < 128; i += 64 * RWAVES) reinterpret_cast<uint32_t *>(s_code)[i] = reinterpret_cast<const uint32_t *>(zm.lit_code)[i];
@@ -533,7 +534,7 @@
 }
 
 template <int BZ, bool AL, bool L1, int CODEC, bool KEEP, bool RAW, int SB>
-static void launch_reduce_t(const Scratch &sc, const typename Src<SB>::T *frames, uint32_t B, uint32_t depth, hipStream_t s, hipStream_t s_tail)
+static void launch_reduce_t(const Scratch &sc, const typename Src<SB>::T *frames, uint32_t B, uint32_t depth, hipStream_t s, hipStream_t s_tail, hipEvent_t done)
 {
     const uint32_t ngroups = (B + BZ - 1) / BZ;
     const uint32_t nfull = AL ? (uint32_t)(sc.N / TILE_PX) : 0u;
@@ -544,7 +545,11 @@
     auto go = [&](auto rw) {
         constexpr int RW = decltype(rw)::value;
         auto grid_for = [&](uint32_t nt) { return (((nt + RW - 1) / RW + 7) / 8) * 8 * ngroups; };
-        if (nfull)
+        if (nfull && done)
+            hipExtLaunchKernelGGL((k_reduce_tiles<RW, BZ, AL, AL, L1, CODEC, KEEP, RAW, SB>), dim3(grid_for(nfull)), dim3(64 * RW), 0, s, nullptr, done, 0, frames, sc.thr, sc.N,
+                                  sc.ntiles, 0u, nfull, B, ngroups, sc.nb, sc.bitmap, sc.nb_stride, sc.pix_slots, sc.tile_cnt, sc.blk_slots,
+                                  sc.blk_size, depth, sc.status, zm, sc.blk_stride, comb, sc.blk_aux);
+        else if (nfull)
             hipLaunchKernelGGL((k_reduce_tiles<RW, BZ, AL, AL, L1, CODEC, KEEP, RAW, SB>), dim3(grid_for(nfull)), dim3(64 * RW), 0, s, frames, sc.thr, sc.N,
                                sc.ntiles, 0u, nfull, B, ngroups, sc.nb, sc.bitmap, sc.nb_stride, sc.pix_slots, sc.tile_cnt, sc.blk_slots,
                                sc.blk_size, depth, sc.status, zm, sc.blk_stride, comb, sc.blk_aux);
@@ -565,26 +570,26 @@
     go(int_c<4>{});
 }
 template <int BZ, bool AL, bool L1, bool RAW, int SB>
-static void launch_reduce_c(const Scratch &sc, const typename Src<SB>::T *frames, uint32_t B, uint32_t codec, bool keep, uint32_t depth, hipStream_t s, hipStream_t s_tail)
+static void launch_reduce_c(const Scratch &sc, const typename Src<SB>::T *frames, uint32_t B, uint32_t codec, bool keep, uint32_t depth, hipStream_t s, hipStream_t s_tail, hipEvent_t done)
 {
     if (RAW) keep = true;
 #define RC_CODEC(C)                                                                                      \
     if (codec == C) {                                                                                    \
-        if (keep) launch_reduce_t<BZ, AL, L1, C, true, RAW, SB>(sc, frames, B, depth, s, s_tail);        \
-        else if (!RAW) launch_reduce_t<BZ, AL, L1, C, false, false, SB>(sc, frames, B, depth, s, s_tail); \
+        if (keep) launch_reduce_t<BZ, AL, L1, C, true, RAW, SB>(sc, frames, B, depth, s, s_tail, done);        \
+        else if (!RAW) launch_reduce_t<BZ, AL, L1, C, false, false, SB>(sc, frames, B, depth, s, s_tail, done); \
         return;                                                                                          \
     }
     RC_CODEC(CODEC_LZ4_RUNS) RC_CODEC(CODEC_LZ4_EVENTS) RC_CODEC(CODEC_ZSTD_FAST) RC_CODEC(CODEC_ZSTD_MODELLED) RC_CODEC(CODEC_BLOSC) RC_CODEC(CODEC_DEFLATE)
 #undef RC_CODEC
-    launch_reduce_t<BZ, AL, L1, CODEC_NONE, true, RAW, SB>(sc, frames, B, depth, s, s_tail);
+    launch_reduce_t<BZ, AL, L1, CODEC_NONE, true, RAW, SB>(sc, frames, B, depth, s, s_tail, done);
 }
 template <int BZ, bool AL, int SB>
 static void launch_reduce_a(const Scratch &sc, const typename Src<SB>::T *frames, uint32_t B, uint32_t level, uint32_t codec, bool keep,
-                            uint32_t depth, hipStream_t s, hipStream_t s_tail)
-{
-    if (level == 2) launch_reduce_c<BZ, AL, true, true, SB>(sc, frames, B, codec, keep, depth, s, s_tail);
-    else if (level == 1) launch_reduce_c<BZ, AL, true, false, SB>(sc, frames, B, codec, keep, depth, s, s_tail);
-    else launch_reduce_c<BZ, AL, false, false, SB>(sc, frames, B, codec, keep, depth, s, s_tail);
+                            uint32_t depth, hipStream_t s, hipStream_t s_tail, hipEvent_t done)
+{
+    if (level == 2) launch_reduce_c<BZ, AL, true, true, SB>(sc, frames, B, codec, keep, depth, s, s_tail, done);
+    else if (level == 1) launch_reduce_c<BZ, AL, true, false, SB>(sc, frames, B, codec, keep, depth, s, s_tail, done);
+    else launch_reduce_c<BZ, AL, false, false, SB>(sc, frames, B, codec, keep, depth, s, s_tail, done);
 }
 #ifdef RC_PHASE_TIMING
 extern "C" __attribute__((visibility("default"))) int rc_debug_phases(unsigned long long *out16)
@@ -596,21 +601,23 @@
     return 0;
 }
 #endif
-void launch_reduce(const Scratch &sc, const void *frames, uint32_t B, uint32_t level, uint32_t codec, bool keep_bitmap,
-                   uint32_t depth, hipStream_t s, hipStream_t s_tail, uint32_t src_bytes)
+bool launch_reduce(const Scratch &sc, const void *frames, uint32_t B, uint32_t level, uint32_t codec, bool keep_bitmap,
+                   uint32_t depth, hipStream_t s, hipStream_t s_tail, uint32_t src_bytes, hipEvent_t done)
 {
     if (depth == 0 || depth > 16) depth = 16;
     if (!s_tail) s_tail = s;
+    const bool signalled = done && !sc.guarded_loads && sc.N / TILE_PX != 0;
     const bool aligned = !sc.guarded_loads;
     if (src_bytes == 1) {
         const uint8_t *f8 = static_cast<const uint8_t *>(frames);
-        if (aligned) launch_reduce_a<REDUCE_BZ, true, 1>(sc, f8, B, level, codec, keep_bitmap, depth, s, s_tail);
-        else launch_reduce_a<REDUCE_BZ, false, 1>(sc, f8, B, level, codec, keep_bitmap, depth, s, s_tail);
-        return;
+        if (aligned) launch_reduce_a<REDUCE_BZ, true, 1>(sc, f8, B, level, codec, keep_bitmap, depth, s, s_tail, done);
+        else launch_reduce_a<REDUCE_BZ, false, 1>(sc, f8, B, level, codec, keep_bitmap, depth, s, s_tail, done);
+        return signalled;
     }
     const uint16_t *f16 = static_cast<const uint16_t *>(frames);
-    if (aligned) launch_reduce_a<REDUCE_BZ, true, 2>(sc, f16, B, level, codec, keep_bitmap, depth, s, s_tail);
-    else launch_reduce_a<REDUCE_BZ, false, 2>(sc, f16, B, level, codec, keep_bitmap, depth, s, s_tail);
+    if (aligned) launch_reduce_a<REDUCE_BZ, true, 2>(sc, f16, B, level, codec, keep_bitmap, depth, s, s_tail, done);
+    else launch_reduce_a<REDUCE_BZ, false, 2>(sc, f16, B, level, codec, keep_bitmap, depth, s, s_tail, done);
+    return signalled;
 }
 
 constexpr int SCAN_T = 256, SCAN_W = SCAN_T / 64;
@@ -952,11 +959,9 @@
 }
 
 constexpr int LWG = WG;
-__global__ __launch_bounds__(LWG) void k_layout(const uint32_t *__restrict__ frame_nnz,
-                                                 const uint32_t *__restrict__ frame_cbytes, const uint32_t *__restrict__ frame_pbytes,
-                                                 RecordParams rp, uint64_t nb,
-                                                 uint32_t ntiles, uint32_t B, uint64_t out_cap, uint64_t *__restrict__ rec_off,
-                                                 uint32_t *__restrict__ md, BatchStatus *__restrict__ st, u32x4 *__restrict__ zl_acc)
+__device__ __forceinline__ void layout_body(const uint32_t *frame_nnz, const uint32_t *frame_cbytes, const uint32_t *frame_pbytes,
+                                            const RecordParams &rp, uint64_t nb, uint32_t ntiles, uint32_t B, uint64_t out_cap,
+                                            uint64_t *__restrict__ rec_off, uint32_t *__restrict__ md, BatchStatus *st, u32x4 *__restrict__ zl_acc)
 {
     __shared__ uint64_t s_part[LWG];
     __shared__ uint32_t s_bad;
@@ -1007,12 +1012,89 @@
         else if (total > out_cap) { st->code = -2; st->frame = 0; }
     }
 }
+__global__ __launch_bounds__(LWG) void k_layout(const uint32_t *__restrict__ frame_nnz,
+                                                 const uint32_t *__restrict__ frame_cbytes, const uint32_t *__restrict__ frame_pbytes,
+                                                 RecordParams rp, uint64_t nb,
+                                                 uint32_t ntiles, uint32_t B, uint64_t out_cap, uint64_t *__restrict__ rec_off,
+                                                 uint32_t *__restrict__ md, BatchStatus *__restrict__ st, u32x4 *__restrict__ zl_acc)
+{
+    layout_body(frame_nnz, frame_cbytes, frame_pbytes, rp, nb, ntiles, B, out_cap, rec_off, md, st, zl_acc);
+}
 
 void launch_layout(const Scratch &sc, const RecordParams &rp, uint32_t B, uint64_t out_cap, uint64_t *rec_off,
                    uint32_t *md, hipStream_t s)
 {
     hipLaunchKernelGGL(k_layout, dim3(1), dim3(LWG), 0, s, sc.frame_nnz, sc.frame_cbytes, sc.frame_pbytes, rp, sc.nb, sc.ntiles, B, out_cap,
                        rec_off, md, sc.status, reinterpret_cast<u32x4 *>(sc.zl_acc));
+}
+
+template <int SCAN_I>
+__device__ __forceinline__ void plan_row(const uint32_t *__restrict__ row, uint32_t *__restrict__ irow, uint32_t n, uint32_t tsh,
+                                         uint32_t *__restrict__ total, uint32_t *sm)
+{
+    const uint32_t imask = (1u << tsh) - 1u;
+    uint32_t carry = 0;
+    for (uint32_t t0 = 0; t0 < n; t0 += SCAN_T * SCAN_I) {
+        const uint32_t t = t0 + threadIdx.x * SCAN_I;
+        uint32_t v[SCAN_I], s = 0;
+#pragma unroll
+        for (int k = 0; k < SCAN_I; ++k) {
+            v[k] = t + k < n ? row[t + k] : 0;
+            s += v[k];
+        }
+        uint32_t tot;
+        uint32_t ex = carry + scan_block_excl(s, sm, &tot);
+#pragma unroll
+        for (int k = 0; k < SCAN_I; ++k) {
+            if (t + k < n && ((t + k) & imask) == 0) irow[(t + k) >> tsh] = ex;
+            ex += v[k];
+        }
+        carry += tot;
+    }
+    if (threadIdx.x == 0) *total = carry;
+}
+
+static_assert(SCAN_T == LWG, "k_plan's last workgroup runs the layout");
+template <int SCAN_I>
+__global__ __launch_bounds__(SCAN_T) void k_plan(const uint32_t *__restrict__ tile_cnt, const uint32_t *__restrict__ blk_size,
+                                                 uint32_t *__restrict__ item_coff, uint32_t *__restrict__ item_boff, uint32_t *frame_nnz,
+                                                 uint32_t *frame_cbytes, uint32_t tsh, RecordParams rp, uint64_t nb, uint32_t ntiles, uint32_t B,
+                                                 uint64_t out_cap, uint64_t *__restrict__ rec_off, uint32_t *__restrict__ md, BatchStatus *st)
+{
+    __shared__ uint32_t sm[SCAN_W];
+    __shared__ uint32_t s_last;
+    const uint32_t f = blockIdx.x, n = ntiles, gpf = (n + (1u << tsh) - 1u) >> tsh;
+    const uint64_t fr = (uint64_t)f * n, ir = (uint64_t)f * gpf;
+    if (blk_size) plan_row<SCAN_I>(blk_size + fr, item_boff + ir, n, tsh, frame_cbytes + f, sm);
+    if (tile_cnt) plan_row<SCAN_I>(tile_cnt + fr, item_coff + ir, n, tsh, frame_nnz + f, sm);
+    asm volatile("s_waitcnt vmcnt(0)" ::: "memory");
+    __syncthreads();
+    if (threadIdx.x == 0) {
+        __builtin_amdgcn_fence(__ATOMIC_RELEASE, "agent");
+        asm volatile("s_waitcnt vmcnt(0)" ::: "memory");
+        s_last = __hip_atomic_fetch_add(plan_ticket(st), 1u, __ATOMIC_RELAXED, __HIP_MEMORY_SCOPE_AGENT) == gridDim.x - 1 ? 1u : 0u;
+    }
+    __syncthreads();
+    if (!s_last) return;
+    if (threadIdx.x == 0) {
+        __builtin_amdgcn_fence(__ATOMIC_ACQUIRE, "agent");
+        asm volatile("s_waitcnt vmcnt(0)" ::: "memory");
+    }
+    __syncthreads();
+    layout_body(frame_nnz, frame_cbytes, nullptr, rp, nb, ntiles, B, out_cap, rec_off, md, st, nullptr);
+}
+
+void launch_plan(const Scratch &sc, const RecordParams &rp, uint32_t B, bool with_counts, bool with_blocks, uint64_t out_cap, uint64_t *rec_off,
+                 uint32_t *md, hipStream_t s)
+{
+    uint32_t tsh = 0;
+    while ((1u << tsh) < gather_tpi(B, sc.ntiles)) ++tsh;
+    const uint32_t *cnt = with_counts ? sc.tile_cnt : nullptr, *blk = with_blocks ? sc.blk_size : nullptr;
+    const dim3 grid(cnt || blk ? B : 1u);
+    if (sc.ntiles > 8192) hipLaunchKernelGGL(k_plan<32>, grid, dim3(SCAN_T), 0, s, cnt, blk, sc.item_coff, sc.item_boff, sc.frame_nnz, sc.frame_cbytes, tsh, rp,
+                                             sc.nb, sc.ntiles, B, out_cap, rec_off, md, sc.status);
+    else hipLaunchKernelGGL(k_plan<16>, grid, dim3(SCAN_T), 0, s, cnt, blk, sc.item_coff, sc.item_boff, sc.frame_nnz, sc.frame_cbytes, tsh, rp,
+                            sc.nb, sc.ntiles, B, out_cap, rec_off, md, sc.status);
 }
 
 static uint32_t xxh32_small(const uint8_t *p, size_t n)
@@ -1035,11 +1117,11 @@
 }
 
 void launch_assemble(const Scratch &sc, const RecordParams &rp, uint32_t B, uint8_t *out, const uint64_t *rec_off,
-                     uint32_t batch_seq, hipStream_t s)
+                     uint32_t batch_seq, hipStream_t s, bool plan)
 {
     static const uint32_t hdr_bitmap = lz4f_descriptor(0x40);
     static const uint32_t hdr_pix = lz4f_descriptor(0x70);
-    launch_gather(sc, rp, B, out, rec_off, hdr_bitmap, hdr_pix, batch_seq, s);
-}
-
-}
+    launch_gather(sc, rp, B, out, rec_off, hdr_bitmap, hdr_pix, batch_seq, s, plan);
+}
+
+}
diff --git a/pyrecode_amd/csrc/rc_reduce32.hip b/pyrecode_amd/csrc/rc_reduce32.hip
--- a/pyrecode_amd/csrc/rc_reduce32.hip
+++ b/pyrecode_amd/csrc/rc_reduce32.hip
@@ -142,7 +142,7 @@
                                                        BatchStatus *__restrict__ status, uint8_t *__restrict__ blk_slots, uint32_t blk_stride,
                                                        uint32_t *__restrict__ blk_size, uint64_t nb)
 {
-    if (blockIdx.x == 0 && blockIdx.y == 0 && threadIdx.x == 0) { status->code = 0; status->frame = 0; status->total = 0; }
+    if (blockIdx.x == 0 && blockIdx.y == 0 && threadIdx.x == 0) { status->code = 0; status->frame = 0; status->total = 0; *plan_ticket(status) = 0; }
     __shared__ Stage32 s_st[R32_WAVES];
     const int wv = __builtin_amdgcn_readfirstlane((int)(threadIdx.x >> 6));
     Stage32 &S = s_st[wv];
```

After: 164,000 frames/s. 0.979x the previous value.
